# realphongha/UDP-Pose

Measured on AMD Instinct MI355X. Metric: images/sec HRNet-W32 256x192 (infer+decode), higher is better.
Workload: dtype f16x2 (split fp16 hi+lo operands = 22 bits, 3 fp16 MFMAs per product, fp32 accumulate); 1 GPU; w32 256x192 f16x2 inference, batch=64 per GPU, flip-test on, DARK decode (forward on 2N images + flip fuse + udp_decode_gaussian); global_batch=64, parallelism=replicas x1 (no data-path collective), weights=seeded synthetic, BN stats calibrated (tests/golden/bn_calib_w32_gaussian.npz)

## Files before the change

udp-pose_amd/csrc/common.h:

```cpp
#pragma once
#include <hip/hip_runtime.h>

#include <cstdarg>
#include <cstdio>
#include <cstring>

#include "../../include/udp_pose_hip.h"

namespace udp {

inline char* err_buf() {
  static thread_local char buf[512] = {0};
  return buf;
}

inline int fail(int code, const char* fmt, ...) {
  va_list ap;
  va_start(ap, fmt);
  vsnprintf(err_buf(), 512, fmt, ap);
  va_end(ap);
  return code;
}

#define UDP_HIP_CHECK(expr)                                                                  \
  do {                                                                                       \
    hipError_t e_ = (expr);                                                                  \
    if (e_ != hipSuccess)                                                                    \
      return udp::fail(UDP_ERR_HIP, "%s failed: %s (%s:%d)", #expr, hipGetErrorString(e_),   \
                       __FILE__, __LINE__);                                                  \
  } while (0)

inline int ceil_div(int a, int b) { return (a + b - 1) / b; }

static __device__ int g_h2_overflow;
__device__ __forceinline__ void h2_range_check(float m) {
  if (!(m < 65520.f)) g_h2_overflow = 1;
}
__device__ __forceinline__ unsigned h2_mag(float v) { return __builtin_bit_cast(unsigned, v) & 0x7FFFFFFFu; }
__device__ __forceinline__ unsigned h2_max(unsigned a, unsigned b) { return a > b ? a : b; }
__device__ __forceinline__ void h2_range_check_bits(unsigned m) {
  if (m >= __builtin_bit_cast(unsigned, 65520.f)) g_h2_overflow = 1;
}
static inline int h2_overflow_fetch(hipStream_t s, int reset, int* flag) {
  int v = 0;
  UDP_HIP_CHECK(hipMemcpyFromSymbolAsync(&v, HIP_SYMBOL(g_h2_overflow), sizeof(int), 0, hipMemcpyDeviceToHost, s));
  UDP_HIP_CHECK(hipStreamSynchronize(s));
  if (v && reset) {
    const int z = 0;
    UDP_HIP_CHECK(hipMemcpyToSymbolAsync(HIP_SYMBOL(g_h2_overflow), &z, sizeof(int), 0, hipMemcpyHostToDevice, s));
    UDP_HIP_CHECK(hipStreamSynchronize(s));
  }
  *flag |= v != 0;
  return UDP_OK;
}

struct ConvParams {
  const void* in;
  void* out;
  const void* wgt;
  const float* bias;
  const void* wgt2;
  const float* bias2;
  const void* res;
  const void* up[3];
  int up_shift[3];
  int nup;
  int N, Hin, Win, Cin, Hout, Wout, Cout, CoutPad;
  int in_pitch, in_coff, out_pitch, out_coff, res_pitch, res_coff;
  int G, R, TW;
  int IH, IW;
  int tiles_x, tiles_y;
  unsigned mTX, mTY;
  int ntiles;
  unsigned mIW, mIH, mRT, mTW;
  int relu;
  int out_nchw_f32;
  int flip_from;
  int sbuf;
  int wfmt;
  int wexp;
  int in_stuff2;
  double* bn_ws;
  void* out2[2];
  const void* add2[2];
  int nout2, out2_coff[2], out2_pitch[2], add2_coff[2], add2_pitch[2];
};

constexpr int kMultiSegs = 64;
constexpr int kMultiTab = 480;
struct ConvMulti {
  ConvParams p[4];
  unsigned start[5];
  unsigned tiles[4];
  unsigned ncby[4];
  int code[4];
  unsigned seg_start[kMultiSegs];
  unsigned seg_first[kMultiSegs];
  int seg_mem[kMultiSegs];
  unsigned tab_n;
  unsigned tab[kMultiTab];
};

}

namespace udp {
struct Launch {
  const void* fn = nullptr;
  dim3 grid, block;
  unsigned lds = 0;
  int groupable = 0;
  int ws_cp = 0;
  ConvParams p;
};
int describe_conv_ws(ConvParams p, int ks, int stride, Launch* out, bool grouped = false);
struct WsTile {
  int cp, pb, G, R, TW, wgs, sbuf;
  size_t lds;
};
int choose_conv_ws(ConvParams& p, int ks, int stride, bool grouped, WsTile* best);
int describe_ws_multi(const Launch* members, int n, ConvMulti* m, Launch* out);
int describe_conv_chain(ConvParams p, Launch* out);
void ws_set_fill_wgs(long wgs);
int ws_set_stamps(unsigned long long* dev_buf);
int describe_deconv(ConvParams p, int dtype, Launch* out);
int deconv_h2_overflow(hipStream_t s, int reset, int* flag);
int dwconv_validate(const udp_conv_op& o, int dtype);
int pixshuf_validate(const udp_conv_op& o, int dtype);
int describe_dwconv(ConvParams p, int dtype, int ks, int stride, Launch* out);
int describe_pixshuf(ConvParams p, int dtype, Launch* out);
int se_validate(const udp_conv_op& o, int dtype);
int describe_se(ConvParams p, int dtype, Launch* out);
int dwconv_h2_overflow(hipStream_t s, int reset, int* flag);
int gnorm_validate(const udp_conv_op& o, int dtype);
int linattn_validate(const udp_conv_op& o, int dtype);
int describe_gnorm(ConvParams p, int dtype, Launch* out);
int describe_linattn(ConvParams p, int dtype, Launch* out);
int lnorm_validate(const udp_conv_op& o, int dtype);
int mhattn_validate(const udp_conv_op& o, int dtype);
int act_op_validate(const udp_conv_op& o, int dtype);
int describe_lnorm(ConvParams p, int dtype, Launch* out);
int describe_mhattn(ConvParams p, int dtype, Launch* out);
int describe_act(ConvParams p, int dtype, Launch* out);
int attn_h2_overflow(hipStream_t s, int reset, int* flag);
int conv_h2_overflow(hipStream_t s, int reset, int* flag);
int conv_ws_h2_overflow(hipStream_t s, int reset, int* flag);
int psa_h2_overflow(hipStream_t s, int reset, int* flag);
}
```

udp-pose_amd/csrc/conv.hip:

```cpp
#include "conv_dev.h"

namespace udp {
template <typename T, int KS, int NB, int MBW>
__device__ __forceinline__ void mfma_chunk(f32x4 (&acc)[MBW][NB], const unsigned char* sb, const unsigned char* wrow,
                                           const int (&prow)[MBW], int IW, int kg, int wswz) {
  constexpr bool F32 = std::is_same<T, float>::value;
  constexpr int BN = NB * 16;
  constexpr int NSTEP = KS * KS * (F32 ? 2 : 1);
  using Frag = typename std::conditional<F32, f32x2, bf16x8>::type;
  Frag wf[2][NB], pf[2][MBW];
  auto load = [&](int s, Frag (&w)[NB], Frag (&x)[MBW]) {
    const int tap = F32 ? s >> 1 : s;
    const int ks = F32 ? (s & 1) : 0;
    const int part = F32 ? 2 * ks + (kg >> 1) : kg;
    const int sub = F32 ? (kg & 1) * 8 : 0;
    const int tap_rows = (tap / KS) * IW + tap % KS;
#pragma unroll
    for (int nb = 0; nb < NB; ++nb)
      w[nb] = *reinterpret_cast<const Frag*>(wrow + (tap * BN + nb * 16) * ROWB + ((part ^ wswz) << 4) + sub);
#pragma unroll
    for (int i = 0; i < MBW; ++i) {
      const int row = prow[i] + tap_rows;
      x[i] = *reinterpret_cast<const Frag*>(sb + row * ROWB + ((part ^ swz<T>(row)) << 4) + sub);
    }
// ... 1080 lines not shown
        const int gx = xo * 2 - 1 + kx;
        if (gx < 0 || gx >= p.Win) continue;
        const f32x4 v = ld4<T>(p.in, (size_t)(n * p.Hin + gy) * p.Win + gx, p.in_pitch, p.in_coff + c);
#pragma unroll
        for (int q = 0; q < 4; ++q) m[q] = v[q] > m[q] ? v[q] : m[q];
      }
    }
    st4<T>(p.out, (size_t)pix, p.out_pitch, p.out_coff + c, m);
  }
}

template <typename T>
__global__ __launch_bounds__(256) void bilinear_ac_kernel(const ConvParams p) {
  const int C4 = p.Cout >> 2;
  const long total = (long)p.N * p.Hout * p.Wout * C4;
  const float sy = p.Hout > 1 ? (float)(p.Hin - 1) / (float)(p.Hout - 1) : 0.f;
  const float sx = p.Wout > 1 ? (float)(p.Win - 1) / (float)(p.Wout - 1) : 0.f;
  for (long idx = (long)blockIdx.x * 256 + threadIdx.x; idx < total; idx += (long)gridDim.x * 256) {
    const int c = (idx % C4) * 4;
    const long pix = idx / C4;
    const int xo = pix % p.Wout;
    const long t2 = pix / p.Wout;
    const int y = t2 % p.Hout;
    const int n = t2 / p.Hout;
    const float fy = sy * (float)y, fx = sx * (float)xo;
    const int y0 = (int)fy, x0 = (int)fx;
    const int y1 = y0 + (y0 < p.Hin - 1 ? 1 : 0), x1 = x0 + (x0 < p.Win - 1 ? 1 : 0);
    const float ly = fy - (float)y0, lx = fx - (float)x0;
    const float hy = 1.f - ly, hx = 1.f - lx;
    const size_t ib = (size_t)n * p.Hin * p.Win;
    const f32x4 v00 = ld4<T>(p.in, ib + (size_t)y0 * p.Win + x0, p.in_pitch, p.in_coff + c);
    const f32x4 v01 = ld4<T>(p.in, ib + (size_t)y0 * p.Win + x1, p.in_pitch, p.in_coff + c);
    const f32x4 v10 = ld4<T>(p.in, ib + (size_t)y1 * p.Win + x0, p.in_pitch, p.in_coff + c);
    const f32x4 v11 = ld4<T>(p.in, ib + (size_t)y1 * p.Win + x1, p.in_pitch, p.in_coff + c);
    f32x4 v;
#pragma unroll
    for (int q = 0; q < 4; ++q) v[q] = hy * (hx * v00[q] + lx * v01[q]) + ly * (hx * v10[q] + lx * v11[q]);
    st4<T>(p.out, (size_t)pix, p.out_pitch, p.out_coff + c, v);
  }
}

size_t conv_choose_tile(ConvParams& p, int ks, int stride, int dtype, int* nb_out, bool grouped = false) {
  auto knob = [](const char* name, long dflt) {
    const char* v = getenv(name);
    return v ? atol(v) : dflt;
  };
  const int kMaxM = (int)knob("UDP_POSE_MAXM", 256);
  const int ck = dtype == UDP_F32 ? 16 : 32;
  const int planes = dtype == UDP_F16X2 ? 2 : 1;
  static const bool h2_dbuf = getenv("UDP_POSE_H2_DBUF") != nullptr;
  p.sbuf = planes == 2 && !h2_dbuf;
  const int nstage = ceil_div(p.Cin, ck) > 1 && !p.sbuf ? 2 : 1;
  int TW = p.Wout;
  while (TW > 64) TW = (TW + 1) / 2;
  int maxR = kMaxM / TW;
  if (maxR < 1) maxR = 1;
  if (maxR > p.Hout) maxR = p.Hout;
  int R = largest_divisor_leq(p.Hout, maxR);
  if (R * 2 <= maxR) R = maxR;
  int G = 1;
  if (R == p.Hout && TW == p.Wout) {
    G = kMaxM / (R * TW);
    if (G < 1) G = 1;
    if (G > p.N) G = p.N;
  }
  int NB = (p.CoutPad % 64 == 0 && !grouped) ? 4 : 2;
  auto npix = [&](int g, int r) { return g * ((r - 1) * stride + ks) * ((TW - 1) * stride + ks); };
  auto lds = [&](int g, int r, int nb) {
    return (size_t)(((npix(g, r) + 15) / 16) * 16 + ks * ks * nb * 16) * ROWB * nstage * planes;
  };
  auto wgs = [&](int g, int r, int nb) {
    return (long)ceil_div(p.N, g) * ceil_div(p.Hout, r) * ceil_div(p.Wout, TW) * (p.CoutPad / (nb * 16));
  };
  const long kMinWgs = grouped ? 0 : knob("UDP_POSE_MINWGS", 512);
  if (wgs(G, R, NB) < kMinWgs && NB == 4) NB = 2;
  while (wgs(G, R, NB) < kMinWgs && G > 1) G = (G + 1) / 2;
  const size_t kLimit = (size_t)knob("UDP_POSE_LDS_KB", planes == 2 && nstage == 2 ? 156 : 76) * 1024;
  while ((lds(G, R, NB) > kLimit || npix(G, R) > MAXG * 64) && G > 1) --G;
  static const bool s2nb4 = getenv("UDP_POSE_NO_S2_NB4") == nullptr;
  if (s2nb4 && stride == 2 && NB == 4)
    while ((lds(G, R, NB) > kLimit || npix(G, R) > MAXG * 64) && R > 2) R = (R + 1) / 2;
  while ((lds(G, R, NB) > kLimit || npix(G, R) > MAXG * 64) && NB == 4) NB = 2;
  while ((lds(G, R, NB) > kLimit || npix(G, R) > MAXG * 64) && R > 1) R = (R + 1) / 2;
  p.G = G;
  p.R = R;
  p.TW = TW;
  p.IH = (R - 1) * stride + ks;
  p.IW = (TW - 1) * stride + ks;
  p.tiles_x = ceil_div(p.Wout, TW);
  p.tiles_y = ceil_div(p.Hout, R);
  auto magic = [](int d) { return (unsigned)(((1u << 20) + (unsigned)d - 1) / (unsigned)d); };
  p.mIW = magic(p.IW);
  p.mIH = magic(p.IH);
  p.mRT = magic(R * TW);
  p.mTW = magic(TW);
  p.ntiles = ceil_div(p.N, G) * p.tiles_y * p.tiles_x;
  auto magic32 = [](int d) { return d == 1 ? 0u : (unsigned)((0x100000000ULL + (unsigned)d - 1) / (unsigned)d); };
  p.mTX = magic32(p.tiles_x);
  p.mTY = magic32(p.tiles_y);
  *nb_out = NB;
  return lds(G, R, NB);
}

template <typename T, int KS, int STRIDE, int NB, int MBW, bool NCHW, int NW>
static int describe_one(const ConvParams& p, size_t lds, Launch* out) {
  static bool attr_set = false;
  const void* kern = reinterpret_cast<const void*>(&conv_mfma_kernel<T, KS, STRIDE, NB, MBW, NCHW, NW>);
  if (!attr_set) {
    UDP_HIP_CHECK(hipFuncSetAttribute(kern, hipFuncAttributeMaxDynamicSharedMemorySize, 160 * 1024));
    attr_set = true;
  }
  out->fn = kern;
  out->grid = dim3(ceil_div(p.N, p.G) * p.tiles_y * p.tiles_x, p.CoutPad / (NB * 16));
  out->block = dim3(NW * 64);
  out->lds = (unsigned)lds;
  out->p = p;
  return UDP_OK;
}

template <typename T, int NB, int MBW, int ACT>
static int describe_hs_one(const ConvParams& p, size_t lds, Launch* out) {
  static bool attr_set = false;
  const void* kern = reinterpret_cast<const void*>(&conv1x1_hs_kernel<T, NB, MBW, ACT>);
  if (!attr_set) {
    UDP_HIP_CHECK(hipFuncSetAttribute(kern, hipFuncAttributeMaxDynamicSharedMemorySize, 160 * 1024));
    attr_set = true;
  }
  out->fn = kern;
  out->grid = dim3(ceil_div(p.N, p.G) * p.tiles_y * p.tiles_x, p.CoutPad / (NB * 16));
  out->block = dim3(256);
  out->lds = (unsigned)lds;
  out->p = p;
  return UDP_OK;
}
template <typename T>
static int describe_hs(const ConvParams& p, int nb, int mbw, size_t lds, Launch* out) {
#define UDP_HS(B, M) \
  if (nb == B && mbw == M) return p.relu == UDP_ACT_SILU ? describe_hs_one<T, B, M, UDP_ACT_SILU>(p, lds, out) : describe_hs_one<T, B, M, UDP_ACT_HSWISH>(p, lds, out);
  UDP_HS(2, 1) UDP_HS(2, 2) UDP_HS(2, 3) UDP_HS(2, 4) UDP_HS(4, 1) UDP_HS(4, 2) UDP_HS(4, 3) UDP_HS(4, 4)
#undef UDP_HS
  return fail(UDP_ERR_UNSUPPORTED, "1x1 conv + hard-swish / SiLU: no kernel for nb=%d, %d pixel blocks per wave", nb, mbw);
}

template <typename T, int KS, int STRIDE, int NB, bool NCHW>
static int describe_mbw(const ConvParams& p, int mbw, size_t lds, Launch* out) {
  static const bool w8 = getenv("UDP_POSE_CONV_8W") != nullptr;
  if (w8 && std::is_same<T, __bf16>::value && !NCHW && mbw >= 3)
    return mbw == 3 ? describe_one<T, KS, STRIDE, NB, 2, NCHW, 8>(p, lds, out) : describe_one<T, KS, STRIDE, NB, 2, NCHW, 8>(p, lds, out);
  switch (mbw) {
    case 1: return describe_one<T, KS, STRIDE, NB, 1, NCHW, 4>(p, lds, out);
    case 2: return describe_one<T, KS, STRIDE, NB, 2, NCHW, 4>(p, lds, out);
    case 3: return describe_one<T, KS, STRIDE, NB, 3, NCHW, 4>(p, lds, out);
    case 4: return describe_one<T, KS, STRIDE, NB, 4, NCHW, 4>(p, lds, out);
  }
  return fail(UDP_ERR_UNSUPPORTED, "conv tile of %d pixel blocks per wave has no kernel", mbw);
}

template <typename T>
static int describe_conv_t(const ConvParams& p, int ks, int stride, int nb, int mbw, size_t lds, Launch* out) {
#define UDP_CASE(K, S, B)                                                              \
  if (ks == K && stride == S && nb == B && !p.out_nchw_f32) return describe_mbw<T, K, S, B, false>(p, mbw, lds, out);
#define UDP_CASE_OUT(K, S, B)                                                          \
  if (ks == K && stride == S && nb == B && p.out_nchw_f32) return describe_mbw<T, K, S, B, true>(p, mbw, lds, out);
  UDP_CASE(3, 1, 2) UDP_CASE(3, 1, 4) UDP_CASE(3, 2, 2) UDP_CASE(3, 2, 4)
  UDP_CASE(1, 1, 2) UDP_CASE(1, 1, 4) UDP_CASE(1, 2, 2) UDP_CASE(1, 2, 4)
  UDP_CASE_OUT(1, 1, 2) UDP_CASE_OUT(1, 1, 4) UDP_CASE_OUT(3, 1, 2) UDP_CASE_OUT(3, 1, 4)
#undef UDP_CASE
#undef UDP_CASE_OUT
  return fail(UDP_ERR_UNSUPPORTED, "conv ks=%d stride=%d nb=%d nchw_out=%d has no kernel", ks, stride, nb,
              p.out_nchw_f32);
}

template <int KS, int STRIDE, int NB, int MBW>
static int describe_persist_one(const ConvParams& p, size_t lds, int grid_x, Launch* out) {
  static bool attr_set = false;
  const void* kern = reinterpret_cast<const void*>(&conv_mfma_persist1<__bf16, KS, STRIDE, NB, MBW>);
  if (!attr_set) {
    UDP_HIP_CHECK(hipFuncSetAttribute(kern, hipFuncAttributeMaxDynamicSharedMemorySize, 160 * 1024));
    attr_set = true;
  }
  out->fn = kern;
  out->grid = dim3(grid_x, p.CoutPad / (NB * 16));
  out->block = dim3(256);
  out->lds = (unsigned)lds;
  out->p = p;
  return UDP_OK;
}

template <int KS, int STRIDE, int NB>
static int describe_persist_mbw(const ConvParams& p, int mbw, size_t lds, int grid_x, Launch* out) {
  switch (mbw) {
    case 1: return describe_persist_one<KS, STRIDE, NB, 1>(p, lds, grid_x, out);
    case 2: return describe_persist_one<KS, STRIDE, NB, 2>(p, lds, grid_x, out);
    case 3: return describe_persist_one<KS, STRIDE, NB, 3>(p, lds, grid_x, out);
    case 4: return describe_persist_one<KS, STRIDE, NB, 4>(p, lds, grid_x, out);
  }
  return 1;
}

static int persist_grid(const ConvParams& p, int ks, int stride, int nb, size_t* lds_out) {
  const int npix = p.G * p.IH * p.IW;
  if (p.out_nchw_f32 || p.Cin != 32 || npix > MAXGP * 64 || p.ntiles >= 65536 || p.bn_ws || p.in_stuff2) return 0;
  if (p.in_pitch != p.Cin || p.in_coff || p.out_pitch != p.Cout || p.out_coff || (p.res && (p.res_pitch != p.Cout || p.res_coff)))
    return 0;
  if (!((ks == 3 || ks == 1) && (stride == 1 || (stride == 2 && ks == 3)))) return 0;
  const size_t lds = (size_t)(ks * ks * nb * 16 + 2 * ((npix + 15) / 16) * 16) * ROWB;
  int per_cu = (int)((150 * 1024) / lds);
  if (per_cu > 4) per_cu = 4;
  if (per_cu < 1) return 0;
  const int cblocks = p.CoutPad / (nb * 16);
  const int budget = ceil_div(256 * per_cu, cblocks);
  if (p.ntiles < 2 * budget) return 0;
  const int rounds = ceil_div(p.ntiles, budget);
  *lds_out = lds;
  return ceil_div(p.ntiles, rounds);
}
static int describe_persist(const ConvParams& p, int ks, int stride, int nb, int mbw, Launch* out) {
  size_t lds = 0;
  const int grid_x = persist_grid(p, ks, stride, nb, &lds);
  if (grid_x == 0) return 1;
#define UDP_CASE(K, S, B) \
  if (ks == K && stride == S && nb == B) return describe_persist_mbw<K, S, B>(p, mbw, lds, grid_x, out);
  UDP_CASE(3, 1, 2) UDP_CASE(3, 1, 4) UDP_CASE(3, 2, 2) UDP_CASE(3, 2, 4) UDP_CASE(1, 1, 2) UDP_CASE(1, 1, 4)
#undef UDP_CASE
  return 1;
}

template <int MBW1, int MBW2, int NW>
static int describe_block_one(const ConvParams& p, size_t lds, int grid_x, Launch* out) {
  static bool attr_set = false;
  const void* kern = reinterpret_cast<const void*>(&basic_block_c32_kernel<MBW1, MBW2, NW>);
  if (!attr_set) {
    UDP_HIP_CHECK(hipFuncSetAttribute(kern, hipFuncAttributeMaxDynamicSharedMemorySize, 160 * 1024));
    attr_set = true;
  }
  out->fn = kern;
  out->grid = dim3(grid_x);
  out->block = dim3(NW * 64);
  out->lds = (unsigned)lds;
  out->p = p;
  return UDP_OK;
}

int describe_block(ConvParams p, int dtype, Launch* out) {
  if (dtype != UDP_BF16 || p.Cin != 32 || p.Cout != 32) return fail(UDP_ERR_UNSUPPORTED, "fused BasicBlock: bf16 with 32 channels only");
  if (p.Hin % kBlkR || p.Hin != p.Hout || p.Win != p.Wout) return fail(UDP_ERR_UNSUPPORTED, "fused BasicBlock: height must be a multiple of %d", kBlkR);
  p.R = kBlkR;
  p.IH = kBlkR + 4;
  p.IW = p.Win + 2;
  p.TW = p.Win;
  p.G = 1;
  const int rows_in = p.IH * p.IW, rows_mid = (kBlkR + 2) * p.IW;
  if (rows_in > kBlkMaxG * 64) return fail(UDP_ERR_UNSUPPORTED, "fused BasicBlock: map too wide (%d)", p.Win);
  const int m1 = (kBlkR + 2) * p.Win, m2 = kBlkR * p.Win;
  int nw = m2 > 128 && getenv("UDP_POSE_BLOCK_4W") == nullptr ? 8 : 4;
  if (m2 > 256 && getenv("UDP_POSE_BLOCK_16W") != nullptr) nw = 16;
  const int mbw1 = ceil_div(m1, nw * 16), mbw2 = ceil_div(m2, nw * 16);
  p.tiles_x = 1;
  p.tiles_y = p.Hin / kBlkR;
  p.ntiles = p.N * p.tiles_y;
  if (p.ntiles >= 65536) return fail(UDP_ERR_UNSUPPORTED, "fused BasicBlock: too many tiles");
  auto magic20 = [](int d) { return (unsigned)(((1u << 20) + d - 1) / d); };
  auto magic32 = [](int d) { return d == 1 ? 0u : (unsigned)((0x100000000ULL + (unsigned)d - 1) / (unsigned)d); };
  p.mIW = magic20(p.IW);
  p.mTW = magic20(p.Win);
  p.mTY = magic32(p.tiles_y);
  const size_t lds = 2 * 9 * 32 * ROWB + (size_t)((rows_mid + 15) / 16) * 16 * ROWB + 2 * (size_t)((rows_in + 15) / 16) * 16 * ROWB;
  if (lds > 160 * 1024) return fail(UDP_ERR_UNSUPPORTED, "fused BasicBlock: %zu bytes of LDS", lds);
  const int grid_x = p.ntiles < 256 ? p.ntiles : ceil_div(p.ntiles, ceil_div(p.ntiles, 256));
  if (nw == 16 && mbw1 == 2 && mbw2 == 2) return describe_block_one<2, 2, 16>(p, lds, grid_x, out);
  if (nw == 8 && mbw1 == 4 && mbw2 == 3) return describe_block_one<4, 3, 8>(p, lds, grid_x, out);
  if (nw == 8 && mbw1 == 2 && mbw2 == 2) return describe_block_one<2, 2, 8>(p, lds, grid_x, out);
  if (nw == 4 && mbw1 == 8 && mbw2 == 6) return describe_block_one<8, 6, 4>(p, lds, grid_x, out);
  if (nw == 4 && mbw1 == 4 && mbw2 == 3) return describe_block_one<4, 3, 4>(p, lds, grid_x, out);
  if (nw == 4 && mbw1 == 3 && mbw2 == 2) return describe_block_one<3, 2, 4>(p, lds, grid_x, out);
  if (nw == 4 && mbw1 == 2 && mbw2 == 1) return describe_block_one<2, 1, 4>(p, lds, grid_x, out);
  return fail(UDP_ERR_UNSUPPORTED, "fused BasicBlock: no kernel for %d columns", p.Win);
}

int describe_conv(ConvParams p, int dtype, int ks, int stride, Launch* out) {
  if (p.Cin % 16 != 0) return fail(UDP_ERR_UNSUPPORTED, "conv Cin=%d is not a multiple of 16", p.Cin);
  if (!p.out_nchw_f32 && p.Cout % 16 != 0)
    return fail(UDP_ERR_UNSUPPORTED, "NHWC conv Cout=%d is not a multiple of 16", p.Cout);
  const size_t esz = dtype == UDP_F32 ? 4 : 2;
  const size_t pix_esz = dtype == UDP_BF16 ? 2 : 4;
  if ((size_t)p.N * p.Hin * p.Win * p.in_pitch * pix_esz >= 0x7FFF0000u || (size_t)p.N * p.Hout * p.Wout * p.out_pitch * 4 >= 0x7FFF0000u ||
      (p.in_coff * esz) % 16 || (p.in_pitch * esz) % 16 ||
      (!p.out_nchw_f32 && ((p.out_coff * esz) % 16 || (p.out_pitch * esz) % 16)) ||
      (p.res && ((p.res_coff * esz) % 16 || (p.res_pitch * esz) % 16)))
    return fail(UDP_ERR_UNSUPPORTED, "conv channel views must be 16-byte aligned and tensors < 2 GiB");
  if (false ||
      p.N >= 2048)
    return fail(UDP_ERR_UNSUPPORTED, "conv tensor exceeds the 2 GiB the 32-bit buffer offsets cover; split the batch");
  if (p.in_stuff2 && (dtype == UDP_F16X2 || stride != 1 || (p.Hin & 1) || (p.Win & 1)))
    return fail(UDP_ERR_UNSUPPORTED, "in_stuff2: a stride-1 fp32 / bf16 conv over an even-sized stuffed image");
  if (p.relu >= UDP_ACT_HSWISH && (ks != 1 || stride != 1 || p.out_nchw_f32 || p.res || p.nup || p.nout2 || p.in_stuff2 || p.bn_ws || dtype == UDP_BF16))
    return fail(UDP_ERR_UNSUPPORTED, "hard-swish / SiLU (activation codes 2, 4): plain 1x1 stride-1 NHWC convs in f32 / f16x2 only");
  if (p.nout2 && p.wfmt != 1) return fail(UDP_ERR_UNSUPPORTED, "second outputs need the weight-stationary split-fp16 conv (wfmt 1)");
  if (p.wfmt == 1) {
    if (dtype != UDP_F16X2) return fail(UDP_ERR_ARG, "wfmt 1 (fragment-major weights) needs UDP_F16X2");
    return describe_conv_ws(p, ks, stride, out);
  }
  if (p.wfmt != 0) return fail(UDP_ERR_ARG, "conv wfmt=%d", p.wfmt);
  int nb = 2;
  const size_t lds = conv_choose_tile(p, ks, stride, dtype, &nb);
  if (p.CoutPad % (nb * 16) != 0)
    return fail(UDP_ERR_UNSUPPORTED, "conv CoutPad=%d is not a multiple of %d", p.CoutPad, nb * 16);
  const int mbw = ceil_div(ceil_div(p.G * p.R * p.TW, 16), 4);
  if (getenv("UDP_POSE_DEBUG_TILES"))
    fprintf(stderr, "conv k%d s%d %dx%d C%d->%d: G=%d R=%d TW=%d NB=%d mbw=%d lds=%zu wgs=%d\n", ks, stride, p.Hout, p.Wout, p.Cin,
            p.Cout, p.G, p.R, p.TW, nb, mbw, lds, p.ntiles * (p.CoutPad / (nb * 16)));
  if (p.relu >= UDP_ACT_HSWISH) return dtype == UDP_F32 ? describe_hs<float>(p, nb, mbw, lds, out) : describe_hs<H2>(p, nb, mbw, lds, out);
  if (dtype == UDP_BF16 && getenv("UDP_POSE_NO_PERSIST") == nullptr) {
    const int rc = describe_persist(p, ks, stride, nb, mbw, out);
    if (rc <= 0) return rc;
  }
  if (dtype == UDP_F32) return describe_conv_t<float>(p, ks, stride, nb, mbw, lds, out);
  if (dtype == UDP_F16X2) return describe_conv_t<H2>(p, ks, stride, nb, mbw, lds, out);
  return describe_conv_t<__bf16>(p, ks, stride, nb, mbw, lds, out);
}

extern "C" int udp_debug_conv_tile(int dtype, int wfmt, int ks, int stride, int n, int hout, int wout, int cin, int cout,
                                   int nchw_out, int grouped, int* out) {
  if (!out || n < 1 || hout < 1 || wout < 1 || cin < 1 || cout < 1) return fail(UDP_ERR_ARG, "udp_debug_conv_tile: bad argument");
  if ((ks != 1 && ks != 3) || (stride != 1 && stride != 2)) return fail(UDP_ERR_ARG, "udp_debug_conv_tile: ks/stride");
  if (dtype != UDP_F32 && dtype != UDP_BF16 && dtype != UDP_F16X2) return fail(UDP_ERR_ARG, "udp_debug_conv_tile: dtype %d", dtype);
  ConvParams p;
  memset(&p, 0, sizeof(p));
  p.N = n;
  p.Hout = hout;
  p.Wout = wout;
  p.Hin = hout * stride;
  p.Win = wout * stride;
  p.Cin = p.in_pitch = cin;
  p.Cout = p.out_pitch = p.res_pitch = cout;
  p.CoutPad = (cout + 31) / 32 * 32;
  p.out_nchw_f32 = nchw_out ? 1 : 0;
  p.wfmt = wfmt;
  p.flip_from = n;
  if (p.Cin % 16 != 0) return fail(UDP_ERR_UNSUPPORTED, "conv Cin=%d is not a multiple of 16", p.Cin);
  if (!p.out_nchw_f32 && p.Cout % 16 != 0) return fail(UDP_ERR_UNSUPPORTED, "NHWC conv Cout=%d is not a multiple of 16", p.Cout);
  for (int i = 0; i < 9; ++i) out[i] = 0;
  if (wfmt == 1) {
    if (dtype != UDP_F16X2) return fail(UDP_ERR_ARG, "wfmt 1 (fragment-major weights) needs UDP_F16X2");
    if (grouped && (stride != 1 || p.out_nchw_f32)) return 1;
    WsTile t{};
    if (const int rc = choose_conv_ws(p, ks, stride, grouped != 0, &t)) return rc;
    out[0] = t.pb;
    out[1] = t.cp;
    out[5] = t.sbuf;
    out[6] = (int)t.lds;
    out[7] = t.wgs;
  } else {
    if (wfmt != 0) return fail(UDP_ERR_ARG, "conv wfmt=%d", wfmt);
    if (grouped && (dtype == UDP_F32 || stride != 1 || p.out_nchw_f32)) return 1;
    int nb = 2;
    const size_t lds = conv_choose_tile(p, ks, stride, dtype, &nb, grouped != 0);
    if (p.CoutPad % (nb * 16) != 0) return fail(UDP_ERR_UNSUPPORTED, "conv CoutPad=%d is not a multiple of %d", p.CoutPad, nb * 16);
    const int mbw = ceil_div(ceil_div(p.G * p.R * p.TW, 16), 4);
    if (grouped && (nb != 2 || p.G * p.R * p.TW > 256)) return 1;
    if (mbw < 1 || mbw > 4) return fail(UDP_ERR_UNSUPPORTED, "conv tile of %d pixel blocks per wave has no kernel", mbw);
    out[0] = nb;
    out[1] = mbw;
    out[5] = p.sbuf;
    out[6] = (int)lds;
    out[7] = p.ntiles * (p.CoutPad / (nb * 16));
    if (dtype == UDP_BF16 && !grouped && getenv("UDP_POSE_NO_PERSIST") == nullptr) {
      size_t plds = 0;
      out[8] = persist_grid(p, ks, stride, nb, &plds);
      if (out[8]) out[6] = (int)plds;
    }
  }
  out[2] = p.G;
  out[3] = p.R;
  out[4] = p.TW;
  return UDP_OK;
}

int describe_conv_grouped(ConvParams p, int dtype, int ks, int stride, Launch* out) {
  if (p.relu >= UDP_ACT_HSWISH) return fail(UDP_ERR_UNSUPPORTED, "hard-swish / SiLU (activation codes 2, 4) have no merged-launch form");
  if (p.wfmt == 1 && dtype == UDP_F16X2 && stride == 1 && (ks == 1 || ks == 3) && !p.out_nchw_f32 && !p.nup) {
    return describe_conv_ws(p, ks, stride, out, true);
  }
  if (p.wfmt != 0 || (dtype != UDP_BF16 && dtype != UDP_F16X2) || (ks != 3 && ks != 1) || stride != 1 || p.out_nchw_f32 || p.nup || p.Cin % 16 || p.Cout % 16 || p.CoutPad % 32 ||
      (p.in_stuff2 && dtype != UDP_BF16))
    return 1;
  const size_t pix_esz = dtype == UDP_BF16 ? 2 : 4;
  if ((size_t)p.N * p.Hin * p.Win * p.in_pitch * pix_esz >= 0x7FFF0000u || (size_t)p.N * p.Hout * p.Wout * p.out_pitch * pix_esz >= 0x7FFF0000u ||
      (p.in_coff * 2) % 16 || (p.in_pitch * 2) % 16 ||
      (p.out_coff * 2) % 16 || (p.out_pitch * 2) % 16 || (p.res && ((p.res_coff * 2) % 16 || (p.res_pitch * 2) % 16)) || p.N >= 2048)
    return 1;
  int nb = 2;
  const size_t lds = conv_choose_tile(p, ks, stride, dtype, &nb, true);
  if (nb != 2 || p.G * p.R * p.TW > 256) return 1;
  if (getenv("UDP_POSE_DEBUG_TILES"))
    fprintf(stderr, "grouped conv %dx%d C%d->%d: G=%d R=%d TW=%d NB=2 lds=%zu wgs=%d\n", p.Hout, p.Wout, p.Cin, p.Cout, p.G, p.R,
            p.TW, lds, p.ntiles * (p.CoutPad / 32));
  const int mbw = ceil_div(ceil_div(p.G * p.R * p.TW, 16), 4);
  const bool m3 = mbw <= 3 && getenv("UDP_POSE_MULTI_MBW4") == nullptr;
  int rc;
  if (dtype == UDP_F16X2) {
    if (ks == 3)
      rc = m3 ? describe_one<H2, 3, 1, 2, 3, false, 4>(p, lds, out) : describe_one<H2, 3, 1, 2, 4, false, 4>(p, lds, out);
    else
      rc = m3 ? describe_one<H2, 1, 1, 2, 3, false, 4>(p, lds, out) : describe_one<H2, 1, 1, 2, 4, false, 4>(p, lds, out);
  } else if (ks == 3) {
    rc = m3 ? describe_one<__bf16, 3, 1, 2, 3, false, 4>(p, lds, out) : describe_one<__bf16, 3, 1, 2, 4, false, 4>(p, lds, out);
  } else {
    rc = m3 ? describe_one<__bf16, 1, 1, 2, 3, false, 4>(p, lds, out) : describe_one<__bf16, 1, 1, 2, 4, false, 4>(p, lds, out);
  }
  if (rc) return rc;
  out->groupable = (dtype == UDP_F16X2 ? 100 : 0) + ks * 10 + (m3 ? 3 : 4);
  return UDP_OK;
}

int describe_multi(const Launch* members, int n, ConvMulti* m, Launch* out) {
  static bool attr_set = false;
  const void* kerns[8] = {reinterpret_cast<const void*>(&conv_mfma_multi<__bf16, 3, 1, 2, 3, 4>),
                          reinterpret_cast<const void*>(&conv_mfma_multi<__bf16, 3, 1, 2, 4, 4>),
                          reinterpret_cast<const void*>(&conv_mfma_multi<__bf16, 1, 1, 2, 3, 4>),
                          reinterpret_cast<const void*>(&conv_mfma_multi<__bf16, 1, 1, 2, 4, 4>),
                          reinterpret_cast<const void*>(&conv_mfma_multi<H2, 3, 1, 2, 3, 4>),
                          reinterpret_cast<const void*>(&conv_mfma_multi<H2, 3, 1, 2, 4, 4>),
                          reinterpret_cast<const void*>(&conv_mfma_multi<H2, 1, 1, 2, 3, 4>),
                          reinterpret_cast<const void*>(&conv_mfma_multi<H2, 1, 1, 2, 4, 4>)};
  if (!attr_set) {
    for (const void* k : kerns) UDP_HIP_CHECK(hipFuncSetAttribute(k, hipFuncAttributeMaxDynamicSharedMemorySize, 160 * 1024));
    attr_set = true;
  }
  if (n < 2 || n > 4) return fail(UDP_ERR_ARG, "describe_multi: %d members", n);
  if (members[0].groupable / 100 == 3) return describe_ws_multi(members, n, m, out);
  const int h2 = members[0].groupable / 100;
  const int ks = members[0].groupable / 10 % 10;
  int mbw = 3;
  for (int j = 0; j < n; ++j) {
    if (members[j].groupable / 10 != members[0].groupable / 10) return fail(UDP_ERR_ARG, "describe_multi: members of different kernel sizes / storage types");
    if (members[j].groupable % 10 > mbw) mbw = members[j].groupable % 10;
  }
  const void* kern = kerns[4 * h2 + (ks == 3 ? 0 : 2) + (mbw == 3 ? 0 : 1)];
  memset(m, 0, sizeof(*m));
  unsigned total = 0, lds = 0;
  for (int j = 0; j < n; ++j) {
    m->p[j] = members[j].p;
    m->start[j] = total;
    m->tiles[j] = members[j].grid.x;
    total += members[j].grid.x * members[j].grid.y;
    if (members[j].lds > lds) lds = members[j].lds;
  }
  for (int j = n; j < 5; ++j) m->start[j] = j < 4 ? 0xFFFFFFFFu : total;
  for (int j = n; j < 4; ++j) m->tiles[j] = 1;
  out->fn = kern;
  out->grid = dim3(total);
  out->block = dim3(256);
  out->lds = lds;
  out->groupable = 0;
  return UDP_OK;
}

int describe_stem(const ConvParams& p, int dtype, Launch* out) {
  if (p.Cout != 64) return fail(UDP_ERR_UNSUPPORTED, "stem conv expects 64 output channels, got %d", p.Cout);
  const long total = (long)p.N * p.Hout * p.Wout;
  if (p.relu >= UDP_ACT_HSWISH) {
    const bool si = p.relu == UDP_ACT_SILU;
    if (dtype == UDP_BF16) return fail(UDP_ERR_UNSUPPORTED, "stem conv + hard-swish / SiLU: storage modes f32 and f16x2 only");
    out->block = dim3(256);
    out->p = p;
    if (dtype == UDP_F16X2 && getenv("UDP_POSE_STEM_VALU") == nullptr) {
      const long ntile = (total + 15) / 16;
      out->fn = si ? reinterpret_cast<const void*>(&stem_mfma_k<H2, 3, UDP_ACT_SILU>) : reinterpret_cast<const void*>(&stem_mfma_k<H2, 3, UDP_ACT_HSWISH>);
      out->grid = dim3((unsigned)((ntile + 3) / 4 < 2048 ? (ntile + 3) / 4 : 2048));
      out->lds = 1 * 4 * 2 * 1024;
      return UDP_OK;
    }
    out->fn = dtype == UDP_F32 ? (si ? reinterpret_cast<const void*>(&stem_conv_kernel<float, UDP_ACT_SILU>) : reinterpret_cast<const void*>(&stem_conv_kernel<float, UDP_ACT_HSWISH>))
                               : (si ? reinterpret_cast<const void*>(&stem_conv_kernel<H2, UDP_ACT_SILU>) : reinterpret_cast<const void*>(&stem_conv_kernel<H2, UDP_ACT_HSWISH>));
    out->grid = dim3((unsigned)((total + 63) / 64));
    out->lds = 0;
    return UDP_OK;
  }
  if (dtype == UDP_BF16 && getenv("UDP_POSE_STEM_VALU") == nullptr) {
    const long ntile = (total + 15) / 16;
    out->fn = reinterpret_cast<const void*>(&stem_mfma_kernel);
    out->grid = dim3((unsigned)((ntile + 3) / 4 < 4096 ? (ntile + 3) / 4 : 4096));
    out->block = dim3(256);
    out->lds = 0;
    out->p = p;
    return UDP_OK;
  }
  if (dtype == UDP_F16X2 && getenv("UDP_POSE_STEM_VALU") == nullptr) {
    const long ntile = (total + 15) / 16;
    out->fn = reinterpret_cast<const void*>(&stem_mfma_k<H2, 3>);
    out->grid = dim3((unsigned)((ntile + 3) / 4 < 2048 ? (ntile + 3) / 4 : 2048));
    out->block = dim3(256);
    out->lds = 1 * 4 * 2 * 1024;
    out->p = p;
    return UDP_OK;
  }
  out->fn = dtype == UDP_F32     ? reinterpret_cast<const void*>(&stem_conv_kernel<float>)
            : dtype == UDP_F16X2 ? reinterpret_cast<const void*>(&stem_conv_kernel<H2>)
                                 : reinterpret_cast<const void*>(&stem_conv_kernel<__bf16>);
  out->grid = dim3((unsigned)((total + 63) / 64));
  out->block = dim3(256);
  out->lds = 0;
  out->p = p;
  return UDP_OK;
}

int describe_fuse(const ConvParams& p, int dtype, Launch* out) {
  if (p.Cout % 4 != 0) return fail(UDP_ERR_UNSUPPORTED, "fuse Cout=%d is not a multiple of 4", p.Cout);
  const long total = (long)p.N * p.Hout * p.Wout * (p.Cout / 4);
  long blocks = (total + 255) / 256;
  if (blocks > 8192) blocks = 8192;
  out->fn = dtype == UDP_F32     ? reinterpret_cast<const void*>(&fuse_sum_kernel<float>)
            : dtype == UDP_F16X2 ? reinterpret_cast<const void*>(&fuse_sum_kernel<H2>)
                                 : reinterpret_cast<const void*>(&fuse_sum_kernel<__bf16>);
  out->grid = dim3((unsigned)blocks);
  out->block = dim3(256);
  out->lds = 0;
  out->p = p;
  return UDP_OK;
}

#ifdef UDP_STAMPS
extern "C" int udp_debug_set_stamps(unsigned long long* dev_buf) {
  UDP_HIP_CHECK(hipMemcpyToSymbol(HIP_SYMBOL(g_stamps), &dev_buf, sizeof(dev_buf)));
  return ws_set_stamps(dev_buf);
}
#endif

template <typename KF, typename KB, typename KH>
static int describe_elementwise(const ConvParams& p, int dtype, KF kf, KB kb, KH kh, Launch* out) {
  if (p.Cout % 4 != 0) return fail(UDP_ERR_UNSUPPORTED, "element-wise op: C=%d is not a multiple of 4", p.Cout);
  const long total = (long)p.N * p.Hout * p.Wout * (p.Cout / 4);
  long blocks = (total + 255) / 256;
  if (blocks > 8192) blocks = 8192;
  out->fn = dtype == UDP_F32 ? reinterpret_cast<const void*>(kf)
                             : dtype == UDP_F16X2 ? reinterpret_cast<const void*>(kh) : reinterpret_cast<const void*>(kb);
  out->grid = dim3((unsigned)blocks);
  out->block = dim3(256);
  out->lds = 0;
  out->p = p;
  return UDP_OK;
}

int describe_maxpool(const ConvParams& p, int dtype, Launch* out) {
  return describe_elementwise(p, dtype, &maxpool3_kernel<float>, &maxpool3_kernel<__bf16>, &maxpool3_kernel<H2>, out);
}

int describe_bilinear(const ConvParams& p, int dtype, Launch* out) {
  return describe_elementwise(p, dtype, &bilinear_ac_kernel<float>, &bilinear_ac_kernel<__bf16>, &bilinear_ac_kernel<H2>, out);
}

template <typename T>
__global__ __launch_bounds__(256) void stem7_lds_kernel(const ConvParams p) {
  constexpr bool SPLIT = std::is_same<T, H2>::value;
  constexpr int KS = 7, K = KS * KS * 3, NS = (K + 31) / 32, PAD = 3, WPL = SPLIT ? 2 : 1;
  constexpr int TR = 2, TC = 32, WR = 2 * TR + 5, WC = 2 * TC + 5, WP = 72, WIN = 3 * WR * WC, PER = (WIN + 255) / 256;
  using E = typename std::conditional<SPLIT, _Float16, __bf16>::type;
  using Frag = typename std::conditional<SPLIT, f16x8, bf16x8>::type;
  extern __shared__ __attribute__((aligned(16))) unsigned char smem[];
  E* wl = reinterpret_cast<E*>(smem);
  float* win = reinterpret_cast<float*>(smem + NS * 4 * WPL * 1024);
  const int tid = threadIdx.x, lane = tid & 63, wave = tid >> 6;
  const int li = lane & 15, kg = lane >> 4;
  const float* wg = reinterpret_cast<const float*>(p.wgt);
  for (int e = tid; e < NS * 4 * WPL * 512; e += 256) {
    const int j = e & 7, ln = (e >> 3) & 63, pl = (e >> 9) % WPL, nb = ((e >> 9) / WPL) & 3, st = (e >> 9) / (WPL * 4);
    const int k = 32 * st + 8 * (ln >> 4) + j;
    const int cout = 16 * ((ln & 15) >> 2) + 4 * nb + (ln & 3);
    const float w = k < K ? wg[k * 64 + cout] : 0.f;
    if constexpr (SPLIT) {
      const _Float16 hi = (_Float16)w;
      wl[e] = pl == 0 ? hi : (_Float16)((w - (float)hi) * kLoScale);
    } else {
      wl[e] = (__bf16)w;
    }
  }
  const int cbase = 16 * kg;
  f32x4 bias[4];
#pragma unroll
  for (int nb = 0; nb < 4; ++nb) bias[nb] = *reinterpret_cast<const f32x4*>(p.bias + cbase + 4 * nb);
  unsigned koff[NS][4];
#pragma unroll
  for (int st = 0; st < NS; ++st)
#pragma unroll
    for (int h = 0; h < 4; ++h) {
      unsigned v = 0;
#pragma unroll
      for (int q = 0; q < 2; ++q) {
        const int k = 32 * st + 8 * kg + 2 * h + q, tap = k / 3;
        const unsigned c = k < K ? (unsigned)(((k % 3) * WR + tap / KS) * WP + tap % KS) : 0xFFFFu;
        v |= c << (16 * q);
      }
      koff[st][h] = v;
    }
  const int tiles_x = (p.Wout + TC - 1) / TC, tiles_y = (p.Hout + TR - 1) / TR;
  const long ntile = (long)p.N * tiles_y * tiles_x;
  const size_t plane = (size_t)p.Hin * p.Win;
  auto fetch = [&](long t, float (&v)[PER]) __attribute__((always_inline)) {
    const int tx = (int)(t % tiles_x);
    const long t2 = t / tiles_x;
    const int ty = (int)(t2 % tiles_y), n = (int)(t2 / tiles_y);
    const bool mirror = n >= p.flip_from;
    const float* in = reinterpret_cast<const float*>(p.in) + (size_t)(mirror ? n - p.flip_from : n) * 3 * plane;
    const int gy0 = ty * TR * 2 - PAD, gx0 = tx * TC * 2 - PAD;
#pragma unroll
// ... 156 lines not shown
```

udp-pose_amd/csrc/conv_ws.hip:

```cpp
#include "conv_dev.h"

namespace udp {

#ifndef UDP_WS_LATE_RES
#define UDP_WS_LATE_RES 1
#endif
template <int NB>
struct ResH2 {
  u32x4 hi[NB / 2], lo[NB / 2];
};
template <int NB>
__device__ __forceinline__ void load_res_h2(ResH2<NB>& o, __amdgpu_buffer_rsrc_t r, unsigned voff, unsigned lo_off) {
#pragma unroll
  for (int h = 0; h < NB / 2; ++h) {
    o.hi[h] = __builtin_amdgcn_raw_buffer_load_b128(r, voff + 16 * h, 0, UDP_H2_RES_AUX);
    o.lo[h] = __builtin_amdgcn_raw_buffer_load_b128(r, voff + lo_off + 16 * h, 0, UDP_H2_RES_AUX);
  }
}
template <int NB>
__device__ __forceinline__ void add_res_h2(f32x4 (&v)[NB], const ResH2<NB>& o) {
#pragma unroll
  for (int h = 0; h < NB / 2; ++h) h2_add8(v[2 * h], v[2 * h + 1], __builtin_bit_cast(f16x8, o.hi[h]), __builtin_bit_cast(f16x8, o.lo[h]));
}

template <int KS, int STRIDE, int PB, int CP, bool NCHW, bool OUT2 = false, int HS = 0, bool NUP = true>
__device__ __forceinline__ void conv_ws_body(const ConvParams& p, const int tile_id, const int cby) {
  using T = H2;
  constexpr int CK = 32, ESZ = 2, NB = 2, NW = 4;
  constexpr int PAD = KS / 2, TAPS = KS * KS;
  extern __shared__ __attribute__((aligned(16))) unsigned char smem[];

  UDP_STAMP(0);
  const int tid = threadIdx.x;
  const int lane = tid & 63;
  const int wave = __builtin_amdgcn_readfirstlane(tid >> 6);
  const int li = lane & 15;
  const int kg = lane >> 4;
  const int cp = wave % CP, pg = wave / CP;

  int t = tile_id;
  const int tx = t % p.tiles_x;
  t /= p.tiles_x;
  const int ty = t % p.tiles_y;
  const int n0 = (t / p.tiles_y) * p.G;
  const int y0 = ty * p.R;
  const int x0 = tx * p.TW;

  const int IH = p.IH, IW = p.IW;
  const int npix_in = p.G * IH * IW;
  const int in_groups = (npix_in + 15) >> 4;
  const int in_bytes = in_groups * 16 * ROWB;
  const int stage_bytes = 2 * in_bytes;
  const int nchunks = (p.Cin + CK - 1) / CK;
  const bool ragged = (p.Cin % CK) != 0;
  const int RT = p.R * p.TW;
  const int M = p.G * RT;
  const unsigned inpb = (unsigned)p.in_pitch * ESZ * 2;
  const unsigned outpb = (unsigned)p.out_pitch * ESZ * 2, respb = (unsigned)p.res_pitch * ESZ * 2;
  const unsigned in_lo = (unsigned)p.in_pitch * ESZ;
  const unsigned out_lo = (unsigned)p.out_pitch * ESZ, res_lo = (unsigned)p.res_pitch * ESZ;

  const unsigned out_pix = (unsigned)p.N * p.Hout * p.Wout;
  const __amdgpu_buffer_rsrc_t r_in = __builtin_amdgcn_make_buffer_rsrc(
      const_cast<void*>(p.in), 0, (unsigned)p.N * p.Hin * p.Win * inpb, 0x00020000);
  const unsigned npairs = (unsigned)p.CoutPad >> 5;
  const __amdgpu_buffer_rsrc_t r_w = __builtin_amdgcn_make_buffer_rsrc(
      const_cast<void*>(p.wgt), 0, (unsigned)TAPS * nchunks * npairs * 4096u, 0x00020000);
#if UDP_WS_DBG & 32
  const bool dbg_nost = nchunks == 1;
#else
  constexpr bool dbg_nost = false;
#endif
#if UDP_WS_DBG & 64
  const bool dbg_nores = nchunks == 1;
#else
  constexpr bool dbg_nores = false;
#endif
  const __amdgpu_buffer_rsrc_t r_out = __builtin_amdgcn_make_buffer_rsrc(
      p.out, 0, (!p.out || dbg_nost) ? 0 : NCHW ? out_pix * p.Cout * 4 : out_pix * outpb, 0x00020000);
  const __amdgpu_buffer_rsrc_t r_bias = __builtin_amdgcn_make_buffer_rsrc(
      const_cast<float*>(p.bias), 0, (unsigned)p.CoutPad * 4u, 0x00020000);
  const __amdgpu_buffer_rsrc_t r_res = __builtin_amdgcn_make_buffer_rsrc(
      const_cast<void*>(p.res), 0, (p.res && !dbg_nores) ? out_pix * respb : 0, 0x00020000);

  const int cwave = (cby * CP + cp) * 32;
  const int cbase = cwave + 8 * kg;
  const unsigned wvoff = (unsigned)lane * 16u;
  const unsigned wpair = (unsigned)(cby * CP + cp) * 4096u;
  constexpr int AD = UDP_WS_AD;
  f16x8 ah[AD][NB], al[AD][NB];
  const int nsteps = nchunks * TAPS;
  auto load_a = [&](int s, f16x8 (&h)[NB], f16x8 (&l)[NB]) __attribute__((always_inline)) {
    const int c = s / TAPS, tap = s - c * TAPS;
    const unsigned soff = (unsigned)(tap * nchunks + c) * (npairs * 4096u) + wpair;
#pragma unroll
    for (int nb = 0; nb < NB; ++nb) {
      h[nb] = __builtin_bit_cast(f16x8, __builtin_amdgcn_raw_buffer_load_b128(r_w, wvoff + 2048u * nb, soff, 0));
      l[nb] = __builtin_bit_cast(f16x8, __builtin_amdgcn_raw_buffer_load_b128(r_w, wvoff + 2048u * nb + 1024u, soff, 0));
    }
  };

#pragma unroll
  for (int k = 0; k < AD - 1; ++k) load_a(k < nsteps ? k : nsteps - 1, ah[k], al[k]);
  f32x4 bias[NB];
#pragma unroll
  for (int nb = 0; nb < NB; ++nb)
    bias[nb] = __builtin_bit_cast(f32x4, __builtin_amdgcn_raw_buffer_load_b128(r_bias, (unsigned)(cbase + 4 * nb) * 4u, 0, 0));

  const int srow = lane >> 2, spart = lane & 3;
  const int gy0 = y0 * STRIDE - PAD, gx0 = x0 * STRIDE - PAD;
  unsigned src_off[MAXG];
#pragma unroll
  for (int i = 0; i < MAXG; ++i) {
    unsigned off = kOobOff;
    if ((wave + NW * i) * 16 < npix_in) {
      const int row = (wave + NW * i) * 16 + srow;
      const int tmp = fdiv20(row, p.mIW);
      const int ix = row - (int)__umul24(tmp, IW);
      const int g = fdiv20(tmp, p.mIH);
      const int iy = tmp - (int)__umul24(g, IH);
      const int n = n0 + g, gy = gy0 + iy, gx = gx0 + ix;
      const bool ok = row < npix_in && n < p.N && (unsigned)gy < (unsigned)p.Hin && (unsigned)gx < (unsigned)p.Win;
      const unsigned pix = __umul24(__umul24(n, p.Hin) + gy, p.Win) + gx;
      off = ok ? pix * inpb + p.in_coff * ESZ + ((spart ^ swz<T>(row)) << 4) : kOobOff;
    }
    src_off[i] = off;
  }
  auto stage = [&](int c, unsigned char* sb) __attribute__((always_inline)) {
    const unsigned coff = (unsigned)c * (CK * ESZ);
    const bool cut = ragged && c == nchunks - 1;
    const int parts_left = (p.Cin - c * CK) / 8;
#pragma unroll
    for (int i = 0; i < MAXG; ++i) {
      const int gidx = wave + NW * i;
      if (gidx < in_groups) {
        unsigned off = src_off[i] + coff;
        if (cut && (spart ^ swz<T>(gidx * 16 + srow)) >= parts_left) off = kOobOff;
        blds16(r_in, off, sb + gidx * (16 * ROWB));
        blds16(r_in, off + in_lo, sb + in_bytes + gidx * (16 * ROWB));
      }
    }
  };

  UDP_STAMP(1);
  stage(0, smem);

  int prow[PB], opix[PB], ocrd[NCHW || NUP ? PB : 1];
#pragma unroll
  for (int i = 0; i < PB; ++i) {
    const int m0 = (pg * PB + i) * 16 + li;
    const int m = m0 < M ? m0 : M - 1;
    const int g = fdiv20(m, p.mRT);
    const int rem = m - (int)__umul24(g, RT);
    const int r = fdiv20(rem, p.mTW);
    const int x = rem - (int)__umul24(r, p.TW);
    prow[i] = (int)__umul24(__umul24(g, IH) + r * STRIDE, IW) + x * STRIDE;
    const int n = n0 + g, y = y0 + r, xo = x0 + x;
    const bool ok = m0 < M && n < p.N && y < p.Hout && xo < p.Wout && (NCHW || cbase < p.Cout);
    const unsigned pix = __umul24(__umul24(n, p.Hout) + y, p.Wout) + xo;
    opix[i] = ok ? (int)pix : -1;
    if constexpr (NCHW || NUP) ocrd[i] = ok ? (y | (xo << 10) | (n << 20)) : -1;
  }

  const float winv = __builtin_ldexpf(1.f, -p.wexp);
  f32x4 acc[PB][NB];
#pragma unroll
  for (int i = 0; i < PB; ++i)
#pragma unroll
    for (int nb = 0; nb < NB; ++nb) acc[i][nb] = f32x4{0.f, 0.f, 0.f, 0.f};

  constexpr bool LATE = UDP_WS_LATE_RES && KS == 3 && STRIDE == 1 && !NCHW && AD == 3;
  constexpr int NR = NCHW ? 0 : PB * NB;
  ResH2<NB> rres[NCHW ? 1 : PB];
  constexpr int RSPLIT = LATE && PB > 6 ? PB / 2 : PB;
  auto load_res = [&](auto I0, auto I1) __attribute__((always_inline)) {
    __builtin_amdgcn_sched_barrier(0);
    asm volatile("" ::: "memory");
#pragma unroll
    for (int i = decltype(I0)::value; i < (NCHW ? 0 : decltype(I1)::value); ++i)
      load_res_h2(rres[i], r_res, opix[i] >= 0 ? (unsigned)opix[i] * respb + (p.res_coff + cbase) * ESZ : kOobOff, res_lo);
    asm volatile("" ::: "memory");
    __builtin_amdgcn_sched_barrier(0);
  };
  if constexpr (!LATE) load_res(std::integral_constant<int, 0>{}, std::integral_constant<int, PB>{});

  UDP_STAMP(2);
  int c = 0, tap = 0;
  const unsigned char* sb = smem;
  auto step = [&](auto BUFC, auto TAILC, int s) __attribute__((always_inline)) {
    constexpr int BUF = decltype(BUFC)::value, TAIL = decltype(TAILC)::value;
#if !(UDP_WS_DBG & 1)
    if constexpr (!LATE)
      load_a(s + AD - 1 < nsteps ? s + AD - 1 : nsteps - 1, ah[(BUF + AD - 1) % AD], al[(BUF + AD - 1) % AD]);
    else if constexpr (TAIL <= 0)
      load_a(s + AD - 1, ah[(BUF + AD - 1) % AD], al[(BUF + AD - 1) % AD]);
#endif
    if constexpr (TAIL == 0) load_res(std::integral_constant<int, 0>{}, std::integral_constant<int, RSPLIT>{});
    if constexpr (TAIL == 1 && RSPLIT < PB) load_res(std::integral_constant<int, RSPLIT>{}, std::integral_constant<int, PB>{});
    if (TAIL < 0 && tap == 0) {
      if (c == 1) UDP_STAMP(9);
      if (c == 2) UDP_STAMP(11);
      if (c == 4) UDP_STAMP(13);
      bool refill = false;
      if constexpr (STRIDE == 2 || OUT2) refill = p.sbuf && c > 0;
      if (refill) {
        __syncthreads();
        stage(c, smem);
        asm volatile("s_waitcnt vmcnt(0)" ::: "memory");
        __syncthreads();
        sb = smem;
      } else {
        if (s == 0)
          asm volatile("s_waitcnt vmcnt(%0)" ::"n"(2 * NB + (LATE ? 0 : NR)) : "memory");
        else
          asm volatile("s_waitcnt vmcnt(%0)" ::"n"(2 * NB) : "memory");
        if (s == 0) UDP_STAMP(3);
        __syncthreads();
        if (s == 0) UDP_STAMP(4);
        if (c == 1) UDP_STAMP(10);
        if (c == 2) UDP_STAMP(12);
        if (c == 4) UDP_STAMP(14);
#if !(UDP_WS_DBG & 4)
        if (c + 1 < nchunks && !((STRIDE == 2 || OUT2) && p.sbuf)) stage(c + 1, smem + ((c + 1) & 1) * stage_bytes);
#endif
        sb = smem + (c & 1) * stage_bytes;
      }
    }
    f16x8 a2[NB];
#pragma unroll
    for (int nb = 0; nb < NB; ++nb) a2[nb] = ah[BUF][nb] * (_Float16)0x1p-11f;
    const int tap_rows = KS == 1 ? 0 : TAIL >= 0 ? (KS - 1) * IW + TAIL : (tap / KS) * IW + tap % KS;
    f16x8 xh[3], xl[3];
    auto load_b = [&](int i, f16x8& h, f16x8& l) __attribute__((always_inline)) {
      const int row = prow[i] + tap_rows;
      const unsigned char* q = sb + row * ROWB + ((kg ^ swz<T>(row)) << 4);
      h = *reinterpret_cast<const f16x8*>(q);
      l = *reinterpret_cast<const f16x8*>(q + in_bytes);
    };
    load_b(0, xh[0], xl[0]);
    if (PB > 1) load_b(1, xh[1], xl[1]);
#pragma unroll
    for (int i = 0; i < PB; ++i) {
#if !(UDP_WS_DBG & 2)
      if (i + 2 < PB) load_b(i + 2, xh[(i + 2) % 3], xl[(i + 2) % 3]);
#endif
      __builtin_amdgcn_sched_barrier(0);
#if UDP_WS_DBG & 16
      acc[i][0] = __builtin_amdgcn_mfma_f32_16x16x32_f16(ah[BUF][0] + al[BUF][1] + a2[0] + a2[1], xh[i % 3] + xl[i % 3], acc[i][0], 0, 0, 0);
#else
#pragma unroll
      for (int nb = 0; nb < NB; ++nb) acc[i][nb] = __builtin_amdgcn_mfma_f32_16x16x32_f16(ah[BUF][nb], xh[i % 3], acc[i][nb], 0, 0, 0);
#pragma unroll
      for (int nb = 0; nb < NB; ++nb) acc[i][nb] = __builtin_amdgcn_mfma_f32_16x16x32_f16(al[BUF][nb], xh[i % 3], acc[i][nb], 0, 0, 0);
#pragma unroll
      for (int nb = 0; nb < NB; ++nb) acc[i][nb] = __builtin_amdgcn_mfma_f32_16x16x32_f16(a2[nb], xl[i % 3], acc[i][nb], 0, 0, 0);
#endif
    }
    if constexpr (TAIL < 0) {
      if (++tap == TAPS) {
        tap = 0;
        ++c;
      }
    }
  };
  constexpr std::integral_constant<int, -1> LOOP{};
  if constexpr (LATE) {
    for (int s = 0; s < nsteps - AD; s += AD) {
      step(std::integral_constant<int, 0>{}, LOOP, s);
      step(std::integral_constant<int, 1>{}, LOOP, s + 1);
      step(std::integral_constant<int, 2>{}, LOOP, s + 2);
    }
    step(std::integral_constant<int, 0>{}, std::integral_constant<int, 0>{}, nsteps - 3);
    step(std::integral_constant<int, 1>{}, std::integral_constant<int, 1>{}, nsteps - 2);
    step(std::integral_constant<int, 2>{}, std::integral_constant<int, 2>{}, nsteps - 1);
  } else {
    for (int s = 0; s < nsteps; s += AD) {
      step(std::integral_constant<int, 0>{}, LOOP, s);
      if (s + 1 < nsteps) step(std::integral_constant<int, 1>{}, LOOP, s + 1);
      if (s + 2 < nsteps) step(std::integral_constant<int, 2>{}, LOOP, s + 2);
      if constexpr (AD > 3) if (s + 3 < nsteps) step(std::integral_constant<int, 3>{}, LOOP, s + 3);
      if constexpr (AD > 4) if (s + 4 < nsteps) step(std::integral_constant<int, 4>{}, LOOP, s + 4);
      if constexpr (AD > 5) if (s + 5 < nsteps) step(std::integral_constant<int, 5>{}, LOOP, s + 5);
    }
  }
  UDP_STAMP(5);
#pragma unroll
  for (int i = 0; i < PB; ++i) {
#pragma unroll
    for (int nb = 0; nb < NB; ++nb)
#pragma unroll
      for (int q = 0; q < 4; ++q) acc[i][nb][q] = __builtin_fmaf(acc[i][nb][q], winv, bias[nb][q]);
    if constexpr (!NCHW) add_res_h2(acc[i], rres[i]);
  }

#pragma unroll
  for (int i = 0; i < PB; ++i) {
    f32x4 v[NB];
#pragma unroll
    for (int nb = 0; nb < NB; ++nb) v[nb] = acc[i][nb];
    if constexpr (NCHW) {
      const int crd = ocrd[i];
      const int y = crd & 1023, xo = (crd >> 10) & 1023, n = crd >> 20;
      const unsigned hw = __umul24(p.Hout, p.Wout);
      const unsigned base = __umul24(__umul24(__umul24(n, p.Cout), p.Hout) + y, p.Wout) + xo;
#pragma unroll
      for (int nb = 0; nb < NB; ++nb)
#pragma unroll
        for (int q = 0; q < 4; ++q) {
          const int cc = cbase + 4 * nb + q;
          float f = v[nb][q];
          if (p.relu) f = f > 0.f ? f : 0.f;
          const unsigned off = (crd >= 0 && cc < p.Cout) ? (base + cc * hw) * 4u : kOobOff;
          __builtin_amdgcn_raw_buffer_store_b32(__builtin_bit_cast(unsigned, f), r_out, off, 0, 0);
        }
    } else {
      const unsigned ooff = opix[i] >= 0 ? (unsigned)opix[i] * outpb + (p.out_coff + cbase) * ESZ : kOobOff;
      if (NUP && p.nup) {
        const int crd = ocrd[NUP ? i : 0];
        const int y = crd & 1023, xo = (crd >> 10) & 1023, n = crd >> 20;
#pragma unroll
        for (int u = 0; u < 3; ++u) {
          if (u < p.nup) {
            const int sh = p.up_shift[u];
            const long up_pix = ((long)(n * (p.Hout >> sh) + (y >> sh)) * (p.Wout >> sh) + (xo >> sh));
            if (crd >= 0)
              add_vec<T, NB>(v, reinterpret_cast<const unsigned char*>(p.up[u]) + (up_pix * p.Cout * 2 + cbase) * ESZ, p.Cout * ESZ);
          }
        }
      }
      if constexpr (HS) {
#pragma unroll
        for (int nb = 0; nb < NB; ++nb)
#pragma unroll
          for (int q = 0; q < 4; ++q) v[nb][q] = act_hs<HS>(v[nb][q]);
      } else
      if (p.relu) {
#pragma unroll
        for (int nb = 0; nb < NB; ++nb)
#pragma unroll
          for (int q = 0; q < 4; ++q) v[nb][q] = v[nb][q] > 0.f ? v[nb][q] : 0.f;
      }
      store_vec_buf<T, NB>(r_out, ooff, out_lo, v);
      if (OUT2 && p.nout2) {
        f16x8 sh, sl;
        h2_split8(v[0], v[1], sh, sl);
        f32x4 vr[NB];
#pragma unroll
        for (int q = 0; q < 4; ++q) {
          vr[0][q] = (float)sh[q] + (float)sl[q] * kLoInv;
          vr[1][q] = (float)sh[4 + q] + (float)sl[4 + q] * kLoInv;
        }
#pragma unroll
        for (int u = 0; u < 2; ++u) {
          if (u < p.nout2 && opix[i] >= 0) {
            const size_t px = (size_t)opix[i];
            const _Float16* a = reinterpret_cast<const _Float16*>(p.add2[u]) + px * (2 * (size_t)p.add2_pitch[u]) + p.add2_coff[u] + cbase;
            const f16x8 ah8 = *reinterpret_cast<const f16x8*>(a), al8 = *reinterpret_cast<const f16x8*>(a + p.add2_pitch[u]);
            f32x4 w[NB];
#pragma unroll
            for (int q = 0; q < 4; ++q) {
              w[0][q] = ((float)ah8[q] + (float)al8[q] * kLoInv) + vr[0][q];
              w[1][q] = ((float)ah8[4 + q] + (float)al8[4 + q] * kLoInv) + vr[1][q];
            }
            f16x8 oh, ol;
            h2_split8(w[0], w[1], oh, ol);
            _Float16* o2 = reinterpret_cast<_Float16*>(p.out2[u]) + px * (2 * (size_t)p.out2_pitch[u]) + p.out2_coff[u] + cbase;
            *reinterpret_cast<f16x8*>(o2) = oh;
            *reinterpret_cast<f16x8*>(o2 + p.out2_pitch[u]) = ol;
          }
        }
      }
    }
  }
  UDP_STAMP(6);
#ifdef UDP_STAMPS
  asm volatile("s_waitcnt vmcnt(0)" ::: "memory");
  UDP_STAMP(7);
#endif
}

__host__ __device__ __forceinline__ void ws_decode(unsigned b, unsigned ntiles, unsigned nc, int& tile, int& cby) {
  if (nc == 1) {
    tile = (int)b;
    cby = 0;
    return;
  }
  const unsigned full = (ntiles >> 3) * 8u * nc;
  unsigned base = 0, width = 8, r = b;
  if (b < full) {
    const unsigned g = b / (8u * nc);
    r = b - g * 8u * nc;
    base = g * 8u;
  } else {
    r = b - full;
    base = (ntiles >> 3) * 8u;
    width = ntiles & 7u;
  }
  const unsigned c = r / width;
  cby = (int)c;
  tile = (int)(base + r - c * width);
}

template <int KS, int STRIDE, int PB, int CP, bool NCHW>
__global__ __launch_bounds__(256, 2) void conv_ws_h2_kernel(const ConvParams p) {
  int tile, cby;
  ws_decode(blockIdx.x + gridDim.x * blockIdx.y, gridDim.x, gridDim.y, tile, cby);
  conv_ws_body<KS, STRIDE, PB, CP, NCHW, KS == 3 && STRIDE == 1 && !NCHW>(p, tile, cby);
}

template <int PB, int CP, int ACT>
__global__ __launch_bounds__(256, 2) void conv_ws_hs_kernel(const ConvParams p) {
  int tile, cby;
  ws_decode(blockIdx.x + gridDim.x * blockIdx.y, gridDim.x, gridDim.y, tile, cby);
  conv_ws_body<1, 1, PB, CP, false, false, ACT>(p, tile, cby);
}

#ifndef UDP_WS_MPB
#define UDP_WS_MPB 6
#define UDP_WS_MOCC 2
#endif
constexpr int kWsCode8 = 8;
constexpr bool kWsHave8 = UDP_WS_MPB == 6 && UDP_WS_LATE_RES && UDP_WS_AD == 3;
template <int KS>
__global__ __launch_bounds__(256, UDP_WS_MOCC) void conv_ws_multi(const ConvMulti m) {
  const unsigned b = blockIdx.x;
  int j, tile, cby;
  int code;
  const unsigned e = __builtin_amdgcn_readfirstlane(m.tab[(b >> 3) < (unsigned)kMultiTab ? (b >> 3) : 0u]);
  if (m.tab_n) {
    j = (int)(e & 3u);
    code = 1 << ((e >> 2) & 3u);
    cby = (int)((e >> 4) & 63u);
    tile = (int)((e >> 10) + (b & 7u));
  } else {
    int sg = 0;
#pragma unroll
    for (int k = 1; k < kMultiSegs; ++k) sg += b >= m.seg_start[k];
    j = __builtin_amdgcn_readfirstlane(m.seg_mem[sg]);
    const unsigned r = __builtin_amdgcn_readfirstlane(b - m.seg_start[sg] + m.seg_first[sg]);
    ws_decode(r, m.tiles[j], m.ncby[j], tile, cby);
    tile = __builtin_amdgcn_readfirstlane(tile);
    cby = __builtin_amdgcn_readfirstlane(cby);
    code = m.code[j];
  }
  if constexpr (KS == 3 && kWsHave8) {
    if (code == kWsCode8) {
      conv_ws_body<KS, 1, 8, 1, false, false, 0, false>(m.p[j], tile, (int)cby);
      return;
    }
  }
  switch (code) {
    case 1: conv_ws_body<KS, 1, UDP_WS_MPB, 1, false>(m.p[j], tile, (int)cby); break;
    case 2: conv_ws_body<KS, 1, UDP_WS_MPB, 2, false>(m.p[j], tile, (int)cby); break;
    default: conv_ws_body<KS, 1, UDP_WS_MPB, 4, false>(m.p[j], tile, (int)cby); break;
  }
}

__global__ __launch_bounds__(256, 2) void conv_ws_pb8_kernel(const ConvParams p) {
  conv_ws_body<3, 1, 8, 1, false, false, 0, false>(p, (int)blockIdx.x, (int)blockIdx.y);
}

template <int KS, int STRIDE, int PB, int CP, bool NCHW>
static int describe_ws_one(const ConvParams& p, size_t lds, Launch* out) {
  static bool attr_set = false;
  const void* kern = reinterpret_cast<const void*>(&conv_ws_h2_kernel<KS, STRIDE, PB, CP, NCHW>);
  if (!attr_set) {
    UDP_HIP_CHECK(hipFuncSetAttribute(kern, hipFuncAttributeMaxDynamicSharedMemorySize, 160 * 1024));
    attr_set = true;
  }
  out->fn = kern;
  out->grid = dim3(p.ntiles, p.CoutPad / (CP * 32));
  out->block = dim3(256);
  out->lds = (unsigned)lds;
  out->p = p;
  return UDP_OK;
}
template <int KS, int STRIDE, bool NCHW>
static int describe_ws_pb(const ConvParams& p, int pb, int cp, size_t lds, Launch* out) {
#define UDP_WS(B, C) \
  if (pb == B && cp == C) return describe_ws_one<KS, STRIDE, B, C, NCHW>(p, lds, out);
  UDP_WS(2, 1) UDP_WS(3, 1) UDP_WS(4, 1) UDP_WS(6, 1) UDP_WS(2, 2) UDP_WS(3, 2) UDP_WS(4, 2) UDP_WS(6, 2)
  UDP_WS(2, 4) UDP_WS(3, 4) UDP_WS(4, 4) UDP_WS(6, 4)
#undef UDP_WS
  return 1;
}
static int describe_ws_pb8(const ConvParams& p, size_t lds, Launch* out) {
  static bool attr_set = false;
  const void* kern = reinterpret_cast<const void*>(&conv_ws_pb8_kernel);
  if (!attr_set) {
    UDP_HIP_CHECK(hipFuncSetAttribute(kern, hipFuncAttributeMaxDynamicSharedMemorySize, 160 * 1024));
    attr_set = true;
  }
  out->fn = kern;
  out->grid = dim3(p.ntiles, p.CoutPad / 32);
  out->block = dim3(256);
  out->lds = (unsigned)lds;
  out->p = p;
  return UDP_OK;
}
template <int PB, int CP, int ACT>
static int describe_ws_hs_one(const ConvParams& p, size_t lds, Launch* out) {
  static bool attr_set = false;
  const void* kern = reinterpret_cast<const void*>(&conv_ws_hs_kernel<PB, CP, ACT>);
  if (!attr_set) {
    UDP_HIP_CHECK(hipFuncSetAttribute(kern, hipFuncAttributeMaxDynamicSharedMemorySize, 160 * 1024));
    attr_set = true;
  }
  out->fn = kern;
  out->grid = dim3(p.ntiles, p.CoutPad / (CP * 32));
  out->block = dim3(256);
  out->lds = (unsigned)lds;
  out->p = p;
  return UDP_OK;
}
static int describe_ws_hs(const ConvParams& p, int pb, int cp, size_t lds, Launch* out) {
#define UDP_WS(B, C) \
  if (pb == B && cp == C) return p.relu == UDP_ACT_SILU ? describe_ws_hs_one<B, C, UDP_ACT_SILU>(p, lds, out) : describe_ws_hs_one<B, C, UDP_ACT_HSWISH>(p, lds, out);
  UDP_WS(2, 1) UDP_WS(3, 1) UDP_WS(4, 1) UDP_WS(6, 1) UDP_WS(2, 2) UDP_WS(3, 2) UDP_WS(4, 2) UDP_WS(6, 2)
  UDP_WS(2, 4) UDP_WS(3, 4) UDP_WS(4, 4) UDP_WS(6, 4)
#undef UDP_WS
  return 1;
}
static bool ws_tile(const ConvParams& p, int ks, int stride, int cp, int pb, WsTile* t, bool own_launch) {
  const int pg = 4 / cp;
  const int maxM = 16 * pb * pg;
  bool have = false;
  double best_util = 0.0;
  for (int split = 1; split <= 4 || !have; ++split) {
    if (split > 8) break;
    const int TW = ceil_div(p.Wout, split);
    if (TW > 64 || TW > maxM || (have && TW < 8)) continue;
    int maxR = maxM / TW;
    if (maxR > p.Hout) maxR = p.Hout;
    int R = largest_divisor_leq(p.Hout, maxR);
    if (R * 2 <= maxR) R = maxR;
    int G = 1;
    if (R == p.Hout && TW == p.Wout) {
      G = maxM / (R * TW);
      if (G > p.N) G = p.N;
      if (G < 1) G = 1;
    }
    auto npix = [&](int g, int r) { return g * ((r - 1) * stride + ks) * ((TW - 1) * stride + ks); };
    while (npix(G, R) > MAXG * 64 && G > 1) --G;
    while (npix(G, R) > MAXG * 64 && R > 1) R = (R + 1) / 2;
    if (npix(G, R) > MAXG * 64) continue;
    int nstage = ceil_div(p.Cin, 32) > 1 ? 2 : 1;
    size_t lds = (size_t)((npix(G, R) + 15) / 16) * 16 * ROWB * 2 * nstage;
    static const int sbuf_mode = getenv("UDP_POSE_WS_SBUF") == nullptr ? 1 : atoi(getenv("UDP_POSE_WS_SBUF"));
    const bool sbuf_kernel = stride == 2 || (ks == 3 && own_launch && sbuf_mode != 2);
    const bool sbuf = sbuf_kernel && nstage == 2 && lds > 80 * 1024 && lds / 2 <= 80 * 1024 && sbuf_mode != 0;
    if (sbuf) {
      nstage = 1;
      lds /= 2;
    }
    if (lds > 160 * 1024) continue;
    if (pb == 8 && (G * R * TW != maxM || p.Hout % R || TW * split != p.Wout || lds > 80 * 1024)) continue;
    const int need = ceil_div(ceil_div(G * R * TW, 16), pg);
    if (need > pb) continue;
    const int pbe = need <= 2 ? 2 : need <= 3 ? 3 : need <= 4 ? 4 : need <= 6 ? 6 : 8;
    const int tiles = ceil_div(p.N, G) * ceil_div(p.Hout, R) * ceil_div(p.Wout, TW);
    const double util = (double)p.N * p.Hout * p.Wout / ((double)tiles * 16 * pbe * pg) *
                        ((double)G * R * TW * stride * stride / (double)npix(G, R));
    if (!have || util > best_util + 0.05) {
      have = true;
      best_util = util;
      t->cp = cp;
      t->pb = pbe;
      t->G = G;
      t->R = R;
      t->TW = TW;
      t->lds = lds;
      t->sbuf = sbuf ? 1 : 0;
      t->wgs = tiles * (p.CoutPad / (cp * 32));
    }
  }
  return have;
}

static long g_ws_fill_wgs = 512;
void ws_set_fill_wgs(long wgs) { g_ws_fill_wgs = wgs; }

int choose_conv_ws(ConvParams& p, int ks, int stride, bool grouped, WsTile* best_out) {
  if (p.relu >= UDP_ACT_HSWISH && (ks != 1 || stride != 1 || p.out_nchw_f32 || p.res || p.nup || p.nout2 || grouped))
    return fail(UDP_ERR_UNSUPPORTED, "hard-swish / SiLU (activation codes 2, 4): plain 1x1 stride-1 NHWC convs on their own launch only");
  if ((stride != 1 && stride != 2) || (ks != 3 && ks != 1) || (p.out_nchw_f32 && stride != 1))
    return fail(UDP_ERR_UNSUPPORTED, "fragment-major weights (wfmt 1): conv ks=%d stride=%d nchw_out=%d has no weight-stationary kernel",
                ks, stride, p.out_nchw_f32);
  auto knob = [](const char* name, long dflt) {
    const char* v = getenv(name);
    return v ? atol(v) : dflt;
  };
  const int pairs = p.CoutPad / 32;
  const int force_cp = (int)knob("UDP_POSE_WS_CP", 0), force_pb = (int)knob("UDP_POSE_WS_PB", 0);
  const long min_wgs = grouped ? 0 : knob("UDP_POSE_WS_MINWGS", g_ws_fill_wgs);
  const bool offer8 = kWsHave8 && grouped && ks == 3 && stride == 1 && pairs % 2 == 1 && !p.out_nchw_f32 && !p.nout2 && !p.nup &&
                      knob("UDP_POSE_WS_PB8", 1) != 0;
  WsTile best{}, t{};
  bool have = false;
  for (int pb : {8, 6, 4, 3, 2}) {
    for (int cp : {4, 2, 1}) {
      if (pb == 8 && (!offer8 || cp != 1)) continue;
      if (pairs % cp || (force_cp && cp != force_cp) || (force_pb && pb != force_pb)) continue;
      if (grouped && stride == 1 && UDP_WS_MPB != 6 && pb != UDP_WS_MPB) continue;
      if (!ws_tile(p, ks, stride, cp, pb, &t, !grouped && !p.out_nchw_f32)) continue;
      const bool fills = t.wgs >= min_wgs, best_fills = have && best.wgs >= min_wgs;
      if (!have || (!best_fills && (fills || t.wgs > best.wgs))) {
        best = t;
// ... 142 lines not shown
    total += tiles[j] * ncby[j];
  }
  for (int j = n; j < 5; ++j) m.start[j] = j < 4 ? 0xFFFFFFFFu : total;
  m.start[4] = total;
  for (int j = n; j < 4; ++j) m.tiles[j] = m.ncby[j] = 1;
  if (total > cap) return -1;
  ws_order(&m, n);
  if (used_table) *used_table = m.tab_n != 0;
  for (unsigned b = 0; b < total; ++b) {
    int j, tile, cby;
    if (m.tab_n) {
      const unsigned e = m.tab[b >> 3];
      j = (int)(e & 3u);
      if ((1 << ((e >> 2) & 3u)) != m.code[j]) return -1;
      cby = (int)((e >> 4) & 63u);
      tile = (int)((e >> 10) + (b & 7u));
    } else {
      int sg = 0;
      for (int k = 1; k < kMultiSegs; ++k) sg += b >= m.seg_start[k];
      j = m.seg_mem[sg];
      ws_decode(b - m.seg_start[sg] + m.seg_first[sg], m.tiles[j], m.ncby[j], tile, cby);
    }
    out_member[b] = (unsigned)j;
    out_tile[b] = (unsigned)tile;
    out_cby[b] = (unsigned)cby;
  }
  return (int)total;
}

int describe_ws_multi(const Launch* members, int n, ConvMulti* m, Launch* out) {
  static bool ws_attr_set = false;
  const void* wk[2] = {reinterpret_cast<const void*>(&conv_ws_multi<3>), reinterpret_cast<const void*>(&conv_ws_multi<1>)};
  if (!ws_attr_set) {
    for (const void* k : wk) UDP_HIP_CHECK(hipFuncSetAttribute(k, hipFuncAttributeMaxDynamicSharedMemorySize, 160 * 1024));
    ws_attr_set = true;
  }
  memset(m, 0, sizeof(*m));
  unsigned total = 0, lds = 0;
  for (int j = 0; j < n; ++j) {
    if (members[j].groupable / 10 != members[0].groupable / 10) return fail(UDP_ERR_ARG, "describe_multi: mixed weight-stationary members");
    m->p[j] = members[j].p;
    m->start[j] = total;
    m->tiles[j] = members[j].grid.x;
    m->ncby[j] = members[j].grid.y;
    m->code[j] = members[j].groupable % 10 == 8 ? kWsCode8 : members[j].ws_cp;
    total += members[j].grid.x * members[j].grid.y;
    if (members[j].lds > lds) lds = members[j].lds;
  }
  for (int j = n; j < 5; ++j) m->start[j] = j < 4 ? 0xFFFFFFFFu : total;
  for (int j = n; j < 4; ++j) m->tiles[j] = m->ncby[j] = 1;
  ws_order(m, n);
  out->fn = wk[members[0].groupable / 10 % 10 == 3 ? 0 : 1];
  out->grid = dim3(total);
  out->block = dim3(256);
  out->lds = lds;
  out->groupable = 0;
  return UDP_OK;
}

#ifdef UDP_STAMPS
int ws_set_stamps(unsigned long long* dev_buf) {
  UDP_HIP_CHECK(hipMemcpyToSymbol(HIP_SYMBOL(g_stamps), &dev_buf, sizeof(dev_buf)));
  return UDP_OK;
}
extern "C" int udp_debug_set_stamps_ws(unsigned long long* dev_buf) { return ws_set_stamps(dev_buf); }
#endif

template <int NCH, int PB, int RD, bool LDSW>
__global__ __launch_bounds__(LDSW ? 512 : 256) __attribute__((amdgpu_waves_per_eu(2))) void conv_chain_kernel(const ConvParams p) {
  using T = H2;
  constexpr int ESZ = 2, NB = 2, Q = 2;
  constexpr int NWAVES = LDSW ? 8 : 4;
  constexpr int AD = LDSW ? 2 : 3;
  extern __shared__ __attribute__((aligned(16))) unsigned char smem[];
  const int lane = threadIdx.x & 63, wave = __builtin_amdgcn_readfirstlane(threadIdx.x >> 6);
  const int li = lane & 15, kg = lane >> 4;
  const unsigned npix = (unsigned)p.N * p.Hout * p.Wout;
  constexpr int NP = 8;
  const int cout2 = p.up_shift[0];
  const unsigned inpb = (unsigned)p.in_pitch * ESZ * 2, outpb = (unsigned)p.out_pitch * ESZ * 2, respb = (unsigned)p.res_pitch * ESZ * 2;
  const unsigned zpb = (unsigned)cout2 * ESZ * 2;
  const unsigned in_lo = (unsigned)p.in_pitch * ESZ, out_lo = (unsigned)p.out_pitch * ESZ, res_lo = (unsigned)p.res_pitch * ESZ;
  const unsigned z_lo = (unsigned)cout2 * ESZ;
  const __amdgpu_buffer_rsrc_t r_in = __builtin_amdgcn_make_buffer_rsrc(const_cast<void*>(p.in), 0, (p.sbuf & 8) ? 0 : npix * inpb, 0x00020000);
  const __amdgpu_buffer_rsrc_t r_w = __builtin_amdgcn_make_buffer_rsrc(const_cast<void*>(p.wgt), 0, (p.sbuf & 1) ? 0 : (unsigned)NCH * NP * 4096u, 0x00020000);
  const __amdgpu_buffer_rsrc_t r_w2 = __builtin_amdgcn_make_buffer_rsrc(const_cast<void*>(p.wgt2), 0, (p.sbuf & 1) ? 0 : (unsigned)NP * Q * 4096u, 0x00020000);
  const __amdgpu_buffer_rsrc_t r_bias = __builtin_amdgcn_make_buffer_rsrc(const_cast<float*>(p.bias), 0, (unsigned)p.CoutPad * 4u, 0x00020000);
  const __amdgpu_buffer_rsrc_t r_bias2 = __builtin_amdgcn_make_buffer_rsrc(const_cast<float*>(p.bias2), 0, (unsigned)cout2 * 4u, 0x00020000);
  const __amdgpu_buffer_rsrc_t r_res = __builtin_amdgcn_make_buffer_rsrc(const_cast<void*>(p.res), 0, (p.res && !(p.sbuf & 4)) ? npix * respb : 0, 0x00020000);
  const __amdgpu_buffer_rsrc_t r_out = __builtin_amdgcn_make_buffer_rsrc(p.out, 0, (p.sbuf & 2) ? 0 : npix * outpb, 0x00020000);
  const __amdgpu_buffer_rsrc_t r_z = __builtin_amdgcn_make_buffer_rsrc(const_cast<void*>(p.up[0]), 0, (p.sbuf & 2) ? 0 : npix * zpb, 0x00020000);
  const float winv = __builtin_ldexpf(1.f, -p.wexp), winv2 = __builtin_ldexpf(1.f, -p.up_shift[1]);
  const unsigned wvoff = (unsigned)lane * 16u;

  constexpr unsigned kW1 = (unsigned)NCH * 8 * 4096u, kBias = kW1 + 8u * Q * 4096u;
  if constexpr (LDSW) {
    for (unsigned blk = wave; blk < kBias / 1024u; blk += NWAVES) {
      const bool first = blk * 1024u < kW1;
      blds16(first ? r_w : r_w2, (first ? blk * 1024u : blk * 1024u - kW1) + wvoff, smem + blk * 1024u);
    }
    float* sbias = reinterpret_cast<float*>(smem + kBias);
    if (threadIdx.x < 256 + 64) sbias[threadIdx.x] = threadIdx.x < 256 ? p.bias[threadIdx.x] : p.bias2[threadIdx.x - 256];
    asm volatile("s_waitcnt vmcnt(0)" ::: "memory");
    __syncthreads();
  }
  const unsigned ngroups = (npix + PB * 16 - 1) / (PB * 16);
  for (unsigned grp = (unsigned)blockIdx.x * NWAVES + wave; grp < ngroups; grp += LDSW ? gridDim.x * NWAVES : ngroups) {
  unsigned wv = wvoff;
  int kgl = kg;
  if constexpr (LDSW) {
    asm volatile("" : "+v"(wv));
    asm volatile("" : "+v"(kgl));
  }
  unsigned pix[PB];
  bool ok[PB];
#pragma unroll
  for (int i = 0; i < PB; ++i) {
    pix[i] = grp * (PB * 16) + i * 16 + li;
    ok[i] = pix[i] < npix;
  }
  f16x8 xh[PB][NCH], xl[PB][NCH];
#pragma unroll
  for (int i = 0; i < PB; ++i)
#pragma unroll
    for (int c = 0; c < NCH; ++c) {
      const unsigned off = ok[i] ? pix[i] * inpb + (unsigned)(p.in_coff + 32 * c + 8 * kgl) * ESZ : kOobOff;
      xh[i][c] = __builtin_bit_cast(f16x8, __builtin_amdgcn_raw_buffer_load_b128(r_in, off, 0, 0));
      xl[i][c] = __builtin_bit_cast(f16x8, __builtin_amdgcn_raw_buffer_load_b128(r_in, off + in_lo, 0, 0));
    }
  constexpr int S = NCH + Q;
  f16x8 ah[AD][NB], al[AD][NB];
  auto load_a = [&](int pr, int st, f16x8 (&h)[NB], f16x8 (&l)[NB]) __attribute__((always_inline)) {
    const bool first = st < NCH;
    const unsigned soff = first ? (unsigned)(st * NP + pr) * 4096u : (unsigned)(pr * Q + (st - NCH)) * 4096u;
#pragma unroll
    for (int nb = 0; nb < NB; ++nb) {
      if constexpr (LDSW) {
        const unsigned char* q = smem + (first ? 0u : kW1) + soff + wv + 2048u * nb;
        h[nb] = *reinterpret_cast<const f16x8*>(q);
        l[nb] = *reinterpret_cast<const f16x8*>(q + 1024);
      } else {
        h[nb] = __builtin_bit_cast(f16x8, __builtin_amdgcn_raw_buffer_load_b128(first ? r_w : r_w2, wv + 2048u * nb, soff, 0));
        l[nb] = __builtin_bit_cast(f16x8, __builtin_amdgcn_raw_buffer_load_b128(first ? r_w : r_w2, wv + 2048u * nb + 1024u, soff, 0));
      }
    }
  };
  ResH2<NB> rres[RD][PB];
  auto load_res = [&](int pr, ResH2<NB> (&r)[PB]) __attribute__((always_inline)) {
#pragma unroll
    for (int i = 0; i < PB; ++i)
      load_res_h2(r[i], r_res, ok[i] ? pix[i] * respb + (unsigned)(p.res_coff + 32 * pr + 8 * kgl) * ESZ : kOobOff, res_lo);
  };
#pragma unroll
  for (int k = 0; k < RD - 1; ++k) load_res(k, rres[k]);
  load_a(0, 0, ah[0], al[0]);
  if constexpr (AD > 2) load_a(0, 1, ah[1], al[1]);

  f32x4 acc2[PB][Q][NB];
#pragma unroll
  for (int i = 0; i < PB; ++i)
#pragma unroll
    for (int q = 0; q < Q; ++q)
#pragma unroll
      for (int nb = 0; nb < NB; ++nb) acc2[i][q][nb] = f32x4{0.f, 0.f, 0.f, 0.f};

  auto mfma3 = [&](f32x4 (&acc)[NB], const f16x8 (&h)[NB], const f16x8 (&l)[NB], const f16x8 (&a2)[NB], const f16x8 bh, const f16x8 bl)
      __attribute__((always_inline)) {
#pragma unroll
        for (int nb = 0; nb < NB; ++nb) acc[nb] = __builtin_amdgcn_mfma_f32_16x16x32_f16(h[nb], bh, acc[nb], 0, 0, 0);
#pragma unroll
        for (int nb = 0; nb < NB; ++nb) acc[nb] = __builtin_amdgcn_mfma_f32_16x16x32_f16(l[nb], bh, acc[nb], 0, 0, 0);
#pragma unroll
        for (int nb = 0; nb < NB; ++nb) acc[nb] = __builtin_amdgcn_mfma_f32_16x16x32_f16(a2[nb], bl, acc[nb], 0, 0, 0);
      };

  auto pair_body = [&](auto KC) __attribute__((always_inline)) {
    constexpr int pr = decltype(KC)::value, BUF0 = (pr * S) % AD, SIDE = pr % RD;
    if constexpr (pr + RD - 1 < NP) load_res(pr + RD - 1, rres[(SIDE + RD - 1) % RD]);
    f32x4 bias[NB];
#pragma unroll
    for (int nb = 0; nb < NB; ++nb) {
      if constexpr (LDSW)
        bias[nb] = *reinterpret_cast<const f32x4*>(smem + kBias + (unsigned)(32 * pr + 8 * kgl + 4 * nb) * 4u);
      else
        bias[nb] = __builtin_bit_cast(f32x4, __builtin_amdgcn_raw_buffer_load_b128(r_bias, (unsigned)(32 * pr + 8 * kgl + 4 * nb) * 4u, 0, 0));
    }
    f32x4 acc[PB][NB];
#pragma unroll
    for (int i = 0; i < PB; ++i)
#pragma unroll
      for (int nb = 0; nb < NB; ++nb) acc[i][nb] = f32x4{0.f, 0.f, 0.f, 0.f};
    f16x8 yh[PB], yl[PB];
#pragma unroll
    for (int st = 0; st < S; ++st) {
      constexpr int dummy = 0;
      (void)dummy;
      const int buf = (BUF0 + st) % AD;
      {
        int npr = pr, nst = st + AD - 1;
        if (nst >= S) {
          nst -= S;
          npr = pr + 1 < NP ? pr + 1 : pr;
          if (pr + 1 >= NP) nst = S - 1;
        }
        load_a(npr, nst, ah[(buf + AD - 1) % AD], al[(buf + AD - 1) % AD]);
      }
      f16x8 a2[NB];
#pragma unroll
      for (int nb = 0; nb < NB; ++nb) a2[nb] = ah[buf][nb] * (_Float16)0x1p-11f;
      if (st < NCH) {
#pragma unroll
        for (int i = 0; i < PB; ++i) mfma3(acc[i], ah[buf], al[buf], a2, xh[i][st], xl[i][st]);
        if (st == NCH - 1) {
          const int cbase = 32 * pr + 8 * kgl;
#pragma unroll
          for (int i = 0; i < PB; ++i) {
#pragma unroll
            for (int nb = 0; nb < NB; ++nb)
#pragma unroll
              for (int q = 0; q < 4; ++q) acc[i][nb][q] = __builtin_fmaf(acc[i][nb][q], winv, bias[nb][q]);
            add_res_h2(acc[i], rres[SIDE][i]);
            if (p.relu) {
#pragma unroll
              for (int nb = 0; nb < NB; ++nb)
#pragma unroll
                for (int q = 0; q < 4; ++q) acc[i][nb][q] = acc[i][nb][q] > 0.f ? acc[i][nb][q] : 0.f;
            }
            h2_split8(acc[i][0], acc[i][1], yh[i], yl[i]);
            const unsigned ooff = ok[i] ? pix[i] * outpb + (unsigned)(p.out_coff + cbase) * ESZ : kOobOff;
            __builtin_amdgcn_raw_buffer_store_b128(__builtin_bit_cast(u32x4, yh[i]), r_out, ooff, 0, 0);
            __builtin_amdgcn_raw_buffer_store_b128(__builtin_bit_cast(u32x4, yl[i]), r_out, ooff + out_lo, 0, 0);
          }
        }
      } else {
#pragma unroll
        for (int i = 0; i < PB; ++i) mfma3(acc2[i][st - NCH], ah[buf], al[buf], a2, yh[i], yl[i]);
      }
    }
  };
  pair_body(std::integral_constant<int, 0>{});
  pair_body(std::integral_constant<int, 1>{});
  pair_body(std::integral_constant<int, 2>{});
  pair_body(std::integral_constant<int, 3>{});
  pair_body(std::integral_constant<int, 4>{});
  pair_body(std::integral_constant<int, 5>{});
  pair_body(std::integral_constant<int, 6>{});
  pair_body(std::integral_constant<int, 7>{});
#pragma unroll
  for (int q = 0; q < Q; ++q) {
    const int cbase = 32 * q + 8 * kgl;
    f32x4 b2[NB];
#pragma unroll
    for (int nb = 0; nb < NB; ++nb) {
      if constexpr (LDSW)
        b2[nb] = *reinterpret_cast<const f32x4*>(smem + kBias + 1024u + (unsigned)(cbase + 4 * nb) * 4u);
      else
        b2[nb] = __builtin_bit_cast(f32x4, __builtin_amdgcn_raw_buffer_load_b128(r_bias2, (unsigned)(cbase + 4 * nb) * 4u, 0, 0));
    }
#pragma unroll
    for (int i = 0; i < PB; ++i) {
      f32x4 v[NB];
#pragma unroll
      for (int nb = 0; nb < NB; ++nb)
#pragma unroll
        for (int k = 0; k < 4; ++k) {
          v[nb][k] = __builtin_fmaf(acc2[i][q][nb][k], winv2, b2[nb][k]);
          if (p.up_shift[2]) v[nb][k] = v[nb][k] > 0.f ? v[nb][k] : 0.f;
        }
      store_vec_buf<T, NB>(r_z, ok[i] ? pix[i] * zpb + (unsigned)cbase * ESZ : kOobOff, z_lo, v);
    }
  }
  }
}

int describe_conv_chain(ConvParams p, Launch* out) {
  const int cout2 = p.up_shift[0];
  if (p.Cin % 32 || (p.Cin != 64 && p.Cin != 128) || p.CoutPad != p.Cout || p.Cout != 256 || cout2 != 64 || p.nup ||
      p.nout2 || p.out_nchw_f32 || !p.out || !p.up[0] || !p.wgt2 || !p.bias2 || p.Hin != p.Hout || p.Win != p.Wout)
    return fail(UDP_ERR_UNSUPPORTED, "chained 1x1 convs: C%d -> %d -> %d (64 | 128 -> 256 -> 64, dense NHWC outputs)", p.Cin, p.Cout, cout2);
  static const int var = getenv("UDP_POSE_CHAIN_VAR") ? atoi(getenv("UDP_POSE_CHAIN_VAR")) : 0;
  constexpr int PB = 2;
  const long npix = (long)p.N * p.Hout * p.Wout;
  if (npix * (long)std::max(std::max(p.in_pitch, p.out_pitch), p.res_pitch) * 4 >= (1L << 31))
    return fail(UDP_ERR_UNSUPPORTED, "chained 1x1 convs: tensor beyond the 2 GiB buffer-descriptor range");
  const long groups = (npix + PB * 16 - 1) / (PB * 16);
  out->lds = 0;
  if (p.Cin == 64 && var == 0) {
    out->fn = reinterpret_cast<const void*>(&conv_chain_kernel<2, PB, 3, true>);
    out->lds = (2 * 8 + 8 * 2) * 4096 + 1280;
    out->grid = dim3((unsigned)std::min<long>(256, (groups + 7) / 8));
    out->block = dim3(512);
    UDP_HIP_CHECK(hipFuncSetAttribute(out->fn, hipFuncAttributeMaxDynamicSharedMemorySize, (int)out->lds));
  } else {
    out->fn = p.Cin == 64 ? reinterpret_cast<const void*>(&conv_chain_kernel<2, PB, 3, false>) : reinterpret_cast<const void*>(&conv_chain_kernel<4, PB, 2, false>);
    out->grid = dim3((unsigned)((groups + 3) / 4));
    out->block = dim3(256);
  }
  out->groupable = 0;
  out->p = p;
  out->p.sbuf = getenv("UDP_POSE_CHAIN_DBG") ? atoi(getenv("UDP_POSE_CHAIN_DBG")) : 0;
  return UDP_OK;
}

int conv_ws_h2_overflow(hipStream_t s, int reset, int* flag) { return h2_overflow_fetch(s, reset, flag); }

}
```

udp-pose_amd/csrc/decode.hip:

```cpp
#include "common.h"

namespace udp {

constexpr int kMaxTaps = 15;

struct Taps {
  float k[kMaxTaps];
  int ksize;
};

__device__ __forceinline__ int reflect101(int i, int n) {
  if (n == 1) return 0;
  while (i < 0 || i >= n) {
    if (i < 0) i = -i;
    if (i >= n) i = 2 * (n - 1) - i;
  }
  return i;
}

__device__ void blur_pass(const float* __restrict__ src, float* __restrict__ dst, int h, int w,
                          const Taps& t, int axis) {
  const int r = (t.ksize - 1) / 2;
  for (int i = threadIdx.x; i < h * w; i += blockDim.x) {
    const int y = i / w, x = i - y * w;
    float acc = t.k[r] * src[i];
    for (int d = 1; d <= r; ++d) {
      float a, b;
      if (axis == 1) {
        a = src[y * w + reflect101(x - d, w)];
        b = src[y * w + reflect101(x + d, w)];
      } else {
        a = src[reflect101(y - d, h) * w + x];
        b = src[reflect101(y + d, h) * w + x];
      }
      const float pair = a + b;
      acc = acc + t.k[r + d] * pair;
    }
    dst[i] = acc;
  }
}

struct MaxMin {
  float mx;
  int idx;
  float mn;
};

__device__ MaxMin block_argmax_min(const float* __restrict__ a, int count, float* red_v, int* red_i,
                                   float* red_m) {
  float bv = -INFINITY, bm = INFINITY;
  int bi = 0x7fffffff;
  for (int i = threadIdx.x; i < count; i += blockDim.x) {
    const float v = a[i];
    if (v > bv) {
      bv = v;
      bi = i;
    }
    bm = v < bm ? v : bm;
  }
  for (int off = 32; off > 0; off >>= 1) {
    const float ov = __shfl_down(bv, off);
    const int oi = __shfl_down(bi, off);
    const float om = __shfl_down(bm, off);
    if (ov > bv || (ov == bv && oi < bi)) {
      bv = ov;
      bi = oi;
    }
    bm = om < bm ? om : bm;
  }
  const int wave = threadIdx.x >> 6, lane = threadIdx.x & 63;
  __syncthreads();
  if (lane == 0) {
    red_v[wave] = bv;
    red_i[wave] = bi;
    red_m[wave] = bm;
  }
  __syncthreads();
  MaxMin r;
  r.mx = red_v[0];
  r.idx = red_i[0];
  r.mn = red_m[0];
  const int nw = blockDim.x >> 6;
  for (int k = 1; k < nw; ++k) {
    if (red_v[k] > r.mx || (red_v[k] == r.mx && red_i[k] < r.idx)) {
      r.mx = red_v[k];
      r.idx = red_i[k];
    }
    r.mn = red_m[k] < r.mn ? red_m[k] : r.mn;
  }
  if (r.idx == 0x7fffffff) r.idx = 0;
  return r;
}

__device__ void write_preds(double cx, double cy, bool f32_coords, const double* center,
                            const double* scale, int cs_is_f32, int h, int w, double* preds,
                            double* preds_in) {
  const double wm1 = (double)w - 1.0, hm1 = (double)h - 1.0;
  if (f32_coords) {
    const float fx = (float)cx, fy = (float)cy;
    preds_in[0] = (double)(fx / (float)wm1 * (float)(4.0 * w - 1.0));
    preds_in[1] = (double)(fy / (float)hm1 * (float)(4.0 * h - 1.0));
    if (cs_is_f32) {
      const float s0 = (float)scale[0] * 200.0f, s1 = (float)scale[1] * 200.0f;
      const float sx = s0 / (float)wm1, sy = s1 / (float)hm1;
      const float px = fx * sx + (float)center[0] - s0 * 0.5f;
      const float py = fy * sy + (float)center[1] - s1 * 0.5f;
      preds[0] = (double)px;
      preds[1] = (double)py;
    } else {
      const double s0 = scale[0] * 200.0, s1 = scale[1] * 200.0;
      const double sx = s0 / wm1, sy = s1 / hm1;
      preds[0] = (double)(float)((double)fx * sx + center[0] - s0 * 0.5);
      preds[1] = (double)(float)((double)fy * sy + center[1] - s1 * 0.5);
    }
  } else {
    preds_in[0] = cx / wm1 * (4.0 * w - 1.0);
    preds_in[1] = cy / hm1 * (4.0 * h - 1.0);
    if (cs_is_f32) {
      const float s0 = (float)scale[0] * 200.0f, s1 = (float)scale[1] * 200.0f;
      const float sx = s0 / (float)wm1, sy = s1 / (float)hm1;
      const float h0 = s0 * 0.5f, h1 = s1 * 0.5f;
      preds[0] = cx * (double)sx + (double)(float)center[0] - (double)h0;
      preds[1] = cy * (double)sy + (double)(float)center[1] - (double)h1;
    } else {
      const double s0 = scale[0] * 200.0, s1 = scale[1] * 200.0;
      preds[0] = cx * (s0 / wm1) + center[0] - s0 * 0.5;
      preds[1] = cy * (s1 / hm1) + center[1] - s1 * 0.5;
    }
  }
}

__global__ __launch_bounds__(256) void decode_gaussian_kernel(
    const float* __restrict__ hm, int j, int h, int w, const double* __restrict__ center,
    const double* __restrict__ scale, int cs_is_f32, int post, Taps t7, double* __restrict__ preds,
    float* __restrict__ maxvals, double* __restrict__ preds_in, int* __restrict__ argidx) {
  extern __shared__ float sm[];
  __shared__ float red_v[4], red_m[4];
  __shared__ int red_i[4];
  const int hw = h * w;
  float* raw = sm;
  float* tmp = sm + hw;
  float* blr = sm + 2 * hw;
  const int map = blockIdx.x;
  const int n = map / j;
  const float* src = hm + (size_t)map * hw;
  for (int i = threadIdx.x; i < hw; i += blockDim.x) raw[i] = src[i];
  __syncthreads();
  const MaxMin mm = block_argmax_min(raw, hw, red_v, red_i, red_m);
  const float maxori = mm.mx;
  const bool keep = maxori > 0.0f;
  const int px = keep ? mm.idx % w : 0;
  const int py = keep ? mm.idx / w : 0;
  if (threadIdx.x == 0) {
    maxvals[map] = maxori;
    if (argidx) argidx[map] = mm.idx;
  }
  if (!post) {
    if (threadIdx.x == 0)
      write_preds((double)px, (double)py, true, center + 2 * n, scale + 2 * n, cs_is_f32, h, w,
                  preds + 2 * map, preds_in + 2 * map);
    return;
  }
  blur_pass(raw, tmp, h, w, t7, 1);
  __syncthreads();
  blur_pass(tmp, blr, h, w, t7, 0);
  __syncthreads();
  const MaxMin bm = block_argmax_min(blr, hw, red_v, red_i, red_m);
  if (threadIdx.x == 0) {
    const float mx = bm.mx, mn = bm.mn;
    const float range = mx - mn;
    double s[3][3];
    for (int dy = -1; dy <= 1; ++dy)
      for (int dx = -1; dx <= 1; ++dx) {
        int yy = py + dy, xx = px + dx;
        yy = yy < 0 ? 0 : (yy >= h ? h - 1 : yy);
        xx = xx < 0 ? 0 : (xx >= w ? w - 1 : xx);
        const float rs = (blr[yy * w + xx] - mn) / range * maxori;
        s[dy + 1][dx + 1] = (rs == rs) ? (double)(float)log((double)fminf(fmaxf(rs, 0.001f), 50.0f)) : (double)NAN;
      }
    const double I = s[1][1], Ix1 = s[1][2], Ix1_ = s[1][0], Iy1 = s[2][1], Iy1_ = s[0][1];
    const double Ix1y1 = s[2][2], Ix1_y1_ = s[0][0];
    const double dx = 0.5 * (Ix1 - Ix1_), dy = 0.5 * (Iy1 - Iy1_);
    const double dxx = Ix1 - 2 * I + Ix1_, dyy = Iy1 - 2 * I + Iy1_;
    const double dxy = 0.5 * (Ix1y1 - Ix1 - Iy1 + I + I - Ix1_ - Iy1_ + Ix1_y1_);
    const double det = dxx * dyy - dxy * dxy;
    double sx = 0.0, sy = 0.0;
    if (det != 0.0) {
      const double inv = 1.0 / det;
      sx = inv * (dyy * dx - dxy * dy);
      sy = inv * (dxx * dy - dxy * dx);
    }
    const double cx = (double)px - sx, cy = (double)py - sy;
    write_preds(cx, cy, false, center + 2 * n, scale + 2 * n, cs_is_f32, h, w, preds + 2 * map,
                preds_in + 2 * map);
  }
}

__global__ __launch_bounds__(256) void decode_offset_kernel(
    const float* __restrict__ out, int j, int h, int w, const double* __restrict__ center,
    const double* __restrict__ scale, int cs_is_f32, float kpd, Taps t15, Taps t7,
    double* __restrict__ preds, float* __restrict__ maxvals, double* __restrict__ preds_in,
    int* __restrict__ argidx) {
  extern __shared__ float sm[];
  __shared__ float red_v[4], red_m[4];
  __shared__ int red_i[4];
  __shared__ float off_s[2];
  const int hw = h * w;
  float* raw = sm;
  float* tmp = sm + hw;
  float* blr = sm + 2 * hw;
  const int map = blockIdx.x;
  const int n = map / j;
  const float* src = out + (size_t)map * 3 * hw;
  for (int i = threadIdx.x; i < hw; i += blockDim.x) raw[i] = src[i];
  __syncthreads();
  blur_pass(raw, tmp, h, w, t15, 1);
  __syncthreads();
  blur_pass(tmp, blr, h, w, t15, 0);
  __syncthreads();
  const MaxMin mm = block_argmax_min(blr, hw, red_v, red_i, red_m);
  const bool keep = mm.mx > 0.0f;
  const int px = keep ? mm.idx % w : 0;
  const int py = keep ? mm.idx / w : 0;
  if (threadIdx.x < 2) {
    const float* o = src + (size_t)(1 + threadIdx.x) * hw;
    float rowv[7];
    for (int dy = -3; dy <= 3; ++dy) {
      const int yy = reflect101(py + dy, h);
      float acc = t7.k[3] * (o[yy * w + px] * kpd);
      for (int d = 1; d <= 3; ++d) {
        const float a = o[yy * w + reflect101(px - d, w)] * kpd;
        const float b = o[yy * w + reflect101(px + d, w)] * kpd;
        const float pair = a + b;
        acc = acc + t7.k[3 + d] * pair;
      }
      rowv[dy + 3] = acc;
    }
    float acc = t7.k[3] * rowv[3];
    for (int d = 1; d <= 3; ++d) {
      const float pair = rowv[3 - d] + rowv[3 + d];
      acc = acc + t7.k[3 + d] * pair;
    }
    off_s[threadIdx.x] = acc;
  }
  __syncthreads();
  if (threadIdx.x == 0) {
    maxvals[map] = mm.mx;
    if (argidx) argidx[map] = mm.idx;
    const float cx = (float)px + off_s[0];
    const float cy = (float)py + off_s[1];
    write_preds((double)cx, (double)cy, true, center + 2 * n, scale + 2 * n, cs_is_f32, h, w,
                preds + 2 * map, preds_in + 2 * map);
  }
}

__global__ __launch_bounds__(256) void flip_fuse_kernel(const float* __restrict__ a,
                                                        const float* __restrict__ b,
                                                        const int* __restrict__ src_ch,
                                                        const float* __restrict__ sign, int c, int h,
                                                        int w, long total, float divisor,
                                                        float* __restrict__ out) {
  for (long i = (long)blockIdx.x * 256 + threadIdx.x; i < total; i += (long)gridDim.x * 256) {
    const int x = i % w;
    long t = i / w;
    const int y = t % h;
    t /= h;
    const int ch = t % c;
    const long n = t / c;
    const float fb = b[((n * c + src_ch[ch]) * h + y) * w + (w - 1 - x)] * sign[ch];
    out[i] = (a[i] + fb) * 0.5f / divisor;
  }
}

}

using namespace udp;

extern "C" int udp_gaussian_taps_host(int ksize, float* taps) {
  if (!taps || ksize < 1 || ksize > kMaxTaps || (ksize & 1) == 0)
    return fail(UDP_ERR_ARG, "udp_gaussian_taps_host: ksize=%d (odd, 1..%d)", ksize, kMaxTaps);
  static const double t1[] = {1.0}, t3[] = {0.25, 0.5, 0.25}, t5[] = {0.0625, 0.25, 0.375, 0.25, 0.0625},
                      t7[] = {0.03125, 0.109375, 0.21875, 0.28125, 0.21875, 0.109375, 0.03125};
  const double* fixed = ksize == 1 ? t1 : ksize == 3 ? t3 : ksize == 5 ? t5 : ksize == 7 ? t7 : nullptr;
  const double sigma = 0.3 * ((ksize - 1) * 0.5 - 1.0) + 0.8;
  const double scale2x = -0.5 / (sigma * sigma);
  double sum = 0.0;
  for (int i = 0; i < ksize; ++i) {
    const double x = i - (ksize - 1) * 0.5;
    const double t = fixed ? fixed[i] : exp(scale2x * x * x);
    taps[i] = (float)t;
    sum += (double)taps[i];
  }
  const double inv = 1.0 / sum;
  for (int i = 0; i < ksize; ++i) taps[i] = (float)((double)taps[i] * inv);
  return UDP_OK;
}

static int make_taps(int ksize, Taps* t) {
  memset(t, 0, sizeof(*t));
  t->ksize = ksize;
  return udp_gaussian_taps_host(ksize, t->k);
}

static int check_decode_args(const char* who, const void* hm, int n, int j, int h, int w, const void* c,
                             const void* s, const void* preds, const void* maxvals, const void* pin) {
  if (!hm || !c || !s || !preds || !maxvals || !pin) return fail(UDP_ERR_ARG, "%s: null pointer", who);
  if (n < 0 || j <= 0 || h <= 0 || w <= 0) return fail(UDP_ERR_ARG, "%s: bad shape n=%d j=%d h=%d w=%d", who, n, j, h, w);
  if ((size_t)h * w * 3 * sizeof(float) > 150 * 1024)
    return fail(UDP_ERR_UNSUPPORTED, "%s: map %dx%d does not fit the LDS working set", who, h, w);
  return UDP_OK;
}

extern "C" int udp_decode_gaussian(const float* heatmaps, int n, int j, int h, int w, const double* center,
                                   const double* scale, int cs_is_f32, int post_process, double* preds,
                                   float* maxvals, double* preds_in, int32_t* argidx, void* stream) {
  int rc = check_decode_args("udp_decode_gaussian", heatmaps, n, j, h, w, center, scale, preds, maxvals, preds_in);
  if (rc) return rc;
  if (n == 0) return UDP_OK;
  Taps t7;
  make_taps(7, &t7);
  const size_t lds = (size_t)h * w * 3 * sizeof(float);
  static bool attr = false;
  if (!attr) {
    UDP_HIP_CHECK(hipFuncSetAttribute(reinterpret_cast<const void*>(decode_gaussian_kernel),
                                      hipFuncAttributeMaxDynamicSharedMemorySize, 150 * 1024));
    attr = true;
  }
  hipLaunchKernelGGL(decode_gaussian_kernel, dim3(n * j), dim3(256), lds, (hipStream_t)stream, heatmaps, j, h,
                     w, center, scale, cs_is_f32, post_process, t7, preds, maxvals, preds_in, argidx);
  UDP_HIP_CHECK(hipGetLastError());
  return UDP_OK;
}

extern "C" int udp_decode_offset(const float* heatmaps, int n, int j, int h, int w, const double* center,
                                 const double* scale, int cs_is_f32, float kpd, double* preds, float* maxvals,
                                 double* preds_in, int32_t* argidx, void* stream) {
  int rc = check_decode_args("udp_decode_offset", heatmaps, n, j, h, w, center, scale, preds, maxvals, preds_in);
  if (rc) return rc;
  if (n == 0) return UDP_OK;
  Taps t15, t7;
  make_taps(15, &t15);
  make_taps(7, &t7);
  const size_t lds = (size_t)h * w * 3 * sizeof(float);
  static bool attr = false;
  if (!attr) {
    UDP_HIP_CHECK(hipFuncSetAttribute(reinterpret_cast<const void*>(decode_offset_kernel),
                                      hipFuncAttributeMaxDynamicSharedMemorySize, 150 * 1024));
    attr = true;
  }
  hipLaunchKernelGGL(decode_offset_kernel, dim3(n * j), dim3(256), lds, (hipStream_t)stream, heatmaps, j, h, w,
                     center, scale, cs_is_f32, kpd, t15, t7, preds, maxvals, preds_in, argidx);
  UDP_HIP_CHECK(hipGetLastError());
  return UDP_OK;
}

extern "C" int udp_flip_fuse_scaled(const float* a, const float* b, const int32_t* src_ch, const float* sign, int n,
                                    int c, int h, int w, float divisor, float* out, void* stream) {
  if (!a || !b || !src_ch || !sign || !out) return fail(UDP_ERR_ARG, "udp_flip_fuse: null pointer");
  if (n < 0 || c <= 0 || h <= 0 || w <= 0 || !(divisor > 0.f)) return fail(UDP_ERR_ARG, "udp_flip_fuse: bad shape / divisor");
  const long total = (long)n * c * h * w;
  if (total == 0) return UDP_OK;
  long blocks = (total + 255) / 256;
  if (blocks > 4096) blocks = 4096;
  hipLaunchKernelGGL(flip_fuse_kernel, dim3((unsigned)blocks), dim3(256), 0, (hipStream_t)stream, a, b, src_ch,
                     sign, c, h, w, total, divisor, out);
  UDP_HIP_CHECK(hipGetLastError());
  return UDP_OK;
}

extern "C" int udp_flip_fuse(const float* a, const float* b, const int32_t* src_ch, const float* sign, int n,
                             int c, int h, int w, float* out, void* stream) {
  return udp_flip_fuse_scaled(a, b, src_ch, sign, n, c, h, w, 1.0f, out, stream);
}
```

udp-pose_amd/csrc/hrnet.hip:

```cpp
#include <cstdlib>
#include <vector>

#include "common.h"

namespace udp {
int describe_conv(ConvParams p, int dtype, int ks, int stride, Launch* out);
int describe_stem(const ConvParams& p, int dtype, Launch* out);
int describe_fuse(const ConvParams& p, int dtype, Launch* out);
int describe_stem7(const ConvParams& p, int dtype, Launch* out);
int describe_maxpool(const ConvParams& p, int dtype, Launch* out);
int describe_bilinear(const ConvParams& p, int dtype, Launch* out);
int describe_psa(const ConvParams& p, int dtype, int kind, Launch* out);
int describe_block(ConvParams p, int dtype, Launch* out);
int describe_conv_grouped(ConvParams p, int dtype, int ks, int stride, Launch* out);
int describe_multi(const Launch* members, int n, ConvMulti* m, Launch* out);
int run_launch(const Launch& l, hipStream_t s);
}

using namespace udp;

struct GraphEntry {
  int n, flip;
  const void* in;
  void* ws;
  void* out;
  hipGraph_t graph;
  hipGraphExec_t exec;
};

struct udp_hrnet {
  std::vector<udp_conv_op> ops;
  std::vector<int64_t> buf_elems;
  std::vector<int64_t> buf_off;
  int64_t total_elems = 0;
  const char* weights = nullptr;
  size_t weights_bytes = 0;
  int dtype = UDP_F32;
  int in_h = 0, in_w = 0, out_channels = 0;
  double flops = 0.0;
  std::vector<GraphEntry> graphs;
  int n_lanes = 1;
  hipStream_t lane_stream[UDP_MAX_LANES] = {nullptr, nullptr, nullptr, nullptr};
  std::vector<hipEvent_t> op_done;
  std::vector<char> op_signals;
  hipEvent_t ev_fork = nullptr, ev_join[UDP_MAX_LANES] = {nullptr, nullptr, nullptr, nullptr};
  hipStream_t split_stream = nullptr;
  hipEvent_t split_fork = nullptr, split_join = nullptr;
};

static size_t esize(int dtype) { return dtype == UDP_BF16 ? 2 : 4; }

static int act_validate(const udp_conv_op& o, int dtype, bool has_res) {
  if (o.relu < UDP_ACT_NONE || o.relu > UDP_ACT_SILU || o.relu == 3)
    return fail(UDP_ERR_ARG, "activation code %d (0 none, 1 ReLU, 2 hard-swish, 4 SiLU)", o.relu);
  if (o.relu < UDP_ACT_HSWISH || o.kind == UDP_OP_ACT) return UDP_OK;
  if (o.relu == UDP_ACT_SILU && o.kind == UDP_OP_DWCONV) return UDP_OK;
  const bool plain1x1 = o.kind == UDP_OP_CONV && o.ks == 1 && o.stride == 1 && !o.group && !o.chain_cout && !o.n_up && !o.n_out2 && !has_res &&
                        !o.in_stuff2 && o.out_buf != UDP_BUF_OUTPUT;
  if (dtype == UDP_BF16 || (o.kind != UDP_OP_STEM && !plain1x1))
    return fail(UDP_ERR_UNSUPPORTED, "%s: UDP_OP_STEM and 1x1 stride-1 NHWC UDP_OP_CONV without addends, second outputs, "
                "chain or group, in f32 / f16x2 only (kind %d, ks %d, stride %d)",
                o.relu == UDP_ACT_SILU ? "SiLU (activation code 4; also UDP_OP_DWCONV)" : "hard-swish (activation code 2)", o.kind, o.ks, o.stride);
  return UDP_OK;
}

static int validate_op(const udp_hrnet* h, const udp_conv_op& o, int idx) {
  const int nb = (int)h->buf_elems.size();
  auto buf_ok = [&](int b, int64_t need) { return b >= 0 && b < nb && h->buf_elems[b] >= need; };
  const int64_t out_need = (int64_t)o.hout * o.wout * (o.out_pitch ? o.out_pitch : o.cout);
  if (o.kind < UDP_OP_STEM || o.kind > UDP_OP_ACT) return fail(UDP_ERR_ARG, "op %d: bad kind %d", idx, o.kind);
  if (const int rc = act_validate(o, h->dtype, o.res_buf != UDP_BUF_NONE)) return rc;
  if (o.lane < 0 || o.lane >= UDP_MAX_LANES || o.n_wait < 0 || o.n_wait > UDP_MAX_WAIT) return fail(UDP_ERR_ARG, "op %d: lane/n_wait", idx);
  for (int k = 0; k < o.n_wait; ++k)
    if (o.wait_op[k] < 0 || o.wait_op[k] >= idx) return fail(UDP_ERR_ARG, "op %d: wait_op %d must name an earlier op", idx, o.wait_op[k]);
  if (o.kind == UDP_OP_BLOCK) {
    const int64_t hw = (int64_t)o.hin * o.win;
    if (h->dtype != UDP_BF16 || o.cin != 32 || o.cout != 32 || o.hin != o.hout || o.win != o.wout || o.hin % 8)
      return fail(UDP_ERR_ARG, "op %d: fused BasicBlock needs bf16, 32 channels, height %% 8 == 0", idx);
    if (!buf_ok(o.in_buf, hw * 32) || !buf_ok(o.out_buf, hw * 32) || o.in_buf == o.out_buf)
      return fail(UDP_ERR_ARG, "op %d: fused BasicBlock buffers", idx);
    const size_t wbytes = (size_t)9 * 32 * 32 * 2;
    const int64_t offs[4] = {o.w_off, o.w2_off, o.b_off, o.b2_off};
    for (int k = 0; k < 4; ++k)
      if (offs[k] < 0 || (size_t)offs[k] + (k < 2 ? wbytes : 32 * 4) > h->weights_bytes || (offs[k] & 15))
        return fail(UDP_ERR_ARG, "op %d: fused BasicBlock weight/bias range outside the blob or misaligned", idx);
    return UDP_OK;
  }
  if (o.kind == UDP_OP_DECONV) {
    const int ipitch = o.in_pitch ? o.in_pitch : o.cin, opitch = o.out_pitch ? o.out_pitch : o.cout;
    const bool h2 = h->dtype == UDP_F16X2;
    if (h->dtype == UDP_BF16) return fail(UDP_ERR_UNSUPPORTED, "op %d: deconv: storage modes f32 and f16x2 only", idx);
    if (o.ks != 4 || o.stride != 2 || o.hin <= 0 || o.win <= 0 || o.hout != 2 * o.hin || o.wout != 2 * o.win || o.cin <= 0 ||
        o.cin % (h2 ? 32 : 16) || o.cout <= 0 || o.cout % 8 || o.cout_pad < o.cout || o.cout_pad % 32)
      return fail(UDP_ERR_ARG, "op %d: deconv must be k4 s2 p1, %dx%d -> 2x, cin %% %d == 0, cout %% 8 == 0", idx, o.hin, o.win, h2 ? 32 : 16);
    if (o.wfmt != (h2 ? 1 : 0)) return fail(UDP_ERR_ARG, "op %d: deconv weights: wfmt %d (f16x2: 1, f32: 0)", idx, o.wfmt);
    if (o.res_buf != UDP_BUF_NONE || o.n_up || o.n_out2 || o.chain_cout || o.group || o.in_stuff2)
      return fail(UDP_ERR_UNSUPPORTED, "op %d: deconv takes no addends, second outputs, chains or groups", idx);
    if (o.in_coff < 0 || o.out_coff < 0 || o.in_coff + o.cin > ipitch || o.out_coff + o.cout > opitch || (o.in_coff | ipitch | o.out_coff | opitch) % 8)
      return fail(UDP_ERR_ARG, "op %d: deconv channel views", idx);
    if (!buf_ok(o.in_buf, (int64_t)o.hin * o.win * ipitch) || !buf_ok(o.out_buf, out_need) || o.in_buf == o.out_buf)
      return fail(UDP_ERR_ARG, "op %d: deconv buffers missing, too small or aliased", idx);
    const size_t wbytes = h2 ? (size_t)16 * (o.cin / 32) * (o.cout_pad / 32) * 4096 : (size_t)16 * o.cout_pad * o.cin * 4;
    if (o.w_off < 0 || (size_t)o.w_off + wbytes > h->weights_bytes || (o.w_off & 15) || o.b_off < 0 ||
        (size_t)o.b_off + (size_t)o.cout_pad * 4 > h->weights_bytes || (o.b_off & 15) || o.wexp < -40 || o.wexp > 40)
      return fail(UDP_ERR_ARG, "op %d: deconv weight / bias range outside the blob or misaligned", idx);
    return UDP_OK;
  }
  if (o.kind == UDP_OP_SE) {
    const int rc = se_validate(o, h->dtype);
    if (rc) return rc;
    const int ipitch = o.in_pitch ? o.in_pitch : o.cin;
    if (!buf_ok(o.in_buf, (int64_t)o.hin * o.win * ipitch) || !buf_ok(o.out_buf, out_need) || o.res_buf != UDP_BUF_NONE)
      return fail(UDP_ERR_ARG, "op %d: squeeze-excitation buffers missing or too small (or a residual)", idx);
    if (o.in_buf == o.out_buf && (o.in_coff != o.out_coff || ipitch != (o.out_pitch ? o.out_pitch : o.cout)))
      return fail(UDP_ERR_ARG, "op %d: squeeze-excitation in place needs the same view for in and out", idx);
    const size_t wbytes = ((size_t)2 * o.cin * o.chain_cout + o.chain_cout) * 4;
    if (o.w_off < 0 || (size_t)o.w_off + wbytes > h->weights_bytes || (o.w_off & 15))
      return fail(UDP_ERR_ARG, "op %d: squeeze-excitation parameter block outside the blob or misaligned", idx);
    return UDP_OK;
  }
  if (o.kind == UDP_OP_GNORM || o.kind == UDP_OP_LINATTN) {
    const bool gn = o.kind == UDP_OP_GNORM;
    const int rc = gn ? gnorm_validate(o, h->dtype) : linattn_validate(o, h->dtype);
    if (rc) return rc;
    const int ipitch = o.in_pitch ? o.in_pitch : o.cin;
    if (!buf_ok(o.in_buf, (int64_t)o.hin * o.win * ipitch) || !buf_ok(o.out_buf, out_need) || o.res_buf != UDP_BUF_NONE)
      return fail(UDP_ERR_ARG, "op %d: %s buffers missing or too small (or a residual)", idx, gn ? "group norm" : "linear attention");
    if (o.in_buf == o.out_buf && (!gn || o.in_coff != o.out_coff || ipitch != (o.out_pitch ? o.out_pitch : o.cout)))
      return fail(UDP_ERR_ARG, "op %d: %s", idx, gn ? "group norm in place needs the same view for in and out" : "linear attention: out must not be in");
    if (gn && (o.w_off < 0 || (size_t)o.w_off + (size_t)2 * o.cin * 4 > h->weights_bytes || (o.w_off & 15)))
      return fail(UDP_ERR_ARG, "op %d: group norm parameter block outside the blob or misaligned", idx);
    return UDP_OK;
  }
  if (o.kind == UDP_OP_LNORM || o.kind == UDP_OP_MHATTN || o.kind == UDP_OP_ACT) {
    const char* what = o.kind == UDP_OP_LNORM ? "layer norm" : o.kind == UDP_OP_MHATTN ? "multi-head attention" : "activation op";
    const int rc = o.kind == UDP_OP_LNORM ? lnorm_validate(o, h->dtype) : o.kind == UDP_OP_MHATTN ? mhattn_validate(o, h->dtype) : act_op_validate(o, h->dtype);
    if (rc) return rc;
    const int ipitch = o.in_pitch ? o.in_pitch : o.cin;
    if (!buf_ok(o.in_buf, (int64_t)o.hin * o.win * ipitch) || !buf_ok(o.out_buf, out_need) || o.res_buf != UDP_BUF_NONE)
      return fail(UDP_ERR_ARG, "op %d: %s buffers missing or too small (or a residual)", idx, what);
    if (o.in_buf == o.out_buf && (o.kind == UDP_OP_MHATTN || o.in_coff != o.out_coff || ipitch != (o.out_pitch ? o.out_pitch : o.cout)))
      return fail(UDP_ERR_ARG, "op %d: %s: %s", idx, what, o.kind == UDP_OP_MHATTN ? "out must not be in" : "in place needs the same view for in and out");
    if (o.kind == UDP_OP_LNORM && (o.w_off < 0 || (size_t)o.w_off + (size_t)2 * o.cin * 4 > h->weights_bytes || (o.w_off & 15)))
      return fail(UDP_ERR_ARG, "op %d: layer norm parameter block outside the blob or misaligned", idx);
    return UDP_OK;
  }
  if (o.kind == UDP_OP_DWCONV || o.kind == UDP_OP_PIXSHUF) {
    const bool dw = o.kind == UDP_OP_DWCONV;
    const int rc = dw ? dwconv_validate(o, h->dtype) : pixshuf_validate(o, h->dtype);
    if (rc) return rc;
    const int ipitch = o.in_pitch ? o.in_pitch : o.cin;
    if (!buf_ok(o.in_buf, (int64_t)o.hin * o.win * ipitch) || !buf_ok(o.out_buf, out_need) || o.in_buf == o.out_buf)
      return fail(UDP_ERR_ARG, "op %d: %s buffers missing, too small or aliased", idx, dw ? "depthwise conv" : "pixel shuffle");
    if (dw && o.n_out2) {
      const int64_t hw = (int64_t)o.hout * o.wout;
      const int d = o.out2_buf[0];
      if (!buf_ok(o.res_buf, hw * o.res_pitch) || !buf_ok(d, hw * o.out2_pitch[0]) || d == o.in_buf || d == o.out_buf || d == o.res_buf)
        return fail(UDP_ERR_ARG, "op %d: depthwise conv: passthrough buffers missing, too small or aliased", idx);
    } else if (o.res_buf != UDP_BUF_NONE) {
      return fail(UDP_ERR_UNSUPPORTED, "op %d: %s takes no residual", idx, dw ? "depthwise conv" : "pixel shuffle");
    }
    if (dw && (o.w_off < 0 || (size_t)o.w_off + (size_t)o.ks * o.ks * o.cin * 4 > h->weights_bytes || (o.w_off & 15) || o.b_off < 0 ||
               (size_t)o.b_off + (size_t)o.cin * 4 > h->weights_bytes || (o.b_off & 15)))
      return fail(UDP_ERR_ARG, "op %d: depthwise conv weight / bias range outside the blob or misaligned", idx);
    return UDP_OK;
  }
  if (o.kind >= UDP_OP_PSA_POOL) {
    const int64_t f = 4 / (int64_t)esize(h->dtype);
    const int64_t hw = (int64_t)o.hin * o.win;
    const int C = o.kind == UDP_OP_PSA_SP ? o.cout : o.cin;
    if (C <= 0 || hw <= 0 || C % 16) return fail(UDP_ERR_ARG, "op %d: PSA shape", idx);
    const size_t wbytes = (size_t)(C + (C / 2) * C + (C / 8) * (C / 2) + 3 * (C / 8) + C * (C / 8) + C + (C / 2) * C) * 4;
    bool ok = true;
    switch (o.kind) {
      case UDP_OP_PSA_POOL: ok = buf_ok(o.in_buf, hw * C) && buf_ok(o.out_buf, 2 * C * f); break;
      case UDP_OP_PSA_MLP: ok = buf_ok(o.in_buf, 2 * C * f) && buf_ok(o.out_buf, (C + C / 2) * f); break;
      case UDP_OP_PSA_SCALE: ok = buf_ok(o.in_buf, hw * C) && buf_ok(o.res_buf, (C + C / 2) * f) && buf_ok(o.out_buf, hw * C); break;
      default: ok = buf_ok(o.in_buf, hw * (C / 2)) && buf_ok(o.res_buf, hw * C) && o.n_up == 1 && buf_ok(o.up_buf[0], (C + C / 2) * f) && buf_ok(o.out_buf, hw * C);
    }
    if (!ok) return fail(UDP_ERR_ARG, "op %d: PSA buffers missing or too small", idx);
    if (o.kind <= UDP_OP_PSA_MLP && (o.w_off < 0 || (size_t)o.w_off + wbytes > h->weights_bytes || (o.w_off & 15)))
      return fail(UDP_ERR_ARG, "op %d: PSA parameter block outside the blob or misaligned", idx);
    return UDP_OK;
  }
  const bool is_stem = o.kind == UDP_OP_STEM || o.kind == UDP_OP_STEM7;
  const bool has_w = is_stem || o.kind == UDP_OP_CONV;
  const int ipitch = o.in_pitch ? o.in_pitch : o.cin, opitch = o.out_pitch ? o.out_pitch : o.cout;
  const int rpitch = o.res_pitch ? o.res_pitch : o.cout;
  if (o.in_coff < 0 || o.out_coff < 0 || o.res_coff < 0 || o.in_coff + o.cin > ipitch || o.out_coff + o.cout > opitch ||
      o.res_coff + o.cout > rpitch)
    return fail(UDP_ERR_ARG, "op %d: channel view outside its tensor", idx);
  if (o.cout <= 0 || o.hout <= 0 || o.wout <= 0 || o.cout_pad < o.cout || o.cout_pad % 32)
    return fail(UDP_ERR_ARG, "op %d: bad output shape / cout_pad", idx);
  if (o.out_buf == UDP_BUF_OUTPUT) {
    if (o.kind != UDP_OP_CONV || o.cout != h->out_channels || o.hout * 4 != h->in_h || o.wout * 4 != h->in_w)
      return fail(UDP_ERR_ARG, "op %d: output op must be a conv producing [C=%d,%d,%d]", idx, h->out_channels,
                  h->in_h / 4, h->in_w / 4);
    if (o.res_buf != UDP_BUF_NONE || o.n_up != 0) return fail(UDP_ERR_ARG, "op %d: output op takes no addends", idx);
  } else if (o.out_buf == UDP_BUF_NONE && o.n_out2 > 0 && o.kind == UDP_OP_CONV) {
  } else if (!buf_ok(o.out_buf, out_need)) {
    return fail(UDP_ERR_ARG, "op %d: out_buf %d missing or too small", idx, o.out_buf);
  }
  if (is_stem) {
    const int want = o.kind == UDP_OP_STEM ? 3 : 7;
    if (o.ks != want || o.stride != 2 || o.cin != 3 || o.hin != h->in_h || o.win != h->in_w)
      return fail(UDP_ERR_ARG, "op %d: stem must be %dx%d s2 on the %dx%d input", idx, want, want, h->in_h, h->in_w);
  } else {
    if (!buf_ok(o.in_buf, (int64_t)o.hin * o.win * ipitch)) return fail(UDP_ERR_ARG, "op %d: in_buf %d missing or too small", idx, o.in_buf);
    if (o.in_buf == o.out_buf && o.kind == UDP_OP_CONV && o.ks != 1) return fail(UDP_ERR_ARG, "op %d: in-place 3x3 conv is not supported", idx);
  }
  if (o.kind == UDP_OP_MAXPOOL) {
    if (o.cin != o.cout || o.hout != (o.hin + 2 - 3) / 2 + 1 || o.wout != (o.win + 2 - 3) / 2 + 1)
      return fail(UDP_ERR_ARG, "op %d: maxpool 3x3 s2 p1 shape", idx);
  } else if (o.kind == UDP_OP_BILINEAR) {
    if (o.cin != o.cout) return fail(UDP_ERR_ARG, "op %d: bilinear resize keeps the channel count", idx);
  } else if (has_w) {
    if ((o.ks != 1 && o.ks != 3 && o.ks != 7) || (o.stride != 1 && o.stride != 2)) return fail(UDP_ERR_ARG, "op %d: ks/stride", idx);
    const int pad = o.ks / 2;
    if (o.hout != (o.hin + 2 * pad - o.ks) / o.stride + 1 || o.wout != (o.win + 2 * pad - o.ks) / o.stride + 1)
      return fail(UDP_ERR_ARG, "op %d: output size does not match input/stride", idx);
    if (o.wfmt != 0 && (o.wfmt != 1 || is_stem || h->dtype != UDP_F16X2))
      return fail(UDP_ERR_ARG, "op %d: wfmt %d (fragment-major weights need a UDP_F16X2 UDP_OP_CONV)", idx, o.wfmt);
    const size_t wbytes = is_stem ? (size_t)o.ks * o.ks * 3 * o.cout * 4
                          : o.wfmt == 1 ? (size_t)o.ks * o.ks * ((o.cin + 31) / 32) * (o.cout_pad / 32) * 4096
                                        : (size_t)o.ks * o.ks * o.cout_pad * o.cin * esize(h->dtype);
    if (o.w_off < 0 || (size_t)o.w_off + wbytes > h->weights_bytes || (o.w_off & 15))
      return fail(UDP_ERR_ARG, "op %d: weight range outside the blob or misaligned", idx);
    if (o.b_off < 0 || (size_t)o.b_off + (size_t)o.cout_pad * 4 > h->weights_bytes || (o.b_off & 15))
      return fail(UDP_ERR_ARG, "op %d: bias range outside the blob or misaligned", idx);
  } else if (o.hin != o.hout || o.win != o.wout || o.cin != o.cout) {
    return fail(UDP_ERR_ARG, "op %d: fuse op must keep the shape", idx);
  }
  if (o.lane < 0 || o.lane >= UDP_MAX_LANES || o.n_wait < 0 || o.n_wait > UDP_MAX_WAIT) return fail(UDP_ERR_ARG, "op %d: lane/n_wait", idx);
  for (int k = 0; k < o.n_wait; ++k)
    if (o.wait_op[k] < 0 || o.wait_op[k] >= idx) return fail(UDP_ERR_ARG, "op %d: wait_op %d must name an earlier op", idx, o.wait_op[k]);
  if (o.res_buf != UDP_BUF_NONE && !buf_ok(o.res_buf, (int64_t)o.hout * o.wout * rpitch)) return fail(UDP_ERR_ARG, "op %d: res_buf", idx);
  if (o.n_up < 0 || o.n_up > 3) return fail(UDP_ERR_ARG, "op %d: n_up", idx);
  for (int u = 0; u < o.n_up; ++u) {
    const int s = o.up_shift[u];
    if (s < 1 || s > 5 || (o.hout & ((1 << s) - 1)) || (o.wout & ((1 << s) - 1)))
      return fail(UDP_ERR_ARG, "op %d: up_shift %d does not divide %dx%d", idx, s, o.hout, o.wout);
    if (!buf_ok(o.up_buf[u], (int64_t)(o.hout >> s) * (o.wout >> s) * o.cout)) return fail(UDP_ERR_ARG, "op %d: up_buf %d", idx, u);
  }
  if (o.chain_cout) {
    if (o.kind != UDP_OP_CONV || o.wfmt != 1 || h->dtype != UDP_F16X2 || o.ks != 1 || o.stride != 1 || o.group || o.n_up || o.n_out2 ||
        o.out_buf < 0 || (o.cin != 64 && o.cin != 128) || o.cout != 256 || o.cout_pad != o.cout || o.chain_cout != 64)
      return fail(UDP_ERR_UNSUPPORTED, "op %d: a chained conv needs an ungrouped split-fp16 1x1 conv (wfmt 1), 64 | 128 -> 256 channels, and 64 chained outputs", idx);
    if (!buf_ok(o.chain_buf, (int64_t)o.hout * o.wout * o.chain_cout) || o.chain_buf == o.out_buf || o.chain_buf == o.in_buf || o.chain_buf == o.res_buf)
      return fail(UDP_ERR_ARG, "op %d: chain_buf %d missing, too small or aliased", idx, o.chain_buf);
    const size_t w2bytes = (size_t)(o.cout / 32) * (o.chain_cout / 32) * 4096;
    if (o.w2_off < 0 || (size_t)o.w2_off + w2bytes > h->weights_bytes || (o.w2_off & 15) || o.b2_off < 0 ||
        (size_t)o.b2_off + (size_t)o.chain_cout * 4 > h->weights_bytes || (o.b2_off & 15) || o.chain_wexp < -40 || o.chain_wexp > 40)
      return fail(UDP_ERR_ARG, "op %d: chained conv: weight / bias range outside the blob or misaligned", idx);
  }
  if (o.n_out2 < 0 || o.n_out2 > 2) return fail(UDP_ERR_ARG, "op %d: n_out2", idx);
  if (o.n_out2 && (o.kind != UDP_OP_CONV || o.wfmt != 1 || h->dtype != UDP_F16X2 || o.out_buf == UDP_BUF_OUTPUT || o.cout % 8 || o.ks != 3 || o.stride != 1 || o.group))
    return fail(UDP_ERR_UNSUPPORTED, "op %d: second outputs need an ungrouped 3x3 stride-1 split-fp16 conv with fragment-major weights, an NHWC output and cout %% 8 == 0", idx);
  for (int k = 0; k < o.n_out2; ++k) {
    const int op = o.out2_pitch[k] ? o.out2_pitch[k] : o.cout, ap = o.add2_pitch[k] ? o.add2_pitch[k] : o.cout;
    if (o.out2_coff[k] < 0 || o.out2_coff[k] + o.cout > op || o.add2_coff[k] < 0 || o.add2_coff[k] + o.cout > ap ||
        (o.out2_coff[k] | o.add2_coff[k] | op | ap) % 8)
      return fail(UDP_ERR_ARG, "op %d: second output %d: channel views", idx, k);
    if (!buf_ok(o.out2_buf[k], (int64_t)o.hout * o.wout * op) || !buf_ok(o.add2_buf[k], (int64_t)o.hout * o.wout * ap))
      return fail(UDP_ERR_ARG, "op %d: second output %d: buffers", idx, k);
  }
  return UDP_OK;
}

extern "C" int udp_abi_version(void) { return UDP_POSE_ABI_VERSION; }
extern "C" const char* udp_last_error(void) { return err_buf(); }

extern "C" int udp_f16x2_overflow(void* stream, int reset) {
  hipStream_t s = reinterpret_cast<hipStream_t>(stream);
  int flag = 0;
  int rc = conv_h2_overflow(s, reset, &flag);
  if (!rc) rc = conv_ws_h2_overflow(s, reset, &flag);
  if (!rc) rc = psa_h2_overflow(s, reset, &flag);
  if (!rc) rc = deconv_h2_overflow(s, reset, &flag);
  if (!rc) rc = dwconv_h2_overflow(s, reset, &flag);
  if (!rc) rc = attn_h2_overflow(s, reset, &flag);
  return rc ? rc : flag;
}

extern "C" int udp_hrnet_create(const udp_conv_op* ops, int n_ops, const int64_t* buf_elems, int n_bufs,
                                const void* weights_dev, size_t weights_bytes, int dtype, int in_h, int in_w,
                                int out_channels, udp_hrnet** out) {
  if (!ops || n_ops <= 0 || !buf_elems || n_bufs <= 0 || !weights_dev || !out)
    return fail(UDP_ERR_ARG, "udp_hrnet_create: null/empty argument");
  if (dtype != UDP_F32 && dtype != UDP_BF16 && dtype != UDP_F16X2) return fail(UDP_ERR_ARG, "udp_hrnet_create: dtype %d", dtype);
  if (in_h <= 0 || in_w <= 0 || (in_h % 32) || (in_w % 32))
    return fail(UDP_ERR_UNSUPPORTED, "udp_hrnet_create: input %dx%d must be a multiple of 32", in_h, in_w);
  if (reinterpret_cast<uintptr_t>(weights_dev) & 15) return fail(UDP_ERR_ARG, "udp_hrnet_create: weights not 16-byte aligned");
  udp_hrnet* h = new udp_hrnet();
  h->dtype = dtype;
  h->in_h = in_h;
  h->in_w = in_w;
  h->out_channels = out_channels;
  h->weights = reinterpret_cast<const char*>(weights_dev);
  h->weights_bytes = weights_bytes;
  h->buf_off.resize(n_bufs);
  for (int b = 0; b < n_bufs; ++b) {
    if (buf_elems[b] <= 0) {
      delete h;
      return fail(UDP_ERR_ARG, "udp_hrnet_create: buffer %d has %lld elements", b, (long long)buf_elems[b]);
    }
    const int64_t e = (buf_elems[b] + 63) / 64 * 64;
    h->buf_elems.push_back(e);
    h->buf_off[b] = h->total_elems;
    h->total_elems += e;
  }
  bool has_out = false;
  for (int i = 0; i < n_ops; ++i) {
    const int rc = validate_op(h, ops[i], i);
    if (rc) {
      delete h;
      return rc;
    }
    has_out |= ops[i].out_buf == UDP_BUF_OUTPUT;
    if (ops[i].kind == UDP_OP_STEM || ops[i].kind == UDP_OP_STEM7 || ops[i].kind == UDP_OP_CONV)
      h->flops += 2.0 * ops[i].ks * ops[i].ks * ops[i].cin * ops[i].cout * ops[i].hout * ops[i].wout;
    if (ops[i].kind == UDP_OP_BLOCK) h->flops += 2 * 2.0 * 9 * 32 * 32 * ops[i].hout * ops[i].wout;
    if (ops[i].kind == UDP_OP_DECONV) h->flops += 2.0 * 4 * ops[i].cin * ops[i].cout * ops[i].hout * ops[i].wout;
    if (ops[i].kind == UDP_OP_DWCONV) h->flops += 2.0 * ops[i].ks * ops[i].ks * ops[i].cout * ops[i].hout * ops[i].wout;
    if (ops[i].kind == UDP_OP_SE) h->flops += 2.0 * 2 * ops[i].cin * ops[i].chain_cout;
    if (ops[i].kind == UDP_OP_LINATTN) h->flops += 2.0 * ops[i].cout * ops[i].hout * ops[i].wout;
    if (ops[i].kind == UDP_OP_MHATTN)
      h->flops += 2.0 * 2 * ops[i].chain_cout * (ops[i].hout * ops[i].wout / 4) * ops[i].hout * ops[i].wout;
    if (ops[i].kind == UDP_OP_CONV && ops[i].chain_cout) h->flops += 2.0 * ops[i].cout * ops[i].chain_cout * ops[i].hout * ops[i].wout;
    h->ops.push_back(ops[i]);
  }
  if (!has_out || (h->ops[0].kind != UDP_OP_STEM && h->ops[0].kind != UDP_OP_STEM7) || h->ops[0].lane != 0 || h->ops.back().lane != 0 ||
      h->ops.back().out_buf != UDP_BUF_OUTPUT) {
    delete h;
    return fail(UDP_ERR_ARG, "udp_hrnet_create: program needs a stem op first and the output op last, both on lane 0");
  }
  h->op_signals.assign(n_ops, 0);
  for (int i = 0; i < n_ops; ++i) {
    if (ops[i].lane + 1 > h->n_lanes) h->n_lanes = ops[i].lane + 1;
    for (int k = 0; k < ops[i].n_wait; ++k) h->op_signals[ops[i].wait_op[k]] = 1;
  }
  h->op_done.assign(n_ops, nullptr);
  hipError_t e = hipSuccess;
  for (int l = 1; l < h->n_lanes && e == hipSuccess; ++l) e = hipStreamCreateWithFlags(&h->lane_stream[l], hipStreamNonBlocking);
  for (int l = 1; l < h->n_lanes && e == hipSuccess; ++l) e = hipEventCreateWithFlags(&h->ev_join[l], hipEventDisableTiming);
  if (e == hipSuccess) e = hipEventCreateWithFlags(&h->ev_fork, hipEventDisableTiming);
  for (int i = 0; i < n_ops && e == hipSuccess; ++i)
    if (h->op_signals[i]) e = hipEventCreateWithFlags(&h->op_done[i], hipEventDisableTiming);
  if (e != hipSuccess) {
    udp_hrnet_destroy(h);
    return fail(UDP_ERR_HIP, "udp_hrnet_create: stream/event creation failed: %s", hipGetErrorString(e));
  }
  *out = h;
  return UDP_OK;
}

static size_t ws_bytes_one(const udp_hrnet* h, int n, int flip) {
  const size_t b = (size_t)h->total_elems * (size_t)(n * (flip ? 2 : 1)) * esize(h->dtype);
  return (b + 255) & ~(size_t)255;
}
static size_t out_bytes(const udp_hrnet* h, int images) {
  return (size_t)images * h->out_channels * (size_t)(h->in_h / 4) * (size_t)(h->in_w / 4) * sizeof(float);
}
static bool split_ok(const udp_hrnet* h, int n) {
  if (n < 16) return false;
  const char* e = getenv("UDP_POSE_LANES");
  if (e) return atoi(e) >= 2;
  return h->dtype != UDP_F32 && (long)h->in_h * h->in_w <= 256L * 192L;
}
extern "C" int udp_hrnet_lanes(const udp_hrnet* h, int n) { return h && n > 0 && split_ok(h, n) ? 2 : 1; }
extern "C" size_t udp_hrnet_workspace_bytes(const udp_hrnet* h, int n, int flip_test) {
  if (!h || n <= 0) return 0;
  if (!split_ok(h, n)) return ws_bytes_one(h, n, flip_test);
  const int n0 = (n + 1) / 2;
  return ws_bytes_one(h, n0, flip_test) + ws_bytes_one(h, n - n0, flip_test) + (flip_test ? out_bytes(h, 2 * n) + 512 : 0);
}

extern "C" int udp_hrnet_num_launches(const udp_hrnet* h) { return h ? (int)h->ops.size() : 0; }
extern "C" double udp_hrnet_flops_per_image(const udp_hrnet* h) { return h ? h->flops : 0.0; }

static int describe_all(const udp_hrnet* h, const float* in, int n, int flip, char* ws, float* out,
                        std::vector<Launch>& ls) {
  const int B = n * (flip ? 2 : 1);
  const size_t es = esize(h->dtype);
  auto buf = [&](int b) -> char* { return ws + (size_t)h->buf_off[b] * B * es; };
  ls.resize(h->ops.size());
  for (size_t i = 0; i < h->ops.size(); ++i) {
    const udp_conv_op& o = h->ops[i];
    ConvParams p;
    memset(&p, 0, sizeof(p));
    p.N = B;
    p.Hin = o.hin;
    p.Win = o.win;
    p.Cin = o.cin;
    p.Hout = o.hout;
    p.Wout = o.wout;
    p.Cout = o.cout;
    p.CoutPad = o.cout_pad;
    p.relu = o.relu;
    p.wfmt = o.wfmt;
    p.wexp = o.wexp;
    p.flip_from = flip ? n : B;
    const bool is_stem = o.kind == UDP_OP_STEM || o.kind == UDP_OP_STEM7;
    p.in_pitch = o.in_pitch ? o.in_pitch : o.cin;
    p.in_coff = o.in_coff;
    p.out_pitch = o.out_pitch ? o.out_pitch : o.cout;
    p.out_coff = o.out_coff;
    p.res_pitch = o.res_pitch ? o.res_pitch : o.cout;
    p.res_coff = o.res_coff;
    p.in = is_stem ? reinterpret_cast<const void*>(in) : buf(o.in_buf);
    p.out_nchw_f32 = o.out_buf == UDP_BUF_OUTPUT;
    p.out = p.out_nchw_f32 ? reinterpret_cast<void*>(out) : o.out_buf == UDP_BUF_NONE ? nullptr : buf(o.out_buf);
    p.res = o.res_buf == UDP_BUF_NONE ? nullptr : buf(o.res_buf);
    p.nup = o.n_up;
    for (int u = 0; u < o.n_up; ++u) {
      p.up[u] = buf(o.up_buf[u]);
      p.up_shift[u] = o.up_shift[u];
    }
    p.nout2 = o.n_out2;
    for (int k = 0; k < o.n_out2; ++k) {
      p.out2[k] = buf(o.out2_buf[k]);
      p.add2[k] = o.kind == UDP_OP_DWCONV ? nullptr : buf(o.add2_buf[k]);
      p.out2_coff[k] = o.out2_coff[k];
      p.out2_pitch[k] = o.out2_pitch[k] ? o.out2_pitch[k] : o.cout;
      p.add2_coff[k] = o.add2_coff[k];
      p.add2_pitch[k] = o.add2_pitch[k] ? o.add2_pitch[k] : o.cout;
    }
    if (is_stem || o.kind == UDP_OP_CONV || o.kind == UDP_OP_DECONV || o.kind == UDP_OP_DWCONV) {
      p.wgt = h->weights + o.w_off;
      p.bias = reinterpret_cast<const float*>(h->weights + o.b_off);
    }
    if (o.kind == UDP_OP_CONV && o.chain_cout) {
      p.wgt2 = h->weights + o.w2_off;
      p.bias2 = reinterpret_cast<const float*>(h->weights + o.b2_off);
      p.up[0] = buf(o.chain_buf);
      p.up_shift[0] = o.chain_cout;
      p.up_shift[1] = o.chain_wexp;
      p.up_shift[2] = o.chain_relu;
    }
    if (o.kind == UDP_OP_DWCONV) p.up_shift[0] = o.chain_cout;
    if (o.kind == UDP_OP_SE || o.kind == UDP_OP_GNORM || o.kind == UDP_OP_LNORM) {
      p.wgt = h->weights + o.w_off;
      p.up_shift[0] = o.chain_cout;
    }
    if (o.kind == UDP_OP_MHATTN) {
      p.up_shift[0] = o.chain_cout;
      p.up_shift[1] = o.up_shift[0];
    }
    if (o.kind == UDP_OP_BLOCK) {
      p.wgt = h->weights + o.w_off;
      p.bias = reinterpret_cast<const float*>(h->weights + o.b_off);
      p.wgt2 = h->weights + o.w2_off;
      p.bias2 = reinterpret_cast<const float*>(h->weights + o.b2_off);
    } else if (o.kind >= UDP_OP_PSA_POOL) {
      p.wgt = h->weights + o.w_off;
      if (o.kind == UDP_OP_PSA_SCALE) p.res_pitch = o.cin + o.cin / 2;
    }
    int rc;
    switch (o.kind) {
      case UDP_OP_PSA_POOL:
      case UDP_OP_PSA_MLP:
      case UDP_OP_PSA_SCALE:
      case UDP_OP_PSA_SP: rc = describe_psa(p, h->dtype, o.kind, &ls[i]); break;
      case UDP_OP_BLOCK: rc = describe_block(p, h->dtype, &ls[i]); break;
      case UDP_OP_STEM: rc = describe_stem(p, h->dtype, &ls[i]); break;
      case UDP_OP_STEM7: rc = describe_stem7(p, h->dtype, &ls[i]); break;
      case UDP_OP_FUSE: rc = describe_fuse(p, h->dtype, &ls[i]); break;
      case UDP_OP_MAXPOOL: rc = describe_maxpool(p, h->dtype, &ls[i]); break;
      case UDP_OP_BILINEAR: rc = describe_bilinear(p, h->dtype, &ls[i]); break;
      case UDP_OP_DECONV: rc = describe_deconv(p, h->dtype, &ls[i]); break;
      case UDP_OP_DWCONV: rc = describe_dwconv(p, h->dtype, o.ks, o.stride, &ls[i]); break;
      case UDP_OP_SE: rc = describe_se(p, h->dtype, &ls[i]); break;
      case UDP_OP_GNORM: rc = describe_gnorm(p, h->dtype, &ls[i]); break;
      case UDP_OP_LINATTN: rc = describe_linattn(p, h->dtype, &ls[i]); break;
      case UDP_OP_LNORM: rc = describe_lnorm(p, h->dtype, &ls[i]); break;
      case UDP_OP_MHATTN: rc = describe_mhattn(p, h->dtype, &ls[i]); break;
      case UDP_OP_ACT: rc = describe_act(p, h->dtype, &ls[i]); break;
      case UDP_OP_PIXSHUF: rc = describe_pixshuf(p, h->dtype, &ls[i]); break;
      default:
        if (o.chain_cout) {
          rc = describe_conv_chain(p, &ls[i]);
          break;
        }
        rc = o.group != 0 && getenv("UDP_POSE_NO_GROUPS") == nullptr ? describe_conv_grouped(p, h->dtype, o.ks, o.stride, &ls[i]) : 1;
        if (rc == 1) rc = describe_conv(p, h->dtype, o.ks, o.stride, &ls[i]);
    }
    if (rc) return rc;
  }
  return UDP_OK;
}

struct Node {
  size_t first;
  int n;
};
static std::vector<Node> make_nodes(const udp_hrnet* h, const std::vector<Launch>& L, bool* grouped) {
  std::vector<Node> nodes;
  *grouped = false;
  for (size_t i = 0; i < L.size();) {
    int n = 1;
    if (L[i].groupable && h->ops[i].group != 0)
      while (n < 4 && i + n < L.size() && L[i + n].groupable / 10 == L[i].groupable / 10 && h->ops[i + n].group == h->ops[i].group) ++n;
    nodes.push_back({i, n});
    *grouped |= n > 1;
    i += n;
  }
  return nodes;
}
static int run_node(const std::vector<Launch>& L, const Node& nd, hipStream_t s) {
  if (nd.n == 1) return run_launch(L[nd.first], s);
  ConvMulti m;
  Launch ml;
  const int rc = describe_multi(&L[nd.first], nd.n, &m, &ml);
  if (rc) return rc;
  void* args[] = {&m};
  UDP_HIP_CHECK(hipLaunchKernel(ml.fn, ml.grid, ml.block, args, ml.lds, s));
  return UDP_OK;
}

static int enqueue_all(udp_hrnet* h, const std::vector<Launch>& L, hipStream_t s, hipEvent_t* ev, int lanes) {
  bool grouped = false;
  const std::vector<Node> nodes = make_nodes(h, L, &grouped);
  if (grouped) {
    for (const Node& nd : nodes) {
      if (ev) UDP_HIP_CHECK(hipEventRecord(ev[2 * nd.first], s));
      const int rc = run_node(L, nd, s);
      if (rc) return rc;
      if (ev) UDP_HIP_CHECK(hipEventRecord(ev[2 * nd.first + 1], s));
    }
    return UDP_OK;
  }
  lanes = lanes && h->n_lanes > 1 && !ev && getenv("UDP_POSE_SERIAL") == nullptr;
  hipStream_t ls[UDP_MAX_LANES] = {s, s, s, s};
  if (lanes) {
    UDP_HIP_CHECK(hipEventRecord(h->ev_fork, s));
    for (int l = 1; l < h->n_lanes; ++l) {
      ls[l] = h->lane_stream[l];
      UDP_HIP_CHECK(hipStreamWaitEvent(ls[l], h->ev_fork, 0));
    }
  }
  for (size_t i = 0; i < h->ops.size(); ++i) {
    const udp_conv_op& o = h->ops[i];
    hipStream_t os = ls[o.lane];
    if (lanes)
      for (int k = 0; k < o.n_wait; ++k)
        if (h->ops[o.wait_op[k]].lane != o.lane) UDP_HIP_CHECK(hipStreamWaitEvent(os, h->op_done[o.wait_op[k]], 0));
    if (ev) UDP_HIP_CHECK(hipEventRecord(ev[2 * i], os));
    const int rc = run_launch(L[i], os);
    if (rc) return rc;
    if (ev) UDP_HIP_CHECK(hipEventRecord(ev[2 * i + 1], os));
    if (lanes && h->op_signals[i]) UDP_HIP_CHECK(hipEventRecord(h->op_done[i], os));
  }
  if (lanes)
    for (int l = 1; l < h->n_lanes; ++l) {
      UDP_HIP_CHECK(hipEventRecord(h->ev_join[l], ls[l]));
      UDP_HIP_CHECK(hipStreamWaitEvent(s, h->ev_join[l], 0));
    }
  return UDP_OK;
}

static int build_graph(udp_hrnet* h, const std::vector<Launch>& L, hipGraph_t* graph, hipGraphExec_t* exec) {
  UDP_HIP_CHECK(hipGraphCreate(graph, 0));
  bool grouped = false;
  const std::vector<Node> nodes = make_nodes(h, L, &grouped);
  std::vector<hipGraphNode_t> node(nodes.size());
  std::vector<int> node_of_op(L.size(), -1);
  int last_on_lane[UDP_MAX_LANES] = {-1, -1, -1, -1};
  const bool serial = grouped || getenv("UDP_POSE_SERIAL") != nullptr;
  for (size_t k = 0; k < nodes.size(); ++k) {
    const size_t i = nodes[k].first;
    const udp_conv_op& o = h->ops[i];
    std::vector<hipGraphNode_t> deps;
    if (serial) {
      if (k) deps.push_back(node[k - 1]);
    } else {
      if (last_on_lane[o.lane] >= 0) deps.push_back(node[last_on_lane[o.lane]]);
      for (int w = 0; w < o.n_wait; ++w) deps.push_back(node[node_of_op[o.wait_op[w]]]);
    }
    ConvParams p = L[i].p;
    ConvMulti m;
    Launch ml = L[i];
    void* args[1] = {&p};
    if (nodes[k].n > 1) {
      const int rc = describe_multi(&L[i], nodes[k].n, &m, &ml);
      if (rc) {
        (void)hipGraphDestroy(*graph);
        return rc;
      }
      args[0] = &m;
    }
    hipKernelNodeParams kp;
    memset(&kp, 0, sizeof(kp));
    kp.func = const_cast<void*>(ml.fn);
    kp.gridDim = ml.grid;
    kp.blockDim = ml.block;
    kp.sharedMemBytes = ml.lds;
    kp.kernelParams = args;
    kp.extra = nullptr;
    hipError_t e = hipGraphAddKernelNode(&node[k], *graph, deps.data(), deps.size(), &kp);
    if (e != hipSuccess) {
      (void)hipGraphDestroy(*graph);
      return fail(UDP_ERR_HIP, "hipGraphAddKernelNode(op %zu): %s", i, hipGetErrorString(e));
    }
    for (int j = 0; j < nodes[k].n; ++j) node_of_op[i + j] = (int)k;
    last_on_lane[o.lane] = (int)k;
  }
  hipError_t e = hipGraphInstantiate(exec, *graph, nullptr, nullptr, 0);
  if (e != hipSuccess) {
    (void)hipGraphDestroy(*graph);
    return fail(UDP_ERR_HIP, "hipGraphInstantiate: %s", hipGetErrorString(e));
  }
  return UDP_OK;
}

static int check_forward_args(const char* who, const udp_hrnet* h, const float* in, int n, int flip, const void* ws,
                              size_t ws_bytes, const float* out) {
  if (!h || !in || !ws || !out) return fail(UDP_ERR_ARG, "%s: null pointer", who);
  if (n <= 0) return fail(UDP_ERR_ARG, "%s: n=%d (the reference engine also requires n >= 1)", who, n);
  if (ws_bytes < udp_hrnet_workspace_bytes(h, n, flip))
    return fail(UDP_ERR_WORKSPACE, "%s: workspace %zu < %zu bytes", who, ws_bytes, udp_hrnet_workspace_bytes(h, n, flip));
  if (reinterpret_cast<uintptr_t>(ws) & 255) return fail(UDP_ERR_ARG, "%s: workspace not 256-byte aligned", who);
  return UDP_OK;
}

extern "C" int udp_hrnet_profile(udp_hrnet* h, const float* in_nchw, int n, int flip_test, void* workspace,
                                 size_t workspace_bytes, float* heatmaps_nchw, float* ms_per_op, void* stream) {
  int rc = check_forward_args("udp_hrnet_profile", h, in_nchw, n, flip_test, workspace, workspace_bytes, heatmaps_nchw);
  if (rc) return rc;
  if (!ms_per_op) return fail(UDP_ERR_ARG, "udp_hrnet_profile: null pointer");
  hipStream_t s = reinterpret_cast<hipStream_t>(stream);
  std::vector<Launch> L;
  rc = describe_all(h, in_nchw, n, flip_test ? 1 : 0, reinterpret_cast<char*>(workspace), heatmaps_nchw, L);
  if (rc) return rc;
  const size_t nops = h->ops.size();
  std::vector<hipEvent_t> ev(2 * nops, nullptr);
  for (auto& e : ev) {
    const hipError_t ce = hipEventCreate(&e);
    if (ce != hipSuccess) {
      for (auto& d : ev)
        if (d) (void)hipEventDestroy(d);
      return fail(UDP_ERR_HIP, "hipEventCreate: %s", hipGetErrorString(ce));
    }
  }
  rc = enqueue_all(h, L, s, ev.data(), 0);
  hipError_t se = hipStreamSynchronize(s);
  if (!rc && se == hipSuccess) {
    bool grouped = false;
    for (const Node& nd : make_nodes(h, L, &grouped)) {
      float t = -1.f;
      if (hipEventElapsedTime(&t, ev[2 * nd.first], ev[2 * nd.first + 1]) != hipSuccess) t = -1.f;
      double total = 0.0;
      auto flops = [&](size_t i) { const udp_conv_op& o = h->ops[i]; return (double)o.ks * o.ks * o.cin * o.cout * o.hout * o.wout; };
      for (int j = 0; j < nd.n; ++j) total += flops(nd.first + j);
      for (int j = 0; j < nd.n; ++j) ms_per_op[nd.first + j] = nd.n == 1 || t < 0 ? t : (float)(t * flops(nd.first + j) / total);
    }
  }
  for (auto& e : ev) (void)hipEventDestroy(e);
  if (rc) return rc;
  if (se != hipSuccess) return fail(UDP_ERR_HIP, "hipStreamSynchronize: %s", hipGetErrorString(se));
  return UDP_OK;
}

static int forward_one(udp_hrnet* h, const float* in_nchw, int n, int flip_test, void* workspace, float* heatmaps_nchw,
                       int use_graph, hipStream_t s) {
  int rc;
  if (use_graph)
    for (size_t k = 0; k < h->graphs.size(); ++k) {
      const GraphEntry g = h->graphs[k];
      if (g.n == n && g.flip == flip_test && g.in == in_nchw && g.ws == workspace && g.out == heatmaps_nchw) {
        if (k + 1 != h->graphs.size()) {
          h->graphs.erase(h->graphs.begin() + k);
          h->graphs.push_back(g);
        }
        UDP_HIP_CHECK(hipGraphLaunch(g.exec, s));
        return UDP_OK;
      }
    }
  std::vector<Launch> L;
  rc = describe_all(h, in_nchw, n, flip_test, reinterpret_cast<char*>(workspace), heatmaps_nchw, L);
  if (rc) return rc;
  if (!use_graph) return enqueue_all(h, L, s, nullptr, 1);
  GraphEntry e;
  e.n = n;
  e.flip = flip_test;
  e.in = in_nchw;
  e.ws = workspace;
  e.out = heatmaps_nchw;
  rc = build_graph(h, L, &e.graph, &e.exec);
  if (rc) return rc;
  if (h->graphs.size() >= 8) {
    UDP_HIP_CHECK(hipDeviceSynchronize());
    (void)hipGraphExecDestroy(h->graphs[0].exec);
    (void)hipGraphDestroy(h->graphs[0].graph);
    h->graphs.erase(h->graphs.begin());
  }
  h->graphs.push_back(e);
  UDP_HIP_CHECK(hipGraphLaunch(e.exec, s));
  return UDP_OK;
}

extern "C" int udp_hrnet_forward(udp_hrnet* h, const float* in_nchw, int n, int flip_test, void* workspace,
                                 size_t workspace_bytes, float* heatmaps_nchw, int use_graph, void* stream) {
  int rc = check_forward_args("udp_hrnet_forward", h, in_nchw, n, flip_test, workspace, workspace_bytes, heatmaps_nchw);
  if (rc) return rc;
  hipStream_t s = reinterpret_cast<hipStream_t>(stream);
  flip_test = flip_test ? 1 : 0;
  if (!use_graph || !split_ok(h, n)) return forward_one(h, in_nchw, n, flip_test, workspace, heatmaps_nchw, use_graph, s);
  if (!h->split_stream) {
    UDP_HIP_CHECK(hipStreamCreateWithFlags(&h->split_stream, hipStreamNonBlocking));
    UDP_HIP_CHECK(hipEventCreateWithFlags(&h->split_fork, hipEventDisableTiming));
    UDP_HIP_CHECK(hipEventCreateWithFlags(&h->split_join, hipEventDisableTiming));
  }
  const int n0 = (n + 1) / 2, n1 = n - n0;
  struct FillHint {
    FillHint() { ws_set_fill_wgs(128); }
    ~FillHint() { ws_set_fill_wgs(512); }
  } fill_hint;
  char* ws0 = reinterpret_cast<char*>(workspace);
  char* ws1 = ws0 + ws_bytes_one(h, n0, flip_test);
  const size_t img_in = (size_t)3 * h->in_h * h->in_w;
  const size_t img_out = out_bytes(h, 1) / sizeof(float);
  hipStream_t s2 = h->split_stream;
  UDP_HIP_CHECK(hipEventRecord(h->split_fork, s));
  UDP_HIP_CHECK(hipStreamWaitEvent(s2, h->split_fork, 0));
  if (!flip_test) {
    rc = forward_one(h, in_nchw, n0, 0, ws0, heatmaps_nchw, 1, s);
    if (!rc) rc = forward_one(h, in_nchw + n0 * img_in, n1, 0, ws1, heatmaps_nchw + n0 * img_out, 1, s2);
  } else {
    float* t0 = reinterpret_cast<float*>(ws1 + ws_bytes_one(h, n1, 1));
    float* t1 = t0 + 2 * n0 * img_out;
    rc = forward_one(h, in_nchw, n0, 1, ws0, t0, 1, s);
    if (!rc) {
      UDP_HIP_CHECK(hipMemcpyAsync(heatmaps_nchw, t0, n0 * img_out * sizeof(float), hipMemcpyDeviceToDevice, s));
      UDP_HIP_CHECK(hipMemcpyAsync(heatmaps_nchw + n * img_out, t0 + n0 * img_out, n0 * img_out * sizeof(float), hipMemcpyDeviceToDevice, s));
      rc = forward_one(h, in_nchw + n0 * img_in, n1, 1, ws1, t1, 1, s2);
    }
    if (!rc) {
      UDP_HIP_CHECK(hipMemcpyAsync(heatmaps_nchw + n0 * img_out, t1, n1 * img_out * sizeof(float), hipMemcpyDeviceToDevice, s2));
      UDP_HIP_CHECK(hipMemcpyAsync(heatmaps_nchw + (n + n0) * img_out, t1 + n1 * img_out, n1 * img_out * sizeof(float), hipMemcpyDeviceToDevice, s2));
    }
  }
  UDP_HIP_CHECK(hipEventRecord(h->split_join, s2));
  UDP_HIP_CHECK(hipStreamWaitEvent(s, h->split_join, 0));
  return rc;
}

extern "C" int udp_hrnet_destroy(udp_hrnet* h) {
  if (!h) return UDP_OK;
  if (h->split_stream) {
    (void)hipStreamSynchronize(h->split_stream);
    (void)hipStreamDestroy(h->split_stream);
    (void)hipEventDestroy(h->split_fork);
    (void)hipEventDestroy(h->split_join);
  }
  for (auto& g : h->graphs) {
    (void)hipGraphExecDestroy(g.exec);
    (void)hipGraphDestroy(g.graph);
  }
  for (int l = 1; l < UDP_MAX_LANES; ++l) {
    if (h->lane_stream[l]) (void)hipStreamDestroy(h->lane_stream[l]);
    if (h->ev_join[l]) (void)hipEventDestroy(h->ev_join[l]);
  }
  if (h->ev_fork) (void)hipEventDestroy(h->ev_fork);
  for (auto e : h->op_done)
    if (e) (void)hipEventDestroy(e);
  delete h;
  return UDP_OK;
}

static int conv2d_fused_impl(const udp_conv_op* o, int dtype, int n, const void* in, const void* weights,
                             const float* bias, const void* res, const void* up0, const void* up1,
                             const void* up2, void* out, double* bn_ws, size_t bn_ws_doubles, int* bn_rows, void* stream);

extern "C" int udp_conv2d_fused(const udp_conv_op* o, int dtype, int n, const void* in, const void* weights,
                                const float* bias, const void* res, const void* up0, const void* up1,
                                const void* up2, void* out, void* stream) {
  return conv2d_fused_impl(o, dtype, n, in, weights, bias, res, up0, up1, up2, out, nullptr, 0, nullptr, stream);
}

extern "C" int udp_conv2d_fused_bn(const udp_conv_op* o, int dtype, int n, const void* in, const void* weights,
                                   const float* bias, void* out, double* bn_ws, size_t bn_ws_doubles, int* bn_rows,
                                   void* stream) {
  if (!bn_ws || !bn_rows) return fail(UDP_ERR_ARG, "udp_conv2d_fused_bn: null pointer");
  if (dtype == UDP_F16X2 || !o || o->kind != UDP_OP_CONV || o->out_buf == UDP_BUF_OUTPUT || o->n_up || o->relu ||
      (o->out_pitch && o->out_pitch != o->cout) || o->out_coff)
    return fail(UDP_ERR_UNSUPPORTED, "udp_conv2d_fused_bn: a plain fp32 / bf16 NHWC conv without addends, ReLU or channel views");
  return conv2d_fused_impl(o, dtype, n, in, weights, bias, nullptr, nullptr, nullptr, nullptr, out, bn_ws, bn_ws_doubles, bn_rows, stream);
}

static int conv2d_params(const udp_conv_op* o, int dtype, int n, const void* in, const void* weights,
                         const float* bias, const void* res, const void* up0, const void* up1,
                         const void* up2, void* out, ConvParams* pp) {
  ConvParams& p = *pp;
  if (!o || !in || !out) return fail(UDP_ERR_ARG, "udp_conv2d_fused: null pointer");
  if (dtype != UDP_F32 && dtype != UDP_BF16 && dtype != UDP_F16X2) return fail(UDP_ERR_ARG, "udp_conv2d_fused: dtype %d", dtype);
  if (n <= 0) return fail(UDP_ERR_ARG, "udp_conv2d_fused: n=%d", n);
  if (o->kind != UDP_OP_CONV && o->kind != UDP_OP_FUSE && o->kind != UDP_OP_DECONV && o->kind != UDP_OP_DWCONV && o->kind != UDP_OP_PIXSHUF &&
      o->kind != UDP_OP_SE && o->kind != UDP_OP_GNORM && o->kind != UDP_OP_LINATTN && o->kind != UDP_OP_LNORM && o->kind != UDP_OP_MHATTN &&
      o->kind != UDP_OP_ACT)
    return fail(UDP_ERR_ARG, "udp_conv2d_fused: kind %d", o->kind);
  if (const int rc = act_validate(*o, dtype, res != nullptr)) return rc;
  if (o->kind != UDP_OP_FUSE && o->kind != UDP_OP_PIXSHUF && o->kind != UDP_OP_LINATTN && o->kind != UDP_OP_MHATTN && o->kind != UDP_OP_ACT && (!weights || (!bias && o->kind != UDP_OP_SE && o->kind != UDP_OP_GNORM && o->kind != UDP_OP_LNORM))) return fail(UDP_ERR_ARG, "udp_conv2d_fused: conv needs weights and bias");
  if (o->kind == UDP_OP_SE) {
    const int rc = se_validate(*o, dtype);
    if (rc) return rc;
    if (res) return fail(UDP_ERR_ARG, "udp_conv2d_fused: squeeze-excitation takes no residual");
    if (in == out && (o->in_coff != o->out_coff || (o->in_pitch ? o->in_pitch : o->cin) != (o->out_pitch ? o->out_pitch : o->cout)))
      return fail(UDP_ERR_ARG, "udp_conv2d_fused: squeeze-excitation in place needs the same view for in and out");
  }
  if (o->kind == UDP_OP_GNORM || o->kind == UDP_OP_LINATTN) {
    const bool gn = o->kind == UDP_OP_GNORM;
    const int rc = gn ? gnorm_validate(*o, dtype) : linattn_validate(*o, dtype);
    if (rc) return rc;
    if (res) return fail(UDP_ERR_ARG, "udp_conv2d_fused: %s takes no residual", gn ? "group norm" : "linear attention");
    if (in == out && (!gn || o->in_coff != o->out_coff || (o->in_pitch ? o->in_pitch : o->cin) != (o->out_pitch ? o->out_pitch : o->cout)))
      return fail(UDP_ERR_ARG, "udp_conv2d_fused: %s", gn ? "group norm in place needs the same view for in and out" : "linear attention: out must not be in");
  }
  if (o->kind == UDP_OP_LNORM || o->kind == UDP_OP_MHATTN || o->kind == UDP_OP_ACT) {
    const char* what = o->kind == UDP_OP_LNORM ? "layer norm" : o->kind == UDP_OP_MHATTN ? "multi-head attention" : "activation op";
    const int rc = o->kind == UDP_OP_LNORM ? lnorm_validate(*o, dtype) : o->kind == UDP_OP_MHATTN ? mhattn_validate(*o, dtype) : act_op_validate(*o, dtype);
    if (rc) return rc;
    if (res) return fail(UDP_ERR_ARG, "udp_conv2d_fused: %s takes no residual", what);
    if (in == out && (o->kind == UDP_OP_MHATTN || o->in_coff != o->out_coff || (o->in_pitch ? o->in_pitch : o->cin) != (o->out_pitch ? o->out_pitch : o->cout)))
      return fail(UDP_ERR_ARG, "udp_conv2d_fused: %s: %s", what, o->kind == UDP_OP_MHATTN ? "out must not be in" : "in place needs the same view for in and out");
  }
  if (o->kind == UDP_OP_DWCONV || o->kind == UDP_OP_PIXSHUF) {
    const bool dw = o->kind == UDP_OP_DWCONV;
    const int rc = dw ? dwconv_validate(*o, dtype) : pixshuf_validate(*o, dtype);
    if (rc) return rc;
    const bool pass = dw && o->n_out2 == 1;
    if (pass ? (!res || !up0) : (res != nullptr)) return fail(UDP_ERR_ARG, "udp_conv2d_fused: %s: res / up0 are the passthrough's source / destination (n_out2 = 1) and NULL otherwise", dw ? "depthwise conv" : "pixel shuffle");
  }
  if (o->kind == UDP_OP_DECONV) {
    if (o->ks != 4 || o->stride != 2 || o->hout != 2 * o->hin || o->wout != 2 * o->win)
      return fail(UDP_ERR_ARG, "udp_conv2d_fused: deconv must be k4 s2 p1 (output = 2x the input)");
    if (res || o->n_up || o->out_buf == UDP_BUF_OUTPUT) return fail(UDP_ERR_UNSUPPORTED, "udp_conv2d_fused: deconv takes no addends and writes NHWC");
  }
  if (o->cout <= 0 || o->cout_pad < o->cout || o->cout_pad % 32 || o->n_up < 0 || o->n_up > 3)
    return fail(UDP_ERR_ARG, "udp_conv2d_fused: bad cout/cout_pad/n_up");
  if (o->kind == UDP_OP_CONV) {
    if ((o->ks != 1 && o->ks != 3) || (o->stride != 1 && o->stride != 2)) return fail(UDP_ERR_ARG, "udp_conv2d_fused: ks/stride");
    const int pad = o->ks / 2;
    if (o->hout != (o->hin + 2 * pad - o->ks) / o->stride + 1 || o->wout != (o->win + 2 * pad - o->ks) / o->stride + 1)
      return fail(UDP_ERR_ARG, "udp_conv2d_fused: output size does not match input/stride");
  }
  const void* ups[3] = {up0, up1, up2};
  memset(&p, 0, sizeof(p));
  p.N = n;
  p.Hin = o->hin;
  p.Win = o->win;
  p.Cin = o->cin;
  p.Hout = o->hout;
  p.Wout = o->wout;
  p.Cout = o->cout;
  p.CoutPad = o->cout_pad;
  p.relu = o->relu;
  if (o->kind == UDP_OP_SE || o->kind == UDP_OP_GNORM || o->kind == UDP_OP_LNORM) {
    p.up_shift[0] = o->chain_cout;
  } else if (o->kind == UDP_OP_MHATTN) {
    p.up_shift[0] = o->chain_cout;
    p.up_shift[1] = o->up_shift[0];
  } else if (o->kind == UDP_OP_DWCONV) {
    if (o->n_out2) {
      p.nout2 = 1;
      p.out2[0] = const_cast<void*>(up0);
      p.out2_coff[0] = o->out2_coff[0];
      p.out2_pitch[0] = o->out2_pitch[0];
      p.up_shift[0] = o->chain_cout;
    }
  } else {
    if (o->n_out2) return fail(UDP_ERR_UNSUPPORTED, "udp_conv2d_fused: second outputs (n_out2) exist in udp_hrnet programs only");
    if (o->chain_cout) return fail(UDP_ERR_UNSUPPORTED, "udp_conv2d_fused: chained convs (chain_cout) exist in udp_hrnet programs only");
  }
  p.wfmt = o->wfmt;
  p.wexp = o->wexp;
  p.in_stuff2 = o->in_stuff2 ? 1 : 0;
  p.flip_from = n;
  p.in_pitch = o->in_pitch ? o->in_pitch : o->cin;
  p.in_coff = o->in_coff;
  p.out_pitch = o->out_pitch ? o->out_pitch : o->cout;
  p.out_coff = o->out_coff;
  p.res_pitch = o->res_pitch ? o->res_pitch : o->cout;
  p.res_coff = o->res_coff;
  p.in = in;
  p.out = out;
  p.out_nchw_f32 = o->out_buf == UDP_BUF_OUTPUT;
  p.res = res;
  p.wgt = weights;
  p.bias = bias;
  p.nup = o->n_up;
  for (int u = 0; u < o->n_up; ++u) {
    const int s = o->up_shift[u];
    if (!ups[u] || s < (o->kind == UDP_OP_FUSE ? 0 : 1) || s > 5 || (o->hout & ((1 << s) - 1)) || (o->wout & ((1 << s) - 1)))
      return fail(UDP_ERR_ARG, "udp_conv2d_fused: up %d", u);
    p.up[u] = ups[u];
    p.up_shift[u] = s;
  }
  return UDP_OK;
}

static int conv2d_fused_impl(const udp_conv_op* o, int dtype, int n, const void* in, const void* weights,
                             const float* bias, const void* res, const void* up0, const void* up1,
                             const void* up2, void* out, double* bn_ws, size_t bn_ws_doubles, int* bn_rows, void* stream) {
  ConvParams p;
  const int prc = conv2d_params(o, dtype, n, in, weights, bias, res, up0, up1, up2, out, &p);
  if (prc) return prc;
  hipStream_t s = reinterpret_cast<hipStream_t>(stream);
  Launch l;
  p.bn_ws = bn_ws;
  const int rc = o->kind == UDP_OP_FUSE     ? describe_fuse(p, dtype, &l)
                 : o->kind == UDP_OP_DECONV ? describe_deconv(p, dtype, &l)
                 : o->kind == UDP_OP_DWCONV ? describe_dwconv(p, dtype, o->ks, o->stride, &l)
                 : o->kind == UDP_OP_SE     ? describe_se(p, dtype, &l)
                 : o->kind == UDP_OP_GNORM  ? describe_gnorm(p, dtype, &l)
                 : o->kind == UDP_OP_LINATTN ? describe_linattn(p, dtype, &l)
                 : o->kind == UDP_OP_LNORM  ? describe_lnorm(p, dtype, &l)
                 : o->kind == UDP_OP_MHATTN ? describe_mhattn(p, dtype, &l)
                 : o->kind == UDP_OP_ACT    ? describe_act(p, dtype, &l)
                 : o->kind == UDP_OP_PIXSHUF ? describe_pixshuf(p, dtype, &l)
                                            : describe_conv(p, dtype, o->ks, o->stride, &l);
  if (rc) return rc;
  if (bn_ws) {
    if ((size_t)l.grid.x * 2 * o->cout > bn_ws_doubles || l.grid.x > (unsigned)udp_bn_rows_max())
      return fail(UDP_ERR_WORKSPACE, "udp_conv2d_fused_bn: %u partial rows x %d doubles exceed the workspace or the %d-row limit",
                  l.grid.x, 2 * o->cout, udp_bn_rows_max());
    *bn_rows = (int)l.grid.x;
  }
  return run_launch(l, s);
}

extern "C" int udp_conv2d_fused_group(udp_conv_item* items, int n_items, int dtype, int n, void* stream) {
  if (!items || n_items < 1 || n_items > 4) return fail(UDP_ERR_ARG, "udp_conv2d_fused_group: %d members (1..4)", n_items);
  hipStream_t s = reinterpret_cast<hipStream_t>(stream);
  std::vector<Launch> L((size_t)n_items);
  for (int j = 0; j < n_items; ++j) {
    udp_conv_item& it = items[j];
    const udp_conv_op* o = it.op;
    if (!o || o->kind != UDP_OP_CONV || o->n_up || o->out_buf == UDP_BUF_OUTPUT)
      return fail(UDP_ERR_UNSUPPORTED, "udp_conv2d_fused_group: member %d is not a plain NHWC conv", j);
    if (o->relu >= UDP_ACT_HSWISH) return fail(UDP_ERR_UNSUPPORTED, "udp_conv2d_fused_group: member %d: hard-swish / SiLU have no merged-launch form", j);
    if (it.bn_ws && (dtype == UDP_F16X2 || o->relu || it.res || (o->out_pitch && o->out_pitch != o->cout) || o->out_coff))
      return fail(UDP_ERR_UNSUPPORTED, "udp_conv2d_fused_group: member %d: BatchNorm sums need a plain fp32 / bf16 conv", j);
    ConvParams p;
    int rc = conv2d_params(o, dtype, n, it.in, it.weights, it.bias, it.res, nullptr, nullptr, nullptr, it.out, &p);
    if (rc) return rc;
    p.bn_ws = it.bn_ws;
    rc = n_items > 1 && getenv("UDP_POSE_NO_GROUPS") == nullptr ? describe_conv_grouped(p, dtype, o->ks, o->stride, &L[j]) : 1;
    if (rc == 1) rc = describe_conv(p, dtype, o->ks, o->stride, &L[j]);
    if (rc) return rc;
    if (it.bn_ws) {
      if ((size_t)L[j].grid.x * 2 * o->cout > it.bn_ws_doubles || L[j].grid.x > (unsigned)udp_bn_rows_max())
        return fail(UDP_ERR_WORKSPACE, "udp_conv2d_fused_group: member %d: %u partial rows x %d doubles exceed the workspace or the %d-row limit",
                    j, L[j].grid.x, 2 * o->cout, udp_bn_rows_max());
      it.bn_rows = (int)L[j].grid.x;
    }
  }
  std::vector<Launch> G;
  std::vector<int> rest;
  for (int j = 0; j < n_items; ++j) {
    if (L[j].groupable && (G.empty() || L[j].groupable / 10 == G[0].groupable / 10))
      G.push_back(L[j]);
    else
      rest.push_back(j);
  }
  if (G.size() >= 2) {
    ConvMulti m;
    Launch ml;
    const int rc = describe_multi(G.data(), (int)G.size(), &m, &ml);
    if (rc) return rc;
    void* args[] = {&m};
    UDP_HIP_CHECK(hipLaunchKernel(ml.fn, ml.grid, ml.block, args, ml.lds, s));
  } else {
    for (const Launch& l : G) {
      const int rc = run_launch(l, s);
      if (rc) return rc;
    }
  }
  for (int j : rest) {
    const int rc = run_launch(L[j], s);
    if (rc) return rc;
  }
  return UDP_OK;
}
```

Measured before the change: 8427 images/s.

## Fuse final 1x1 head convs, write flip halves in place, shrink decode LDS

Adds a fused head-chain kernel that runs the last two 1x1 convs (32->128 with upsample adds and ReLU, then 128->joints) in one pass, keeping the 128-channel intermediate in registers. It also adds an out_skip offset so each split-batch lane writes its flipped and unflipped heatmaps straight into the final buffer, removing the temp buffers and four device-to-device copies. The gaussian decode now reuses the raw plane for the blurred map, cutting LDS from three planes to two so more blocks can fit per CU. In exchange the head kernel is hand-specialised to fixed channel counts, and the split path's error handling is reworked.

After: 8611 images/s, median of 6. 2.2% higher.

```diff
diff --git a/udp-pose_amd/csrc/common.h b/udp-pose_amd/csrc/common.h
--- a/udp-pose_amd/csrc/common.h
+++ b/udp-pose_amd/csrc/common.h
@@ -80,6 +80,7 @@
   int wfmt;
   int wexp;
   int in_stuff2;
+  int out_skip;
   double* bn_ws;
   void* out2[2];
   const void* add2[2];
@@ -110,6 +111,7 @@
   unsigned lds = 0;
   int groupable = 0;
   int ws_cp = 0;
+  int pair = 0;
   ConvParams p;
 };
 int describe_conv_ws(ConvParams p, int ks, int stride, Launch* out, bool grouped = false);
@@ -120,6 +122,7 @@
 int choose_conv_ws(ConvParams& p, int ks, int stride, bool grouped, WsTile* best);
 int describe_ws_multi(const Launch* members, int n, ConvMulti* m, Launch* out);
 int describe_conv_chain(ConvParams p, Launch* out);
+int describe_head_chain(ConvParams p, const ConvParams& p2, Launch* out);
 void ws_set_fill_wgs(long wgs);
 int ws_set_stamps(unsigned long long* dev_buf);
 int describe_deconv(ConvParams p, int dtype, Launch* out);
diff --git a/udp-pose_amd/csrc/conv.hip b/udp-pose_amd/csrc/conv.hip
--- a/udp-pose_amd/csrc/conv.hip
+++ b/udp-pose_amd/csrc/conv.hip
@@ -1406,6 +1406,7 @@
     return describe_conv_ws(p, ks, stride, out);
   }
   if (p.wfmt != 0) return fail(UDP_ERR_ARG, "conv wfmt=%d", p.wfmt);
+  if (p.out_skip) return fail(UDP_ERR_UNSUPPORTED, "conv: an output written in place for a sub-batch lane (out_skip) needs fragment-major weights (wfmt 1)");
   int nb = 2;
   const size_t lds = conv_choose_tile(p, ks, stride, dtype, &nb);
   if (p.CoutPad % (nb * 16) != 0)
diff --git a/udp-pose_amd/csrc/conv_ws.hip b/udp-pose_amd/csrc/conv_ws.hip
--- a/udp-pose_amd/csrc/conv_ws.hip
+++ b/udp-pose_amd/csrc/conv_ws.hip
@@ -77,7 +77,7 @@
   constexpr bool dbg_nores = false;
 #endif
   const __amdgpu_buffer_rsrc_t r_out = __builtin_amdgcn_make_buffer_rsrc(
-      p.out, 0, (!p.out || dbg_nost) ? 0 : NCHW ? out_pix * p.Cout * 4 : out_pix * outpb, 0x00020000);
+      p.out, 0, (!p.out || dbg_nost) ? 0 : NCHW ? (out_pix + (unsigned)p.out_skip * p.Hout * p.Wout) * p.Cout * 4 : out_pix * outpb, 0x00020000);
   const __amdgpu_buffer_rsrc_t r_bias = __builtin_amdgcn_make_buffer_rsrc(
       const_cast<float*>(p.bias), 0, (unsigned)p.CoutPad * 4u, 0x00020000);
   const __amdgpu_buffer_rsrc_t r_res = __builtin_amdgcn_make_buffer_rsrc(
@@ -302,7 +302,8 @@
       const int crd = ocrd[i];
       const int y = crd & 1023, xo = (crd >> 10) & 1023, n = crd >> 20;
       const unsigned hw = __umul24(p.Hout, p.Wout);
-      const unsigned base = __umul24(__umul24(__umul24(n, p.Cout), p.Hout) + y, p.Wout) + xo;
+      const int no = n >= p.flip_from ? n + p.out_skip : n;
+      const unsigned base = __umul24(__umul24(__umul24(no, p.Cout), p.Hout) + y, p.Wout) + xo;
 #pragma unroll
       for (int nb = 0; nb < NB; ++nb)
 #pragma unroll
@@ -1051,6 +1052,192 @@
   return UDP_OK;
 }
 
+template <int Q>
+__global__ __launch_bounds__(512) void conv_head_chain_kernel(const ConvParams p) {
+  constexpr int ESZ = 2, NB = 2, PB = 2, NP = 4, NWAVES = 8;
+  extern __shared__ __attribute__((aligned(16))) unsigned char smem[];
+  const int lane = threadIdx.x & 63, wave = __builtin_amdgcn_readfirstlane(threadIdx.x >> 6);
+  const int li = lane & 15, kg = lane >> 4;
+  const unsigned hw = (unsigned)p.Hout * p.Wout;
+  const unsigned npix = (unsigned)p.N * hw;
+  const int cout2 = p.out2_pitch[0];
+  const unsigned inpb = (unsigned)p.in_pitch * ESZ * 2, in_lo = (unsigned)p.in_pitch * ESZ;
+  const __amdgpu_buffer_rsrc_t r_in = __builtin_amdgcn_make_buffer_rsrc(const_cast<void*>(p.in), 0, npix * inpb, 0x00020000);
+  const __amdgpu_buffer_rsrc_t r_w = __builtin_amdgcn_make_buffer_rsrc(const_cast<void*>(p.wgt), 0, (unsigned)NP * 4096u, 0x00020000);
+  const __amdgpu_buffer_rsrc_t r_w2 = __builtin_amdgcn_make_buffer_rsrc(const_cast<void*>(p.wgt2), 0, (unsigned)NP * Q * 4096u, 0x00020000);
+  const __amdgpu_buffer_rsrc_t r_z = __builtin_amdgcn_make_buffer_rsrc(p.out2[0], 0, (unsigned)(p.N + p.out_skip) * hw * (unsigned)cout2 * 4u, 0x00020000);
+  const float winv = __builtin_ldexpf(1.f, -p.wexp), winv2 = __builtin_ldexpf(1.f, -p.out2_coff[0]);
+  const unsigned uppb = (unsigned)p.Cout * ESZ * 2, up_lo = (unsigned)p.Cout * ESZ;
+  __amdgpu_buffer_rsrc_t r_up[3];
+#pragma unroll
+  for (int u = 0; u < 3; ++u)
+    r_up[u] = __builtin_amdgcn_make_buffer_rsrc(const_cast<void*>(p.up[u]), 0,
+                                                u < p.nup ? (unsigned)p.N * (p.Hout >> p.up_shift[u]) * (p.Wout >> p.up_shift[u]) * uppb : 0u, 0x00020000);
+
+  constexpr unsigned kW2 = (unsigned)NP * 4096u, kBias = kW2 + (unsigned)NP * Q * 4096u;
+  for (unsigned off = threadIdx.x * 16u; off < kBias; off += 512u * 16u) {
+    const u32x4 v = off < kW2 ? __builtin_amdgcn_raw_buffer_load_b128(r_w, off, 0, 0) : __builtin_amdgcn_raw_buffer_load_b128(r_w2, off - kW2, 0, 0);
+    *reinterpret_cast<u32x4*>(smem + off) = v;
+  }
+  float* sbias = reinterpret_cast<float*>(smem + kBias);
+  if (threadIdx.x < 128 + 32 * Q) sbias[threadIdx.x] = threadIdx.x < 128 ? p.bias[threadIdx.x] : p.bias2[threadIdx.x - 128];
+  __syncthreads();
+  auto load_a = [&](unsigned blk, f16x8 (&h)[NB], f16x8 (&l)[NB]) __attribute__((always_inline)) {
+#pragma unroll
+    for (int nb = 0; nb < NB; ++nb) {
+      const unsigned char* q = smem + blk + (unsigned)lane * 16u + 2048u * nb;
+      h[nb] = *reinterpret_cast<const f16x8*>(q);
+      l[nb] = *reinterpret_cast<const f16x8*>(q + 1024);
+    }
+  };
+  auto mfma3 = [&](f32x4 (&acc)[NB], const f16x8 (&h)[NB], const f16x8 (&l)[NB], const f16x8 (&a2)[NB], const f16x8 bh, const f16x8 bl)
+      __attribute__((always_inline)) {
+#pragma unroll
+        for (int nb = 0; nb < NB; ++nb) acc[nb] = __builtin_amdgcn_mfma_f32_16x16x32_f16(h[nb], bh, acc[nb], 0, 0, 0);
+#pragma unroll
+        for (int nb = 0; nb < NB; ++nb) acc[nb] = __builtin_amdgcn_mfma_f32_16x16x32_f16(l[nb], bh, acc[nb], 0, 0, 0);
+#pragma unroll
+        for (int nb = 0; nb < NB; ++nb) acc[nb] = __builtin_amdgcn_mfma_f32_16x16x32_f16(a2[nb], bl, acc[nb], 0, 0, 0);
+      };
+
+  const unsigned ngroups = (npix + PB * 16 - 1) / (PB * 16);
+  for (unsigned grp = (unsigned)blockIdx.x * NWAVES + wave; grp < ngroups; grp += gridDim.x * NWAVES) {
+    unsigned pix[PB], upoff[PB][3];
+    int pn[PB], py[PB], px[PB];
+    bool ok[PB];
+    f16x8 xh[PB], xl[PB];
+#pragma unroll
+    for (int i = 0; i < PB; ++i) {
+      pix[i] = grp * (PB * 16) + i * 16 + li;
+      ok[i] = pix[i] < npix;
+      const unsigned pc = ok[i] ? pix[i] : 0u;
+      pn[i] = (int)(pc / hw);
+      const unsigned rem = pc - (unsigned)pn[i] * hw;
+      py[i] = (int)(rem / (unsigned)p.Wout);
+      px[i] = (int)(rem - (unsigned)py[i] * p.Wout);
+      const unsigned off = ok[i] ? pix[i] * inpb + (unsigned)(p.in_coff + 8 * kg) * ESZ : kOobOff;
+      xh[i] = __builtin_bit_cast(f16x8, __builtin_amdgcn_raw_buffer_load_b128(r_in, off, 0, 0));
+      xl[i] = __builtin_bit_cast(f16x8, __builtin_amdgcn_raw_buffer_load_b128(r_in, off + in_lo, 0, 0));
+#pragma unroll
+      for (int u = 0; u < 3; ++u) {
+        const int sh = u < p.nup ? p.up_shift[u] : 0;
+        const unsigned up_pix = (unsigned)(pn[i] * (p.Hout >> sh) + (py[i] >> sh)) * (unsigned)(p.Wout >> sh) + (unsigned)(px[i] >> sh);
+        upoff[i][u] = ok[i] ? up_pix * uppb : kOobOff;
+      }
+    }
+    f32x4 acc2[PB][Q][NB];
+#pragma unroll
+    for (int i = 0; i < PB; ++i)
+#pragma unroll
+      for (int q = 0; q < Q; ++q)
+#pragma unroll
+        for (int nb = 0; nb < NB; ++nb) acc2[i][q][nb] = f32x4{0.f, 0.f, 0.f, 0.f};
+
+#pragma unroll
+    for (int pr = 0; pr < NP; ++pr) {
+      __builtin_amdgcn_sched_barrier(0);
+      const int cbase = 32 * pr + 8 * kg;
+      u32x4 uh[PB][3], ul[PB][3];
+#pragma unroll
+      for (int i = 0; i < PB; ++i)
+#pragma unroll
+        for (int u = 0; u < 3; ++u) {
+          uh[i][u] = __builtin_amdgcn_raw_buffer_load_b128(r_up[u], upoff[i][u] + (unsigned)cbase * ESZ, 0, 0);
+          ul[i][u] = __builtin_amdgcn_raw_buffer_load_b128(r_up[u], upoff[i][u] + (unsigned)cbase * ESZ + up_lo, 0, 0);
+        }
+      f16x8 ah[NB], al[NB], a2[NB];
+      load_a((unsigned)pr * 4096u, ah, al);
+#pragma unroll
+      for (int nb = 0; nb < NB; ++nb) a2[nb] = ah[nb] * (_Float16)0x1p-11f;
+      f32x4 bias[NB];
+#pragma unroll
+      for (int nb = 0; nb < NB; ++nb) bias[nb] = *reinterpret_cast<const f32x4*>(smem + kBias + (unsigned)(cbase + 4 * nb) * 4u);
+      f16x8 yh[PB], yl[PB];
+#pragma unroll
+      for (int i = 0; i < PB; ++i) {
+        f32x4 acc[NB];
+#pragma unroll
+        for (int nb = 0; nb < NB; ++nb) acc[nb] = f32x4{0.f, 0.f, 0.f, 0.f};
+        mfma3(acc, ah, al, a2, xh[i], xl[i]);
+#pragma unroll
+        for (int nb = 0; nb < NB; ++nb)
+#pragma unroll
+          for (int q = 0; q < 4; ++q) acc[nb][q] = __builtin_fmaf(acc[nb][q], winv, bias[nb][q]);
+#pragma unroll
+        for (int u = 0; u < 3; ++u) h2_add8(acc[0], acc[1], __builtin_bit_cast(f16x8, uh[i][u]), __builtin_bit_cast(f16x8, ul[i][u]));
+        if (p.relu) {
+#pragma unroll
+          for (int nb = 0; nb < NB; ++nb)
+#pragma unroll
+            for (int q = 0; q < 4; ++q) acc[nb][q] = acc[nb][q] > 0.f ? acc[nb][q] : 0.f;
+        }
+        h2_split8(acc[0], acc[1], yh[i], yl[i]);
+      }
+#pragma unroll
+      for (int q = 0; q < Q; ++q) {
+        f16x8 bh[NB], bl[NB], b2[NB];
+        load_a(kW2 + (unsigned)(pr * Q + q) * 4096u, bh, bl);
+#pragma unroll
+        for (int nb = 0; nb < NB; ++nb) b2[nb] = bh[nb] * (_Float16)0x1p-11f;
+#pragma unroll
+        for (int i = 0; i < PB; ++i) mfma3(acc2[i][q], bh, bl, b2, yh[i], yl[i]);
+      }
+    }
+#pragma unroll
+    for (int q = 0; q < Q; ++q) {
+      f32x4 b2[NB];
+#pragma unroll
+      for (int nb = 0; nb < NB; ++nb) b2[nb] = *reinterpret_cast<const f32x4*>(smem + kBias + 512u + (unsigned)(32 * q + 8 * kg + 4 * nb) * 4u);
+#pragma unroll
+      for (int i = 0; i < PB; ++i) {
+        const int no = pn[i] >= p.flip_from ? pn[i] + p.out_skip : pn[i];
+        const unsigned base = ((unsigned)no * (unsigned)cout2 * (unsigned)p.Hout + (unsigned)py[i]) * (unsigned)p.Wout + (unsigned)px[i];
+#pragma unroll
+        for (int nb = 0; nb < NB; ++nb)
+#pragma unroll
+          for (int k = 0; k < 4; ++k) {
+            const int cc = 32 * q + 8 * kg + 4 * nb + k;
+            const float f = __builtin_fmaf(acc2[i][q][nb][k], winv2, b2[nb][k]);
+            const unsigned off = (ok[i] && cc < cout2) ? (base + (unsigned)cc * hw) * 4u : kOobOff;
+            __builtin_amdgcn_raw_buffer_store_b32(__builtin_bit_cast(unsigned, f), r_z, off, 0, 0);
+          }
+      }
+    }
+  }
+}
+
+int describe_head_chain(ConvParams p, const ConvParams& p2, Launch* out) {
+  const int q = p2.CoutPad / 32;
+  if (p.Cin != 32 || p.Cout != 128 || p.CoutPad != 128 || p2.Cin != 128 || (q != 1 && q != 2) || p2.Cout > p2.CoutPad || p.wfmt != 1 ||
+      p2.wfmt != 1 || p.relu != UDP_ACT_RELU || p2.relu || p.res || p2.res || p2.nup || p.nout2 || p2.nout2 || !p2.out_nchw_f32 ||
+      p.Hin != p.Hout || p.Win != p.Wout || p2.Hout != p.Hout || p2.Wout != p.Wout || p2.N != p.N || p.in_pitch % 8 || p.in_coff % 8)
+    return 1;
+  const long npix = (long)p.N * p.Hout * p.Wout;
+  if (npix * p.in_pitch * 4 >= 0x7FFF0000L || npix * 128 >= 0x7FFF0000L || (long)(p.N + p2.out_skip) * p.Hout * p.Wout * p2.Cout * 4 >= 0x7FFF0000L) return 1;
+  for (int u = 0; u < p.nup; ++u)
+    if (!p.up[u]) return 1;
+  p.wgt2 = p2.wgt;
+  p.bias2 = p2.bias;
+  p.out2[0] = p2.out;
+  p.out2_pitch[0] = p2.Cout;
+  p.out2_coff[0] = p2.wexp;
+  p.flip_from = p2.flip_from;
+  p.out_skip = p2.out_skip;
+  p.out = nullptr;
+  const long groups = (npix + 31) / 32;
+  out->fn = q == 1 ? reinterpret_cast<const void*>(&conv_head_chain_kernel<1>) : reinterpret_cast<const void*>(&conv_head_chain_kernel<2>);
+  out->lds = (unsigned)(4 * 4096 + 4 * q * 4096 + (128 + 32 * q) * 4);
+  out->grid = dim3((unsigned)std::min<long>(256, (groups + 7) / 8));
+  out->block = dim3(512);
+  out->groupable = 0;
+  out->ws_cp = 0;
+  out->p = p;
+  UDP_HIP_CHECK(hipFuncSetAttribute(out->fn, hipFuncAttributeMaxDynamicSharedMemorySize, (int)out->lds));
+  if (getenv("UDP_POSE_DEBUG_TILES"))
+    fprintf(stderr, "head chain %dx%d C%d->%d->%d: wgs=%u lds=%u\n", p.Hout, p.Wout, p.Cin, p.Cout, p2.Cout, out->grid.x, out->lds);
+  return UDP_OK;
+}
+
 int conv_ws_h2_overflow(hipStream_t s, int reset, int* flag) { return h2_overflow_fetch(s, reset, flag); }
 
 }
diff --git a/udp-pose_amd/csrc/decode.hip b/udp-pose_amd/csrc/decode.hip
--- a/udp-pose_amd/csrc/decode.hip
+++ b/udp-pose_amd/csrc/decode.hip
@@ -140,7 +140,7 @@
   const int hw = h * w;
   float* raw = sm;
   float* tmp = sm + hw;
-  float* blr = sm + 2 * hw;
+  float* blr = sm;
   const int map = blockIdx.x;
   const int n = map / j;
   const float* src = hm + (size_t)map * hw;
@@ -303,10 +303,10 @@
 }
 
 static int check_decode_args(const char* who, const void* hm, int n, int j, int h, int w, const void* c,
-                             const void* s, const void* preds, const void* maxvals, const void* pin) {
+                             const void* s, const void* preds, const void* maxvals, const void* pin, int planes) {
   if (!hm || !c || !s || !preds || !maxvals || !pin) return fail(UDP_ERR_ARG, "%s: null pointer", who);
   if (n < 0 || j <= 0 || h <= 0 || w <= 0) return fail(UDP_ERR_ARG, "%s: bad shape n=%d j=%d h=%d w=%d", who, n, j, h, w);
-  if ((size_t)h * w * 3 * sizeof(float) > 150 * 1024)
+  if ((size_t)h * w * planes * sizeof(float) > 150 * 1024)
     return fail(UDP_ERR_UNSUPPORTED, "%s: map %dx%d does not fit the LDS working set", who, h, w);
   return UDP_OK;
 }
@@ -314,12 +314,12 @@
 extern "C" int udp_decode_gaussian(const float* heatmaps, int n, int j, int h, int w, const double* center,
                                    const double* scale, int cs_is_f32, int post_process, double* preds,
                                    float* maxvals, double* preds_in, int32_t* argidx, void* stream) {
-  int rc = check_decode_args("udp_decode_gaussian", heatmaps, n, j, h, w, center, scale, preds, maxvals, preds_in);
+  int rc = check_decode_args("udp_decode_gaussian", heatmaps, n, j, h, w, center, scale, preds, maxvals, preds_in, 2);
   if (rc) return rc;
   if (n == 0) return UDP_OK;
   Taps t7;
   make_taps(7, &t7);
-  const size_t lds = (size_t)h * w * 3 * sizeof(float);
+  const size_t lds = (size_t)h * w * 2 * sizeof(float);
   static bool attr = false;
   if (!attr) {
     UDP_HIP_CHECK(hipFuncSetAttribute(reinterpret_cast<const void*>(decode_gaussian_kernel),
@@ -335,7 +335,7 @@
 extern "C" int udp_decode_offset(const float* heatmaps, int n, int j, int h, int w, const double* center,
                                  const double* scale, int cs_is_f32, float kpd, double* preds, float* maxvals,
                                  double* preds_in, int32_t* argidx, void* stream) {
-  int rc = check_decode_args("udp_decode_offset", heatmaps, n, j, h, w, center, scale, preds, maxvals, preds_in);
+  int rc = check_decode_args("udp_decode_offset", heatmaps, n, j, h, w, center, scale, preds, maxvals, preds_in, 3);
   if (rc) return rc;
   if (n == 0) return UDP_OK;
   Taps t15, t7;
diff --git a/udp-pose_amd/csrc/hrnet.hip b/udp-pose_amd/csrc/hrnet.hip
--- a/udp-pose_amd/csrc/hrnet.hip
+++ b/udp-pose_amd/csrc/hrnet.hip
@@ -20,7 +20,7 @@
 using namespace udp;
 
 struct GraphEntry {
-  int n, flip;
+  int n, flip, skip;
   const void* in;
   void* ws;
   void* out;
@@ -46,6 +46,7 @@
   hipEvent_t ev_fork = nullptr, ev_join[UDP_MAX_LANES] = {nullptr, nullptr, nullptr, nullptr};
   hipStream_t split_stream = nullptr;
   hipEvent_t split_fork = nullptr, split_join = nullptr;
+  bool out_in_place = false;
 };
 
 static size_t esize(int dtype) { return dtype == UDP_BF16 ? 2 : 4; }
@@ -334,6 +335,9 @@
     delete h;
     return fail(UDP_ERR_ARG, "udp_hrnet_create: program needs a stem op first and the output op last, both on lane 0");
   }
+  h->out_in_place = dtype == UDP_F16X2;
+  for (int i = 0; i < n_ops; ++i)
+    if (ops[i].out_buf == UDP_BUF_OUTPUT && (ops[i].kind != UDP_OP_CONV || ops[i].wfmt != 1)) h->out_in_place = false;
   h->op_signals.assign(n_ops, 0);
   for (int i = 0; i < n_ops; ++i) {
     if (ops[i].lane + 1 > h->n_lanes) h->n_lanes = ops[i].lane + 1;
@@ -378,7 +382,39 @@
 extern "C" int udp_hrnet_num_launches(const udp_hrnet* h) { return h ? (int)h->ops.size() : 0; }
 extern "C" double udp_hrnet_flops_per_image(const udp_hrnet* h) { return h ? h->flops : 0.0; }
 
-static int describe_all(const udp_hrnet* h, const float* in, int n, int flip, char* ws, float* out,
+static int mark_head_chain(const udp_hrnet* h, std::vector<Launch>& L) {
+  const char* off = getenv("UDP_POSE_NO_HEAD_CHAIN");
+  if (h->dtype != UDP_F16X2 || (off && atoi(off) != 0)) return UDP_OK;
+  for (size_t i = 0; i + 1 < h->ops.size(); ++i) {
+    const udp_conv_op& a = h->ops[i];
+    const udp_conv_op& b = h->ops[i + 1];
+    if (a.kind != UDP_OP_CONV || a.ks != 1 || a.stride != 1 || a.wfmt != 1 || a.relu != UDP_ACT_RELU || a.cin % 32 || a.out_buf < 0 ||
+        a.out_coff || (a.out_pitch && a.out_pitch != a.cout) || a.res_buf != UDP_BUF_NONE || a.n_out2 || a.chain_cout || a.group || a.in_stuff2)
+      continue;
+    if (b.kind != UDP_OP_CONV || b.ks != 1 || b.stride != 1 || b.wfmt != 1 || b.out_buf != UDP_BUF_OUTPUT || b.res_buf != UDP_BUF_NONE ||
+        b.n_up || b.relu || b.n_out2 || b.chain_cout || b.group || b.in_stuff2 || b.in_buf != a.out_buf || b.in_coff ||
+        (b.in_pitch && b.in_pitch != a.cout) || b.cin != a.cout || b.lane != a.lane)
+      continue;
+    bool shared = false;
+    for (size_t k = i + 2; k < h->ops.size() && !shared; ++k) {
+      const udp_conv_op& o = h->ops[k];
+      shared = o.in_buf == a.out_buf || o.res_buf == a.out_buf || (o.chain_cout && o.chain_buf == a.out_buf);
+      for (int u = 0; u < o.n_up && u < 3; ++u) shared |= o.up_buf[u] == a.out_buf;
+      for (int u = 0; u < o.n_out2 && u < 2; ++u) shared |= o.add2_buf[u] == a.out_buf || o.out2_buf[u] == a.out_buf;
+    }
+    if (shared) continue;
+    Launch fused;
+    const int rc = describe_head_chain(L[i].p, L[i + 1].p, &fused);
+    if (rc == 1) continue;
+    if (rc) return rc;
+    fused.pair = 1;
+    L[i] = fused;
+    ++i;
+  }
+  return UDP_OK;
+}
+
+static int describe_all(const udp_hrnet* h, const float* in, int n, int flip, int out_skip, char* ws, float* out,
                         std::vector<Launch>& ls) {
   const int B = n * (flip ? 2 : 1);
   const size_t es = esize(h->dtype);
@@ -409,6 +445,7 @@
     p.res_coff = o.res_coff;
     p.in = is_stem ? reinterpret_cast<const void*>(in) : buf(o.in_buf);
     p.out_nchw_f32 = o.out_buf == UDP_BUF_OUTPUT;
+    p.out_skip = p.out_nchw_f32 ? out_skip : 0;
     p.out = p.out_nchw_f32 ? reinterpret_cast<void*>(out) : o.out_buf == UDP_BUF_NONE ? nullptr : buf(o.out_buf);
     p.res = o.res_buf == UDP_BUF_NONE ? nullptr : buf(o.res_buf);
     p.nup = o.n_up;
@@ -486,7 +523,7 @@
     }
     if (rc) return rc;
   }
-  return UDP_OK;
+  return mark_head_chain(h, ls);
 }
 
 struct Node {
@@ -498,16 +535,19 @@
   *grouped = false;
   for (size_t i = 0; i < L.size();) {
     int n = 1;
-    if (L[i].groupable && h->ops[i].group != 0)
+    if (L[i].pair) {
+      n = 2;
+    } else if (L[i].groupable && h->ops[i].group != 0) {
       while (n < 4 && i + n < L.size() && L[i + n].groupable / 10 == L[i].groupable / 10 && h->ops[i + n].group == h->ops[i].group) ++n;
+      *grouped |= n > 1;
+    }
     nodes.push_back({i, n});
-    *grouped |= n > 1;
     i += n;
   }
   return nodes;
 }
 static int run_node(const std::vector<Launch>& L, const Node& nd, hipStream_t s) {
-  if (nd.n == 1) return run_launch(L[nd.first], s);
+  if (nd.n == 1 || L[nd.first].pair) return run_launch(L[nd.first], s);
   ConvMulti m;
   Launch ml;
   const int rc = describe_multi(&L[nd.first], nd.n, &m, &ml);
@@ -541,14 +581,18 @@
   for (size_t i = 0; i < h->ops.size(); ++i) {
     const udp_conv_op& o = h->ops[i];
     hipStream_t os = ls[o.lane];
+    const size_t last = i + (L[i].pair ? 1 : 0);
     if (lanes)
-      for (int k = 0; k < o.n_wait; ++k)
-        if (h->ops[o.wait_op[k]].lane != o.lane) UDP_HIP_CHECK(hipStreamWaitEvent(os, h->op_done[o.wait_op[k]], 0));
+      for (size_t j = i; j <= last; ++j)
+        for (int k = 0; k < h->ops[j].n_wait; ++k)
+          if (h->ops[h->ops[j].wait_op[k]].lane != o.lane) UDP_HIP_CHECK(hipStreamWaitEvent(os, h->op_done[h->ops[j].wait_op[k]], 0));
     if (ev) UDP_HIP_CHECK(hipEventRecord(ev[2 * i], os));
     const int rc = run_launch(L[i], os);
     if (rc) return rc;
     if (ev) UDP_HIP_CHECK(hipEventRecord(ev[2 * i + 1], os));
-    if (lanes && h->op_signals[i]) UDP_HIP_CHECK(hipEventRecord(h->op_done[i], os));
+    for (size_t j = i; j <= last; ++j)
+      if (lanes && h->op_signals[j]) UDP_HIP_CHECK(hipEventRecord(h->op_done[j], os));
+    i = last;
   }
   if (lanes)
     for (int l = 1; l < h->n_lanes; ++l) {
@@ -574,13 +618,15 @@
       if (k) deps.push_back(node[k - 1]);
     } else {
       if (last_on_lane[o.lane] >= 0) deps.push_back(node[last_on_lane[o.lane]]);
-      for (int w = 0; w < o.n_wait; ++w) deps.push_back(node[node_of_op[o.wait_op[w]]]);
+      for (int j = 0; j < nodes[k].n; ++j)
+        for (int w = 0; w < h->ops[i + j].n_wait; ++w)
+          if ((size_t)h->ops[i + j].wait_op[w] < i) deps.push_back(node[node_of_op[h->ops[i + j].wait_op[w]]]);
     }
     ConvParams p = L[i].p;
     ConvMulti m;
     Launch ml = L[i];
     void* args[1] = {&p};
-    if (nodes[k].n > 1) {
+    if (nodes[k].n > 1 && !L[i].pair) {
       const int rc = describe_multi(&L[i], nodes[k].n, &m, &ml);
       if (rc) {
         (void)hipGraphDestroy(*graph);
@@ -629,7 +675,7 @@
   if (!ms_per_op) return fail(UDP_ERR_ARG, "udp_hrnet_profile: null pointer");
   hipStream_t s = reinterpret_cast<hipStream_t>(stream);
   std::vector<Launch> L;
-  rc = describe_all(h, in_nchw, n, flip_test ? 1 : 0, reinterpret_cast<char*>(workspace), heatmaps_nchw, L);
+  rc = describe_all(h, in_nchw, n, flip_test ? 1 : 0, 0, reinterpret_cast<char*>(workspace), heatmaps_nchw, L);
   if (rc) return rc;
   const size_t nops = h->ops.size();
   std::vector<hipEvent_t> ev(2 * nops, nullptr);
@@ -660,13 +706,13 @@
   return UDP_OK;
 }
 
-static int forward_one(udp_hrnet* h, const float* in_nchw, int n, int flip_test, void* workspace, float* heatmaps_nchw,
-                       int use_graph, hipStream_t s) {
+static int forward_one(udp_hrnet* h, const float* in_nchw, int n, int flip_test, int out_skip, void* workspace,
+                       float* heatmaps_nchw, int use_graph, hipStream_t s) {
   int rc;
   if (use_graph)
     for (size_t k = 0; k < h->graphs.size(); ++k) {
       const GraphEntry g = h->graphs[k];
-      if (g.n == n && g.flip == flip_test && g.in == in_nchw && g.ws == workspace && g.out == heatmaps_nchw) {
+      if (g.n == n && g.flip == flip_test && g.skip == out_skip && g.in == in_nchw && g.ws == workspace && g.out == heatmaps_nchw) {
         if (k + 1 != h->graphs.size()) {
           h->graphs.erase(h->graphs.begin() + k);
           h->graphs.push_back(g);
@@ -676,12 +722,13 @@
       }
     }
   std::vector<Launch> L;
-  rc = describe_all(h, in_nchw, n, flip_test, reinterpret_cast<char*>(workspace), heatmaps_nchw, L);
+  rc = describe_all(h, in_nchw, n, flip_test, out_skip, reinterpret_cast<char*>(workspace), heatmaps_nchw, L);
   if (rc) return rc;
   if (!use_graph) return enqueue_all(h, L, s, nullptr, 1);
   GraphEntry e;
   e.n = n;
   e.flip = flip_test;
+  e.skip = out_skip;
   e.in = in_nchw;
   e.ws = workspace;
   e.out = heatmaps_nchw;
@@ -704,7 +751,7 @@
   if (rc) return rc;
   hipStream_t s = reinterpret_cast<hipStream_t>(stream);
   flip_test = flip_test ? 1 : 0;
-  if (!use_graph || !split_ok(h, n)) return forward_one(h, in_nchw, n, flip_test, workspace, heatmaps_nchw, use_graph, s);
+  if (!use_graph || !split_ok(h, n)) return forward_one(h, in_nchw, n, flip_test, 0, workspace, heatmaps_nchw, use_graph, s);
   if (!h->split_stream) {
     UDP_HIP_CHECK(hipStreamCreateWithFlags(&h->split_stream, hipStreamNonBlocking));
     UDP_HIP_CHECK(hipEventCreateWithFlags(&h->split_fork, hipEventDisableTiming));
@@ -720,28 +767,42 @@
   const size_t img_in = (size_t)3 * h->in_h * h->in_w;
   const size_t img_out = out_bytes(h, 1) / sizeof(float);
   hipStream_t s2 = h->split_stream;
-  UDP_HIP_CHECK(hipEventRecord(h->split_fork, s));
-  UDP_HIP_CHECK(hipStreamWaitEvent(s2, h->split_fork, 0));
-  if (!flip_test) {
-    rc = forward_one(h, in_nchw, n0, 0, ws0, heatmaps_nchw, 1, s);
-    if (!rc) rc = forward_one(h, in_nchw + n0 * img_in, n1, 0, ws1, heatmaps_nchw + n0 * img_out, 1, s2);
+  hipError_t he = hipSuccess;
+  const char* he_what = "";
+  auto hip_try = [&](hipError_t e, const char* what) {
+    if (e != hipSuccess && he == hipSuccess) {
+      he = e;
+      he_what = what;
+    }
+    return e == hipSuccess;
+  };
+  bool forked = hip_try(hipEventRecord(h->split_fork, s), "hipEventRecord(fork)");
+  forked = forked && hip_try(hipStreamWaitEvent(s2, h->split_fork, 0), "hipStreamWaitEvent(fork)");
+  if (!forked) {
+  } else if (!flip_test) {
+    rc = forward_one(h, in_nchw, n0, 0, 0, ws0, heatmaps_nchw, 1, s);
+    if (!rc) rc = forward_one(h, in_nchw + n0 * img_in, n1, 0, 0, ws1, heatmaps_nchw + n0 * img_out, 1, s2);
+  } else if (h->out_in_place && (size_t)2 * n * img_out * sizeof(float) < 0x7FFF0000u) {
+    rc = forward_one(h, in_nchw, n0, 1, n - n0, ws0, heatmaps_nchw, 1, s);
+    if (!rc) rc = forward_one(h, in_nchw + n0 * img_in, n1, 1, n0, ws1, heatmaps_nchw + n0 * img_out, 1, s2);
   } else {
     float* t0 = reinterpret_cast<float*>(ws1 + ws_bytes_one(h, n1, 1));
     float* t1 = t0 + 2 * n0 * img_out;
-    rc = forward_one(h, in_nchw, n0, 1, ws0, t0, 1, s);
+    rc = forward_one(h, in_nchw, n0, 1, 0, ws0, t0, 1, s);
     if (!rc) {
-      UDP_HIP_CHECK(hipMemcpyAsync(heatmaps_nchw, t0, n0 * img_out * sizeof(float), hipMemcpyDeviceToDevice, s));
-      UDP_HIP_CHECK(hipMemcpyAsync(heatmaps_nchw + n * img_out, t0 + n0 * img_out, n0 * img_out * sizeof(float), hipMemcpyDeviceToDevice, s));
-      rc = forward_one(h, in_nchw + n0 * img_in, n1, 1, ws1, t1, 1, s2);
+      hip_try(hipMemcpyAsync(heatmaps_nchw, t0, n0 * img_out * sizeof(float), hipMemcpyDeviceToDevice, s), "hipMemcpyAsync(lane 0)");
+      hip_try(hipMemcpyAsync(heatmaps_nchw + n * img_out, t0 + n0 * img_out, n0 * img_out * sizeof(float), hipMemcpyDeviceToDevice, s), "hipMemcpyAsync(lane 0, mirrored)");
+      rc = forward_one(h, in_nchw + n0 * img_in, n1, 1, 0, ws1, t1, 1, s2);
     }
     if (!rc) {
-      UDP_HIP_CHECK(hipMemcpyAsync(heatmaps_nchw + n0 * img_out, t1, n1 * img_out * sizeof(float), hipMemcpyDeviceToDevice, s2));
-      UDP_HIP_CHECK(hipMemcpyAsync(heatmaps_nchw + (n + n0) * img_out, t1 + n1 * img_out, n1 * img_out * sizeof(float), hipMemcpyDeviceToDevice, s2));
-    }
-  }
-  UDP_HIP_CHECK(hipEventRecord(h->split_join, s2));
-  UDP_HIP_CHECK(hipStreamWaitEvent(s, h->split_join, 0));
-  return rc;
+      hip_try(hipMemcpyAsync(heatmaps_nchw + n0 * img_out, t1, n1 * img_out * sizeof(float), hipMemcpyDeviceToDevice, s2), "hipMemcpyAsync(lane 1)");
+      hip_try(hipMemcpyAsync(heatmaps_nchw + (n + n0) * img_out, t1 + n1 * img_out, n1 * img_out * sizeof(float), hipMemcpyDeviceToDevice, s2), "hipMemcpyAsync(lane 1, mirrored)");
+    }
+  }
+  if (forked && hip_try(hipEventRecord(h->split_join, s2), "hipEventRecord(join)")) hip_try(hipStreamWaitEvent(s, h->split_join, 0), "hipStreamWaitEvent(join)");
+  if (rc) return rc;
+  if (he != hipSuccess) return fail(UDP_ERR_HIP, "udp_hrnet_forward: %s failed: %s", he_what, hipGetErrorString(he));
+  return UDP_OK;
 }
 
 extern "C" int udp_hrnet_destroy(udp_hrnet* h) {
```
